# MrOlm/inStrain

Measured on AMD Instinct MI355X. Metric: Gbp profiled/s, higher is better.
Workload: dtype u32

## Files before the change

include/instrain_amd.h:

```cpp
#ifndef INSTRAIN_AMD_H
#define INSTRAIN_AMD_H

#include <stdint.h>

#ifdef __cplusplus
extern "C" {
#endif

#define ISX_OK 0
#define ISX_ERR_ARG (-1)
#define ISX_ERR_HIP (-2)
#define ISX_ERR_CAPACITY (-3)
#define ISX_ERR_MM_RANGE (-4)
#define ISX_ERR_IO (-5)
#define ISX_ERR_STATE (-6)

#define ISX_ABI_VERSION 5


typedef struct isx_ctx isx_ctx;
typedef struct isx_batch isx_batch;
typedef struct isx_bam isx_bam;
struct isx_bam_params_s;
struct isx_bam_info_s;
// ... 206 lines not shown
int isx_genes_create(isx_ctx *ctx, int64_t n_genes, const isx_gene *genes, const char *seq, int64_t seq_bytes, isx_genes **out);
void isx_genes_destroy(isx_genes *g);
int isx_genes_sites(isx_genes *g, double *sites, float *device_ms);
int isx_batch_profile_genes(isx_batch *b, isx_genes *g, int32_t n_scaffolds, const int64_t *scaffold_bounds, const int32_t *gene_first,
                            const int32_t *gene_last, isx_gene_cov *cov_out, uint8_t *scaffold_flags, float *device_ms);
int isx_genes_profile_snvs(isx_genes *g, int32_t n_scaffolds, const int64_t *scaffold_bounds, const int32_t *gene_first,
                           const int32_t *gene_last, int64_t n_snv, const isx_snv *snv, int32_t n_levels, isx_gene_mutation *mut_out,
                           isx_gene_snv_count *cnt_out, float *device_ms);

typedef struct isx_pipe isx_pipe;

typedef struct {
    int64_t max_pos;
    int64_t max_obs;
    int32_t max_splits;
    int32_t depth;
    int32_t host_threads;
    int32_t pin_threads;
    double jump_slack;
    int32_t want_counts;
    int32_t ring_kib;
    int32_t stage_async;
    int32_t lean_output;
    int64_t max_segs;
} isx_pipe_params;

typedef struct {
    uint32_t gpos;
    float clon_rarefied;
} isx_rare;

typedef struct {
    uint32_t gpos;
    uint32_t coverage;
} isx_sat;

typedef struct {
    int64_t ticket;
    int64_t n_pos, n_obs;
    isx_sizes sizes;
    const uint16_t *coverage16;
    const float *clon;
    const isx_rare *rare;
    int64_t n_rare, n_saturated;
    const uint32_t *counts;
    const float *clon_rarefied;
    const isx_snv *snv;
    isx_batch *batch;
    float encode_ms;
    float h2d_ms, kernel_ms, d2h_ms;
    float collect_wait_ms;
    int32_t record_bytes;
    int32_t encode_passes;
    int64_t h2d_bytes, d2h_bytes;
    const isx_ld *ld;
    const uint8_t *coverage8;
    const isx_rare *clon_sparse;
    int64_t n_clon;
    const isx_sat *saturated;
    const uint8_t *coverage4;
    const uint16_t *cov_rows;
    const uint32_t *cov_row_window;
    int64_t n_cov_rows;
    int32_t cov_window, pad_cov;
    const void *lev_mask;
    const void *lev_cov;
    const uint32_t *lev_win_off;
    const isx_rare *lev_clon, *lev_rare;
    const isx_sat *lev_sat;
    int64_t n_lev, n_lev_clon, n_lev_rare, n_lev_sat;
    int32_t lev_mask_bytes, lev_cov_bytes, lev_window, n_lev_windows, lev_min_cov, pad_lev;
    uint64_t rows_checksum;
} isx_pipe_result;

int isx_levels_expand(const isx_pipe_result *r, int32_t host_threads, uint32_t *gpos, uint32_t *mm_cov, float *clon, float *clon_rarefied);

int isx_pipe_create(isx_ctx *ctx, const isx_params *params, const isx_pipe_params *pp, isx_pipe **out);
void isx_pipe_destroy(isx_pipe *p);
int isx_pipe_submit(isx_pipe *p, int64_t n_pos, const uint8_t *ref, int32_t n_splits, const int64_t *split_bounds,
                    int64_t n_obs, const isx_obs *obs, const uint32_t *pair, int64_t *ticket);
int isx_pipe_submit_bam(isx_pipe *p, isx_bam *bam, const struct isx_bam_params_s *bp, const int32_t *refs, int32_t n_refs,
                        const uint8_t *ref, int32_t n_splits, const int64_t *split_bounds, struct isx_bam_info_s *info,
                        int64_t *ticket);
int isx_pipe_collect(isx_pipe *p, int64_t ticket, isx_pipe_result *out);
int isx_pipe_release(isx_pipe *p, int64_t ticket);
int isx_pipe_fetch_entries(isx_pipe *p, int64_t ticket, isx_entry *out);
int isx_pipe_fetch_entries_shrunk(isx_pipe *p, int64_t ticket, uint32_t *gpos, uint32_t *mm_cov, float *clon, float *clon_rarefied);


#define ISX_SEG_BASES 150
#define ISX_SEG_WORDS 15
#define ISX_SEG_SKIP_WORD 0x24924924u
#define ISX_DREC_WORDS 8
#define ISX_DREC_EXC 6
#define ISX_DREC_EXC_FULL 3
#define ISX_DREC_DUAL 0x80000000u
#define ISX_DREC_NO_EXC 0x3FFFFFFFu

typedef struct {
    int64_t n_seg;
    const uint32_t *gpos;
    const uint8_t *len;
    const uint8_t *mm;
    const uint32_t *pair;
    const uint32_t *bases;
} isx_segs;

int isx_batch_create_reads(isx_ctx *ctx, const isx_params *params, int64_t n_pos, const uint8_t *ref, int32_t n_splits,
                           const int64_t *split_bounds, const isx_segs *segs, isx_batch **out);
int isx_pipe_submit_reads(isx_pipe *p, int64_t n_pos, const uint8_t *ref, int32_t n_splits, const int64_t *split_bounds,
                          const isx_segs *segs, int64_t *ticket);

typedef struct isx_wire isx_wire;
int isx_pipe_stage_reads(isx_pipe *p, int64_t n_pos, const uint8_t *ref, int32_t n_splits, const int64_t *split_bounds,
                         const isx_segs *segs, isx_wire **out);
int isx_pipe_submit_wire(isx_pipe *p, const isx_wire *wire, int64_t *ticket);
int64_t isx_wire_bytes(const isx_wire *wire);
void isx_wire_free(isx_wire *wire);
int isx_wire_keep_reference(isx_pipe *p, isx_wire *wire);

#define ISX_PLANE_WORDS 8
typedef struct {
    int64_t n_seg;
    const uint32_t *gpos;
    const uint8_t *len;
    const uint32_t *pair;
    const uint64_t *planes;
    const uint8_t *mm;
} isx_read_planes;

typedef struct {
    const uint8_t *plane2;
    const uint8_t *nplane;
    uint64_t key;
} isx_ref_planes;

int isx_pack_ref_planes(const uint8_t *ref, int64_t n_pos, int32_t host_threads, uint8_t *plane2, uint8_t *nplane, int32_t *has_n);
int isx_planes_from_segs(const isx_segs *segs, int32_t host_threads, uint64_t *planes);
int isx_pack_read_planes(int64_t n_reads, const int64_t *ref_start, const int64_t *clip_lo, const int64_t *clip_hi,
                         const uint32_t *cigar, const int64_t *cigar_off, const char *seq, const uint8_t *qual, const int64_t *seq_off,
                         const uint32_t *pair, int32_t min_base_quality, int64_t cap_seg, uint32_t *seg_gpos,
                         uint8_t *seg_len, uint32_t *seg_pair, uint64_t *seg_planes, int64_t *n_seg);
int isx_pipe_submit_planes(isx_pipe *p, int64_t n_pos, const isx_ref_planes *ref, int32_t n_splits, const int64_t *split_bounds,
                           const isx_read_planes *reads, int64_t *ticket);
int isx_pipe_stage_planes(isx_pipe *p, int64_t n_pos, const isx_ref_planes *ref, int32_t n_splits, const int64_t *split_bounds,
                          const isx_read_planes *reads, isx_wire **out);
int isx_pipe_set_reference_budget(isx_pipe *p, int64_t mib);
int isx_host_register(const void *ptr, int64_t bytes);
int isx_host_unregister(const void *ptr);
int isx_encode_planes(const isx_read_planes *reads, const isx_ref_planes *ref, int64_t n_pos, int32_t host_threads, int32_t slack_groups,
                      int64_t cap_rec, int64_t ring_records, uint32_t *rec, uint32_t *gbase, int64_t *n_rec, int64_t *need_slack);
int isx_encode_planes_mm(const isx_read_planes *reads, const isx_ref_planes *ref, int64_t n_pos, int32_t n_mm_bins, int32_t host_threads, int32_t slack_groups,
                         int64_t cap_rec, int64_t ring_records, uint32_t *rec, uint32_t *gbase, int64_t *n_rec, int64_t *need_slack);

int isx_count_read_segs(int64_t n_reads, const uint32_t *cigar, const int64_t *cigar_off, const int64_t *ref_start,
                        const int64_t *clip_lo, const int64_t *clip_hi, int64_t *n_seg);
int isx_pack_reads(int64_t n_reads, const int64_t *ref_start, const int64_t *clip_lo, const int64_t *clip_hi,
                   const uint32_t *cigar, const int64_t *cigar_off, const char *seq, const uint8_t *qual, const int64_t *seq_off,
                   const uint8_t *mm, const uint32_t *pair, int32_t min_base_quality, int64_t cap_seg, uint32_t *seg_gpos,
                   uint8_t *seg_len, uint8_t *seg_mm, uint32_t *seg_pair, uint32_t *seg_bases, int64_t *n_seg);

int isx_encode_segs(const isx_segs *segs, int64_t n_pos, int32_t n_mm_bins, int32_t host_threads, int64_t cap_rec, uint32_t *rec,
                    uint32_t *gbase, uint32_t *pair_out, int64_t *n_rec);
int64_t isx_seg_records_needed(const uint32_t *gpos, int64_t n_seg, int32_t host_threads);
int isx_encode_segs_ring(const isx_segs *segs, int64_t n_pos, int32_t n_mm_bins, int32_t host_threads, int64_t cap_rec, int64_t ring_records,
                         uint32_t *rec, uint32_t *gbase, uint32_t *pair_out, int64_t *n_rec);

int isx_encode_delta(const isx_segs *segs, const uint8_t *ref, int64_t n_pos, int32_t n_mm_bins, int32_t host_threads, int32_t slack_groups,
                     int64_t cap_rec, int64_t ring_records, uint32_t *rec, uint32_t *gbase, uint32_t *pair_out, int64_t *n_rec, int64_t *need_slack);
int64_t isx_delta_records_needed(const uint32_t *gpos, int64_t n_seg, int32_t host_threads, int32_t slack_groups);

int isx_encode_obs(const isx_obs *obs, const uint32_t *pair, int64_t n_obs, int64_t n_pos, int32_t record_bytes,
                   int32_t host_threads, double slack, int64_t cap_rec, void *rec, uint32_t *gbase, uint32_t *pair_out,
                   int64_t *n_rec, int32_t *passes);
int isx_encode_obs_ring(const isx_obs *obs, const uint32_t *pair, int64_t n_obs, int64_t n_pos, int32_t record_bytes,
                        int32_t host_threads, double slack, int64_t cap_rec, int64_t ring_records, void *rec,
                        uint32_t *gbase, uint32_t *pair_out, int64_t *n_rec, int32_t *passes);

typedef struct {
    int64_t in_off;
    int32_t in_len;
    int32_t out_len;
    int64_t out_off;
} isx_bgzf_block;
int isx_bgzf_index(const uint8_t *image, int64_t n_bytes, int64_t cap_blocks, isx_bgzf_block *blocks, int64_t *n_blocks, int64_t *out_bytes);
int isx_bgzf_inflate_device(isx_ctx *ctx, const uint8_t *image, int64_t n_bytes, const isx_bgzf_block *blocks, int64_t n_blocks,
                            uint8_t *out, int64_t out_bytes, float *kernel_ms);
int isx_bgzf_inflate_host(const uint8_t *image, int64_t n_bytes, const isx_bgzf_block *blocks, int64_t n_blocks, uint8_t *out, int64_t out_bytes);
int isx_bgzf_inflate_fast(const uint8_t *image, int64_t n_bytes, const isx_bgzf_block *blocks, int64_t n_blocks, uint8_t *out, int64_t out_bytes);

typedef struct isx_bam_params_s {
    double min_read_ani;
    int32_t min_mapq;
    double max_insert_relative;
    int32_t min_insert;
    int32_t min_base_quality;
    int32_t skip_mm;
    int32_t window_length;
    int32_t pairing_filter;
} isx_bam_params;

typedef struct isx_bam_info_s {
    int32_t n_refs;
    int32_t n_splits;
    int64_t n_reads;
    int64_t n_pos;
    int64_t n_obs;
    int64_t n_pairs;
    int64_t unfiltered_pairs, filtered_pairs;
    int64_t filtered_bases;
    double median_insert;
    int32_t max_mm;
    int32_t pad;
    int64_t unfiltered_reads, unfiltered_singletons, filtered_singletons;
    int64_t n_segs;
} isx_bam_info;

int isx_bam_open(const char *path, isx_bam **out);
void isx_bam_close(isx_bam *bam);
void isx_bam_close_wait(isx_bam *bam);
int isx_bam_set_threads(isx_bam *bam, int32_t threads);
int isx_bam_ref(const isx_bam *bam, int32_t i, const char **name, int64_t *length, int64_t *flat_offset);
int isx_bam_set_priority_reads(isx_bam *bam, int64_t n, const char *names, const int64_t *offs);
int isx_bam_scan(isx_bam *bam, isx_bam_info *info );
int isx_bam_scan_part(isx_bam *bam, int32_t part, int32_t n_parts, isx_bam_info *info );
int isx_bam_set_wanted_refs(isx_bam *bam, const int32_t *refs, int32_t n);
int isx_bam_insert_sizes(isx_bam *bam, int64_t *out, int64_t cap, int64_t *n);
int isx_bam_filter(isx_bam *bam, const isx_bam_params *p, double median_insert , isx_bam_info *info);
int isx_bam_pair_keys(isx_bam *bam, uint64_t *h1, uint64_t *h2, int32_t *tid, int64_t *info4, int64_t cap, int64_t *n);
int isx_bam_set_cross_names(isx_bam *bam, int64_t n, const int64_t *entry, const int64_t *occurrences, const int64_t *info4);
int isx_bam_filter_insert_sizes(isx_bam *bam, int64_t *out, int64_t cap, int64_t *n);
int isx_bam_set_r2m(isx_bam *bam, int32_t ref, int64_t n, const char *names, const int64_t *offs, const int32_t *mm );
int isx_bam_set_mm_cap(isx_bam *bam, int32_t cap);
int isx_bam_mm_levels(const isx_bam *bam, int32_t *levels, int32_t cap, int32_t *n);
int isx_bam_set_mm_levels(isx_bam *bam, const int32_t *levels, int32_t n);
int isx_bam_batch_pair_names(const isx_bam *bam, int64_t *n, int64_t *name_bytes, char *names, int64_t *offs);
int isx_bam_r2m(const isx_bam *bam, int32_t ref, int64_t *n, int64_t *name_bytes, char *names, int64_t *offs, int32_t *mm);
int isx_bam_drop_names(isx_bam *bam);
int isx_bam_ref_counts(const isx_bam *bam, int64_t *reads, int64_t *filtered_pairs);
int isx_bam_expand_refs(isx_bam *bam, const isx_bam_params *p, const int32_t *refs, int32_t n_refs, isx_bam_info *info);
int isx_bam_segment_refs(isx_bam *bam, const isx_bam_params *p, const int32_t *refs, int32_t n_refs, isx_bam_info *info, int64_t *n_seg);
int isx_bam_copy_segs(const isx_bam *bam, uint32_t *gpos, uint8_t *len, uint8_t *mm, uint32_t *pair, uint32_t *bases,
                      int64_t *split_bounds, int32_t *split_ref);
int isx_bam_copy_read_planes(const isx_bam *bam, uint64_t *planes);
int isx_bam_expand_region(isx_bam *bam, const isx_bam_params *p, int32_t ref, int64_t start, int64_t stop, isx_bam_info *info);
int isx_bam_expand(isx_bam *bam, const isx_bam_params *p, isx_bam_info *info);
int isx_bam_copy(const isx_bam *bam, isx_obs *obs, uint32_t *pair, int64_t *split_bounds, int32_t *split_ref);
int isx_bam_view(const isx_bam *bam, const isx_obs **obs, const uint32_t **pair);

#ifdef __cplusplus
}
#endif
#endif
```

instrain_amd/_lib.py:

```python
import ctypes as C
import os

import numpy as np

_HERE = os.path.dirname(os.path.abspath(__file__))
LIB_PATH = os.path.join(_HERE, "libinstrain_amd.so")
if os.environ.get("ISX_LIB"):
    LIB_PATH = os.path.abspath(os.environ["ISX_LIB"])

BGZF_BLOCK_DT = np.dtype([("in_off", np.int64), ("in_len", np.int32), ("out_len", np.int32), ("out_off", np.int64)])
OBS_DT = np.dtype([("gpos", "<u4"), ("mm", "<u2"), ("base", "u1"), ("flags", "u1")])
ENTRY_DT = np.dtype([("gpos", "<u4"), ("mm", "<u2"), ("flags", "<u2"), ("cnt", "<u4", (4,)), ("clon", "<f4"),
                     ("clon_rarefied", "<f4")])
SNV_DT = np.dtype([("gpos", "<u4"), ("mm", "<u2"), ("con_base", "u1"), ("var_base", "u1"),
                   ("allele_count", "u1"), ("cls", "u1"), ("cryptic", "u1"), ("ref_base", "u1"),
                   ("cnt", "<u4", (4,))])
LD_DT = np.dtype([("gpos_a", "<u4"), ("gpos_b", "<u4"), ("mm", "<u2"), ("allele_A", "u1"), ("allele_a", "u1"),
                  ("allele_B", "u1"), ("allele_b", "u1"), ("pad", "<u2"), ("total", "<u4"), ("countAB", "<u4"),
                  ("countAb", "<u4"), ("countaB", "<u4"), ("countab", "<u4"), ("pad2", "<u4"),
                  ("r2", "<f8"), ("d_prime", "<f8"), ("r2_normalized", "<f8"), ("d_prime_normalized", "<f8")])
AO_DT = np.dtype([("pair", "<u4"), ("gpos", "<u4"), ("order", "<u4"), ("mm", "<u2"), ("base", "u1"), ("pad", "u1")])
assert AO_DT.itemsize == 16
assert OBS_DT.itemsize == 8 and ENTRY_DT.itemsize == 32 and SNV_DT.itemsize == 28 and LD_DT.itemsize == 72


class Params(C.Structure):
    _fields_ = [("min_cov", C.c_int32), ("min_snp", C.c_int32), ("min_freq", C.c_double),
                ("rarefied_coverage", C.c_int32), ("n_mm_bins", C.c_int32), ("enable_linkage", C.c_int32),
                ("linkage_mode", C.c_int32), ("window", C.c_int32), ("seed", C.c_uint64), ("layout", C.c_int32),
                ("reserved", C.c_int32)]


LAYOUT_WIDE_RECORDS, LAYOUT_NO_SHORT_RECORDS, LAYOUT_NO_PACKED_COUNTERS, LAYOUT_SEG64_RECORDS = 1, 2, 4, 8


class PipeParams(C.Structure):
    _fields_ = [("max_pos", C.c_int64), ("max_obs", C.c_int64), ("max_splits", C.c_int32), ("depth", C.c_int32),
                ("host_threads", C.c_int32), ("pin_threads", C.c_int32), ("jump_slack", C.c_double),
                ("want_counts", C.c_int32), ("ring_kib", C.c_int32), ("stage_async", C.c_int32), ("lean_output", C.c_int32),
                ("max_segs", C.c_int64)]


SEG_BASES, SEG_WORDS, SEG_SKIP_WORD = 150, 15, 0x24924924


class Segs(C.Structure):
    _fields_ = [("n_seg", C.c_int64), ("gpos", C.c_void_p), ("len", C.c_void_p), ("mm", C.c_void_p), ("pair", C.c_void_p),
                ("bases", C.c_void_p)]


PLANE_WORDS = 8
LAYOUT_MM_ENTRIES = 16
LAYOUT_MM_DELTA_RECORDS = 32
ABI_VERSION = 5


class ReadPlanes(C.Structure):
    _fields_ = [("n_seg", C.c_int64), ("gpos", C.c_void_p), ("len", C.c_void_p), ("pair", C.c_void_p), ("planes", C.c_void_p), ("mm", C.c_void_p)]


class RefPlanes(C.Structure):
    _fields_ = [("plane2", C.c_void_p), ("nplane", C.c_void_p), ("key", C.c_uint64)]


RARE_DT = np.dtype([("gpos", "<u4"), ("clon_rarefied", "<f4")])
CLON_DT = np.dtype([("gpos", "<u4"), ("clon", "<f4")])
SAT_DT = np.dtype([("gpos", "<u4"), ("coverage", "<u4")])


class Sizes(C.Structure):
    _fields_ = [(n, C.c_int64) for n in ("n_entries", "n_snv", "n_sites", "n_allele_obs", "n_increments",
                                         "n_edges", "n_ld")]


class Timings(C.Structure):
    _fields_ = [(n, C.c_float) for n in ("pileup_ms", "sites_ms", "allele_ms", "group_ms", "incr_ms", "ld_ms",
                                         "total_ms")] + \
               [(n, C.c_int32) for n in ("pileup_blocks", "pileup_threads", "pileup_lds_bytes", "pileup_window")] + \
               [("mfma_ms", C.c_float), ("dense_tiles", C.c_int32), ("dense_macs", C.c_int64), ("dense_bytes", C.c_int64),
                ("record_bytes", C.c_int32), ("pad", C.c_int32)]


class PipeResult(C.Structure):
    _fields_ = [("ticket", C.c_int64), ("n_pos", C.c_int64), ("n_obs", C.c_int64), ("sizes", Sizes),
                ("coverage16", C.c_void_p), ("clon", C.c_void_p), ("rare", C.c_void_p), ("n_rare", C.c_int64),
                ("n_saturated", C.c_int64), ("counts", C.c_void_p), ("clon_rarefied", C.c_void_p), ("snv", C.c_void_p),
                ("batch", C.c_void_p),
                ("encode_ms", C.c_float), ("h2d_ms", C.c_float), ("kernel_ms", C.c_float), ("d2h_ms", C.c_float),
                ("collect_wait_ms", C.c_float), ("record_bytes", C.c_int32), ("encode_passes", C.c_int32),
                ("h2d_bytes", C.c_int64), ("d2h_bytes", C.c_int64), ("ld", C.c_void_p),
                ("coverage8", C.c_void_p), ("clon_sparse", C.c_void_p), ("n_clon", C.c_int64), ("saturated", C.c_void_p),
                ("coverage4", C.c_void_p), ("cov_rows", C.c_void_p), ("cov_row_window", C.c_void_p), ("n_cov_rows", C.c_int64),
                ("cov_window", C.c_int32), ("pad_cov", C.c_int32),
                ("lev_mask", C.c_void_p), ("lev_cov", C.c_void_p), ("lev_win_off", C.c_void_p), ("lev_clon", C.c_void_p), ("lev_rare", C.c_void_p),
                ("lev_sat", C.c_void_p), ("n_lev", C.c_int64), ("n_lev_clon", C.c_int64), ("n_lev_rare", C.c_int64), ("n_lev_sat", C.c_int64),
                ("lev_mask_bytes", C.c_int32), ("lev_cov_bytes", C.c_int32), ("lev_window", C.c_int32), ("n_lev_windows", C.c_int32),
                ("lev_min_cov", C.c_int32), ("pad_lev", C.c_int32), ("rows_checksum", C.c_uint64)]


class BamParams(C.Structure):
    _fields_ = [("min_read_ani", C.c_double), ("min_mapq", C.c_int32), ("max_insert_relative", C.c_double),
                ("min_insert", C.c_int32), ("min_base_quality", C.c_int32), ("skip_mm", C.c_int32),
                ("window_length", C.c_int32), ("pairing_filter", C.c_int32)]


PAIRING_FILTERS = {"paired_only": 0, "non_discordant": 1, "all_reads": 2}


class BamInfo(C.Structure):
    _fields_ = [("n_refs", C.c_int32), ("n_splits", C.c_int32), ("n_reads", C.c_int64), ("n_pos", C.c_int64),
                ("n_obs", C.c_int64), ("n_pairs", C.c_int64), ("unfiltered_pairs", C.c_int64),
                ("filtered_pairs", C.c_int64), ("filtered_bases", C.c_int64), ("median_insert", C.c_double),
                ("max_mm", C.c_int32), ("pad", C.c_int32), ("unfiltered_reads", C.c_int64),
                ("unfiltered_singletons", C.c_int64), ("filtered_singletons", C.c_int64), ("n_segs", C.c_int64)]


SCAFFOLD_LEVEL_DT = np.dtype([("nonzero", "<i8"), ("sum_cov", "<u8"), ("sumsq_cov", "<u8"), ("median_cov", "<f8"),
                              ("counted", "<i8"), ("sum_clon", "<f8"), ("median_clon", "<f8"),
                              ("counted_rarefied", "<i8"), ("sum_clon_rarefied", "<f8"),
                              ("median_clon_rarefied", "<f8"), ("mm", "<i4"), ("present", "<i4")])
assert SCAFFOLD_LEVEL_DT.itemsize == 88
GENOME_LEVEL_DT = np.dtype([("n", "<i8"), ("sum_cov", "<u8"), ("sumsq_cov", "<u8"), ("median_cov", "<f8"), ("mm", "<i4"), ("pad", "<i4")])
assert GENOME_LEVEL_DT.itemsize == 40


COMPARE_LEVEL_DT = np.dtype([("both", "<i8"), ("either", "<i8"), ("mm", "<i4"), ("present_a", "<i4"),
                             ("present_b", "<i4"), ("pad", "<i4"), ("consensus_snps", "<i8"), ("population_snps", "<i8")])
assert COMPARE_LEVEL_DT.itemsize == 48
COMPARE_SNP_DT = np.dtype([("gpos", "<u4"), ("mm", "<u2"), ("consensus_snp", "u1"), ("population_snp", "u1"),
                           ("has_a", "u1"), ("has_b", "u1"), ("con_a", "u1"), ("ref_a", "u1"), ("var_a", "u1"),
                           ("con_b", "u1"), ("ref_b", "u1"), ("var_b", "u1"), ("cnt_a", "<u4", (4,)), ("cnt_b", "<u4", (4,))])
assert COMPARE_SNP_DT.itemsize == 48


GENE_DT = np.dtype([("start", "<i8"), ("end", "<i8"), ("seq_off", "<i8"), ("strand", "<i4"), ("pad", "<i4")])
GENE_COV_DT = np.dtype([("sum_cov", "<u8"), ("nonzero", "<u4"), ("counted", "<u4"), ("sum_clon", "<f8")])
GENE_SNV_COUNT_DT = np.dtype([(n, "<u4") for n in ("divergent", "sns", "sns_n", "sns_s", "snv", "snv_n", "snv_s")])
GENE_MUTATION_DT = np.dtype([("gene", "<i4"), ("k", "<i4"), ("type", "u1"), ("aa_old", "u1"), ("aa_new", "u1"), ("n_genes", "u1"),
                             ("pad", "<u4")])
assert GENE_DT.itemsize == 32 and GENE_COV_DT.itemsize == 24 and GENE_SNV_COUNT_DT.itemsize == 28 and GENE_MUTATION_DT.itemsize == 16
GENE_LEVEL_PRESENT, GENE_COV_ANY, GENE_CLON_ANY = 1, 2, 4


ERR_CAPACITY = -3


class IsxError(RuntimeError):
    def __init__(self, code, msg):
        super().__init__("libinstrain_amd error %d: %s" % (code, msg))
        self.code = code


SYMBOLS = ["isx_last_error", "isx_abi_version", "isx_ctx_create", "isx_ctx_destroy", "isx_ctx_reserve_cus", "isx_set_null_model",
           "isx_batch_create", "isx_batch_create_reads", "isx_batch_destroy", "isx_batch_run", "isx_batch_launch", "isx_batch_wait", "isx_batch_sizes", "isx_batch_timings",
           "isx_batch_fetch_entries", "isx_batch_fetch_dense", "isx_batch_fetch_snv", "isx_batch_fetch_ld", "isx_batch_fetch_allele_obs",
           "isx_batch_summarize", "isx_batch_summarize_genomes", "isx_compare_coverage", "isx_compare_scaffolds", "isx_compare_fetch_snps",
           "isx_genes_create", "isx_genes_destroy", "isx_genes_sites", "isx_batch_profile_genes", "isx_genes_profile_snvs",
           "isx_pipe_create", "isx_pipe_destroy", "isx_pipe_submit", "isx_pipe_submit_reads", "isx_pipe_stage_reads", "isx_pipe_submit_wire", "isx_wire_bytes", "isx_wire_free", "isx_wire_keep_reference", "isx_pipe_submit_bam", "isx_encode_segs", "isx_encode_segs_ring", "isx_seg_records_needed", "isx_encode_delta", "isx_delta_records_needed", "isx_count_read_segs", "isx_pack_reads", "isx_pipe_collect", "isx_pipe_release", "isx_pipe_fetch_entries", "isx_pipe_fetch_entries_shrunk", "isx_levels_expand", "isx_encode_obs", "isx_encode_obs_ring",
           "isx_pack_ref_planes", "isx_planes_from_segs", "isx_pack_read_planes", "isx_pipe_submit_planes", "isx_pipe_stage_planes", "isx_encode_planes", "isx_encode_planes_mm", "isx_pipe_set_reference_budget", "isx_host_register", "isx_host_unregister",
           "isx_bgzf_index", "isx_bgzf_inflate_device", "isx_bgzf_inflate_host", "isx_bgzf_inflate_fast",
           "isx_bam_open", "isx_bam_close", "isx_bam_close_wait", "isx_bam_set_threads", "isx_bam_ref", "isx_bam_set_priority_reads", "isx_bam_scan", "isx_bam_scan_part",
           "isx_bam_insert_sizes", "isx_bam_set_wanted_refs", "isx_bam_pair_keys", "isx_bam_set_cross_names", "isx_bam_filter_insert_sizes", "isx_bam_filter", "isx_bam_set_r2m", "isx_bam_r2m", "isx_bam_drop_names", "isx_bam_batch_pair_names", "isx_bam_set_mm_cap", "isx_bam_mm_levels", "isx_bam_set_mm_levels", "isx_bam_ref_counts",
           "isx_bam_expand_refs", "isx_bam_segment_refs", "isx_bam_copy_segs", "isx_bam_copy_read_planes", "isx_bam_expand_region", "isx_bam_expand", "isx_bam_copy", "isx_bam_view"]

_lib = None


def load():
    global _lib
    if _lib is not None:
        return _lib
    if not os.path.exists(LIB_PATH):
        raise IsxError(-2, "%s not built: run `python -c 'import __graft_entry__ as g; g.build()'` "
                           "(hipcc --offload-arch=gfx950)" % LIB_PATH)
    lib = C.CDLL(LIB_PATH)
    vp, i32, i64 = C.c_void_p, C.c_int32, C.c_int64
    lib.isx_last_error.restype = C.c_char_p
    lib.isx_abi_version.restype = C.c_int
    if lib.isx_abi_version() != ABI_VERSION:
        raise IsxError(-6, "%s has ABI version %d, this package binds version %d: rebuild it (python -c 'import __graft_entry__ as g; g.build()')"
                       % (LIB_PATH, lib.isx_abi_version(), ABI_VERSION))
    lib.isx_ctx_create.argtypes = [C.c_int, C.POINTER(vp)]
    lib.isx_ctx_destroy.argtypes = [vp]
    lib.isx_ctx_reserve_cus.argtypes = [vp, C.c_int]
    lib.isx_bgzf_index.argtypes = [vp, i64, i64, vp, C.POINTER(i64), C.POINTER(i64)]
    lib.isx_bgzf_inflate_device.argtypes = [vp, vp, i64, vp, i64, vp, i64, C.POINTER(C.c_float)]
    lib.isx_bgzf_inflate_host.argtypes = [vp, i64, vp, i64, vp, i64]
    lib.isx_bgzf_inflate_fast.argtypes = [vp, i64, vp, i64, vp, i64]
    lib.isx_ctx_destroy.restype = None
    lib.isx_set_null_model.argtypes = [vp, vp, i64, i32]
    lib.isx_batch_create.argtypes = [vp, C.POINTER(Params), i64, vp, i32, vp, i64, vp, vp, C.POINTER(vp)]
    lib.isx_batch_create_reads.argtypes = [vp, C.POINTER(Params), i64, vp, i32, vp, C.POINTER(Segs), C.POINTER(vp)]
    lib.isx_pipe_submit_reads.argtypes = [vp, i64, vp, i32, vp, C.POINTER(Segs), C.POINTER(i64)]
    lib.isx_pipe_stage_reads.argtypes = [vp, i64, vp, i32, vp, C.POINTER(Segs), C.POINTER(vp)]
    lib.isx_pipe_submit_wire.argtypes = [vp, vp, C.POINTER(i64)]
    lib.isx_wire_bytes.argtypes = [vp]
    lib.isx_wire_bytes.restype = i64
    lib.isx_wire_free.argtypes = [vp]
    lib.isx_wire_keep_reference.argtypes = [vp, vp]
    lib.isx_wire_free.restype = None
    lib.isx_encode_segs.argtypes = [C.POINTER(Segs), i64, i32, i32, i64, vp, vp, vp, C.POINTER(i64)]
    lib.isx_encode_segs_ring.argtypes = [C.POINTER(Segs), i64, i32, i32, i64, i64, vp, vp, vp, C.POINTER(i64)]
    lib.isx_encode_delta.argtypes = [C.POINTER(Segs), vp, i64, i32, i32, i32, i64, i64, vp, vp, vp, C.POINTER(i64), C.POINTER(i64)]
    lib.isx_delta_records_needed.argtypes = [vp, i64, i32, i32]
    lib.isx_delta_records_needed.restype = i64
    lib.isx_seg_records_needed.argtypes = [vp, i64, i32]
    lib.isx_seg_records_needed.restype = i64
    lib.isx_count_read_segs.argtypes = [i64, vp, vp, vp, vp, vp, C.POINTER(i64)]
    lib.isx_pack_reads.argtypes = [i64, vp, vp, vp, vp, vp, vp, vp, vp, vp, vp, i32, i64, vp, vp, vp, vp, vp, C.POINTER(i64)]
    lib.isx_batch_destroy.argtypes = [vp]
    lib.isx_batch_destroy.restype = None
    lib.isx_batch_run.argtypes = [vp]
    lib.isx_batch_launch.argtypes = [vp]
    lib.isx_batch_wait.argtypes = [vp]
    lib.isx_batch_sizes.argtypes = [vp, C.POINTER(Sizes)]
    lib.isx_batch_timings.argtypes = [vp, C.POINTER(Timings)]
    for f in ("isx_batch_fetch_entries", "isx_batch_fetch_snv", "isx_batch_fetch_ld", "isx_batch_fetch_allele_obs"):
        getattr(lib, f).argtypes = [vp, vp]
    lib.isx_batch_fetch_dense.argtypes = [vp, vp, vp, vp]
    lib.isx_batch_summarize.argtypes = [vp, i32, vp, vp, C.POINTER(C.c_float)]
    lib.isx_batch_summarize_genomes.argtypes = [vp, i32, vp, i32, vp, i32, vp, C.POINTER(C.c_float)]
    lib.isx_compare_coverage.argtypes = [vp, vp, i32, vp, i32, vp, C.POINTER(C.c_float)]
    lib.isx_compare_scaffolds.argtypes = [vp, vp, i32, vp, i32, C.c_double, vp, C.POINTER(i64), C.POINTER(C.c_float)]
    lib.isx_compare_fetch_snps.argtypes = [vp, vp]
    lib.isx_genes_create.argtypes = [vp, i64, vp, C.c_char_p, i64, C.POINTER(vp)]
    lib.isx_genes_destroy.argtypes = [vp]
    lib.isx_genes_destroy.restype = None
    lib.isx_genes_sites.argtypes = [vp, vp, C.POINTER(C.c_float)]
    lib.isx_batch_profile_genes.argtypes = [vp, vp, i32, vp, vp, vp, vp, vp, C.POINTER(C.c_float)]
    lib.isx_genes_profile_snvs.argtypes = [vp, i32, vp, vp, vp, i64, vp, i32, vp, vp, C.POINTER(C.c_float)]
    lib.isx_pipe_create.argtypes = [vp, C.POINTER(Params), C.POINTER(PipeParams), C.POINTER(vp)]
    lib.isx_pipe_destroy.argtypes = [vp]
    lib.isx_pipe_destroy.restype = None
    lib.isx_pipe_submit.argtypes = [vp, i64, vp, i32, vp, i64, vp, vp, C.POINTER(i64)]
    lib.isx_pipe_submit_bam.argtypes = [vp, vp, C.POINTER(BamParams), vp, i32, vp, i32, vp, C.POINTER(BamInfo), C.POINTER(i64)]
    lib.isx_pipe_collect.argtypes = [vp, i64, C.POINTER(PipeResult)]
    lib.isx_pipe_release.argtypes = [vp, i64]
    lib.isx_pipe_fetch_entries.argtypes = [vp, i64, vp]
    lib.isx_pipe_fetch_entries_shrunk.argtypes = [vp, i64, vp, vp, vp, vp]
    lib.isx_levels_expand.argtypes = [C.POINTER(PipeResult), i32, vp, vp, vp, vp]
    lib.isx_encode_obs.argtypes = [vp, vp, i64, i64, i32, i32, C.c_double, i64, vp, vp, vp, C.POINTER(i64), C.POINTER(i32)]
    lib.isx_encode_obs_ring.argtypes = [vp, vp, i64, i64, i32, i32, C.c_double, i64, i64, vp, vp, vp, C.POINTER(i64), C.POINTER(i32)]
    lib.isx_bam_open.argtypes = [C.c_char_p, C.POINTER(vp)]
    lib.isx_bam_close.argtypes = [vp]
    lib.isx_bam_close.restype = None
    lib.isx_bam_close_wait.argtypes = [vp]
    lib.isx_bam_close_wait.restype = None
    lib.isx_bam_expand.argtypes = [vp, C.POINTER(BamParams), C.POINTER(BamInfo)]
    lib.isx_bam_set_threads.argtypes = [vp, i32]
    lib.isx_bam_set_priority_reads.argtypes = [vp, i64, C.c_char_p, vp]
    lib.isx_bam_scan.argtypes = [vp, C.POINTER(BamInfo)]
    lib.isx_bam_scan_part.argtypes = [vp, i32, i32, C.POINTER(BamInfo)]
    lib.isx_bam_set_wanted_refs.argtypes = [vp, vp, i32]
    lib.isx_bam_insert_sizes.argtypes = [vp, vp, i64, C.POINTER(i64)]
    lib.isx_bam_filter_insert_sizes.argtypes = [vp, vp, i64, C.POINTER(i64)]
    lib.isx_bam_pair_keys.argtypes = [vp, vp, vp, vp, vp, i64, C.POINTER(i64)]
    lib.isx_bam_set_cross_names.argtypes = [vp, i64, vp, vp, vp]
    lib.isx_bam_filter.argtypes = [vp, C.POINTER(BamParams), C.c_double, C.POINTER(BamInfo)]
    lib.isx_bam_set_r2m.argtypes = [vp, i32, i64, C.c_char_p, vp, vp]
    lib.isx_bam_drop_names.argtypes = [vp]
    lib.isx_bam_r2m.argtypes = [vp, i32, C.POINTER(i64), C.POINTER(i64), vp, vp, vp]
    lib.isx_bam_batch_pair_names.argtypes = [vp, C.POINTER(i64), C.POINTER(i64), vp, vp]
    lib.isx_bam_set_mm_cap.argtypes = [vp, i32]
    lib.isx_bam_mm_levels.argtypes = [vp, vp, i32, vp]
    lib.isx_bam_set_mm_levels.argtypes = [vp, vp, i32]
    lib.isx_bam_ref_counts.argtypes = [vp, vp, vp]
    lib.isx_bam_expand_region.argtypes = [vp, C.POINTER(BamParams), i32, i64, i64, C.POINTER(BamInfo)]
    lib.isx_bam_expand_refs.argtypes = [vp, C.POINTER(BamParams), vp, i32, C.POINTER(BamInfo)]
    lib.isx_bam_segment_refs.argtypes = [vp, C.POINTER(BamParams), vp, i32, C.POINTER(BamInfo), C.POINTER(i64)]
    lib.isx_bam_copy_segs.argtypes = [vp, vp, vp, vp, vp, vp, vp, vp]
    lib.isx_bam_copy_read_planes.argtypes = [vp, vp]
    lib.isx_pack_ref_planes.argtypes = [vp, i64, i32, vp, vp, C.POINTER(i32)]
    lib.isx_planes_from_segs.argtypes = [C.POINTER(Segs), i32, vp]
    lib.isx_pack_read_planes.argtypes = [i64, vp, vp, vp, vp, vp, vp, vp, vp, vp, i32, i64, vp, vp, vp, vp, C.POINTER(i64)]
    lib.isx_pipe_submit_planes.argtypes = [vp, i64, C.POINTER(RefPlanes), i32, vp, C.POINTER(ReadPlanes), C.POINTER(i64)]
    lib.isx_pipe_set_reference_budget.argtypes = [vp, i64]
    lib.isx_host_register.argtypes = [vp, i64]
    lib.isx_host_unregister.argtypes = [vp]
    lib.isx_pipe_stage_planes.argtypes = [vp, i64, C.POINTER(RefPlanes), i32, vp, C.POINTER(ReadPlanes), C.POINTER(vp)]
    lib.isx_encode_planes.argtypes = [C.POINTER(ReadPlanes), C.POINTER(RefPlanes), i64, i32, i32, i64, i64, vp, vp, C.POINTER(i64), C.POINTER(i64)]
    lib.isx_encode_planes_mm.argtypes = [C.POINTER(ReadPlanes), C.POINTER(RefPlanes), i64, i32, i32, i32, i64, i64, vp, vp, C.POINTER(i64), C.POINTER(i64)]
    lib.isx_bam_ref.argtypes = [vp, i32, C.POINTER(C.c_char_p), C.POINTER(i64), C.POINTER(i64)]
    lib.isx_bam_copy.argtypes = [vp, vp, vp, vp, vp]
    lib.isx_bam_view.argtypes = [vp, C.POINTER(vp), C.POINTER(vp)]
    _lib = lib
    return lib


def check(rc):
    if rc != 0:
        raise IsxError(rc, load().isx_last_error().decode(errors="replace"))
```

instrain_amd/csrc/isx_pipe.hip:

```cpp
#include <atomic>
#include <algorithm>
#include <chrono>
#include <cmath>
#include <condition_variable>
#include <cstring>
#include <deque>
#include <mutex>
#include <memory>
#include <string>
#include <thread>
#include <vector>

#include "bam_front.h"
#include "isx_batch.h"
#include "obs_encode.h"
#include "seg_encode.h"
#include "isx_summary.h"
#include <unordered_map>

namespace {

constexpr size_t ALIGN = 256;
inline size_t up(size_t v, size_t a = ALIGN) { return (v + a - 1) / a * a; }

double now_ms()
{
    return std::chrono::duration<double, std::milli>(std::chrono::steady_clock::now().time_since_epoch()).count();
}

int host_block_alloc(void **p, size_t bytes, bool pinned)
{
    *p = nullptr;
    if (pinned) { HIP_TRY(isx_pin_malloc(p, std::max<size_t>(bytes, 1))); return ISX_OK; }
    if (posix_memalign(p, 4096, std::max<size_t>(bytes, 4096)) != 0) { *p = nullptr; isx_set_error("out of host memory"); return ISX_ERR_ARG; }
    return ISX_OK;
}

void host_block_free(void *p, bool pinned)
{
    if (!p) return;
    if (pinned) isx_pin_free(p); else free(p);
}

static const bool pipe_timing = getenv("ISX_PIPE_TIMING") != nullptr;
#define H2D(p, s) ((s).h2d ? (s).h2d : (p)->s_h2d)
struct Slot {
    isx_batch *b = nullptr;
    hipStream_t h2d = nullptr;
    uint8_t *h_in = nullptr, *d_in = nullptr;
    size_t in_bytes = 0;
    size_t off_bounds = 0, off_win = 0, off_ref = 0, off_gbase = 0, off_ridx = 0, off_rec = 0;
    size_t off_pairs = 0;
    isxenc::PairRun *h_runs = nullptr;
    bool runs_pinned = true;
    uint2 *d_runs = nullptr;
    size_t cap_runs = 0;
    hipEvent_t ev_ring[2] = {nullptr, nullptr};
    bool ring_busy[2] = {false, false};
    uint8_t *h_out = nullptr;
    uint8_t *h_small = nullptr;
    size_t small_bytes = 0;
    bool out_pinned = true;
    size_t out_bytes = 0, o_counts = 0, o_clon = 0, o_clonr = 0, o_snv = 0, o_cov16 = 0, o_rare = 0;
    bool rare_dense = false;
    bool cov8 = false, clon_sparse = false;
    bool cov4 = false;
    size_t cov_rows_off = 0;
    int cov_window = 0;
    std::vector<uint32_t> cov_row_win;
    std::vector<isx_sat> sat_rows;
    bool sat_complete = true;
    void *sort_temp = nullptr;
    size_t sort_temp_bytes = 0;
    std::vector<float> clonr_big;
    std::vector<isx_rare> rare_big;
    std::vector<uint32_t> cmin, cmax, dir_pmax, dir_smin;
    std::vector<uint8_t> cany;
    std::vector<uint2> win;
    size_t o_lmask = 0, o_lwin = 0, o_lcov = 0, o_lclon = 0, o_lrare = 0;
    size_t lcov_room = 0, lclon_room = 0, lrare_room = 0;
    std::vector<uint8_t> lcov_big;
    std::vector<isx_rare> lclon_big, lrare_big;
    std::vector<isx_snv> snv_big;
    std::vector<isx_ld> ld_rows;
    uint64_t rows_checksum = 0;
    hipEvent_t ev_h2d0 = nullptr, ev_h2d1 = nullptr, ev_pass = nullptr, ev_d2h0 = nullptr, ev_d2h1 = nullptr;
    hipEvent_t ev_h2da = nullptr, ev_h2db = nullptr;
    bool h2d_split = false;
    int64_t ticket = -1;
    BamBatch *dead_batch = nullptr;
    bool ref_has_n = false;
    int state = 0;
    int rc = 0;
    std::string err;
    float finish_wait_ms = 0.f;
    float encode_ms = 0.f;
    int encode_passes = 0;
    int64_t h2d_bytes = 0, d2h_bytes = 0;
    uint16_t *d_gpos16 = nullptr;
};

static uint64_t bytes_checksum(const void *p, size_t bytes, uint64_t seed)
{
    const uint8_t *b = static_cast<const uint8_t *>(p);
    uint64_t a[4] = {seed ^ 0x9E3779B97F4A7C15ull, seed + 0xC2B2AE3D27D4EB4Full, seed ^ 0x165667B19E3779F9ull, seed + 0x27D4EB2F165667C5ull};
    const size_t n8 = bytes / 8;
    size_t i = 0;
    for (; i + 4 <= n8; i += 4) {
        uint64_t w[4];
        memcpy(w, b + 8 * i, 32);
        for (int k = 0; k < 4; k++) a[k] = a[k] * 0x100000001B3ull + w[k];
    }
    uint64_t h = (uint64_t)bytes;
    for (; i < n8; i++) { uint64_t w; memcpy(&w, b + 8 * i, 8); h = h * 0x100000001B3ull + w; }
    for (size_t j = n8 * 8; j < bytes; j++) h = h * 0x100000001B3ull + b[j];
    for (int k = 0; k < 4; k++) { h ^= a[k]; h *= 0xFF51AFD7ED558CCDull; h ^= h >> 33; }
    return h;
}

static inline size_t ref2_bytes(int64_t n_pos) { return (((size_t)n_pos + 3) / 4 + 15) & ~(size_t)15; }
static inline size_t refn_bytes(int64_t n_pos) { return (((size_t)n_pos + 7) / 8 + 15) & ~(size_t)15; }

static bool copy_ref_planes(isxenc::HostPool &pool, const isx_ref_planes *rp, int64_t n_pos, uint8_t *plane2, uint8_t *nplane)
{
    const size_t b2 = ((size_t)n_pos + 3) / 4, bn = ((size_t)n_pos + 7) / 8;
    const size_t piece = (size_t)1 << 20;
    const int t2 = (int)((b2 + piece - 1) / piece), tn = rp->nplane ? (int)((bn + piece - 1) / piece) : 0;
    std::atomic<int> any{0};
    pool.run(t2 + tn, [&](int t) {
        if (t < t2) { const size_t a = (size_t)t * piece; memcpy(plane2 + a, rp->plane2 + a, std::min(piece, b2 - a)); return; }
        const size_t a = (size_t)(t - t2) * piece, n = std::min(piece, bn - a);
        const uint8_t *src = rp->nplane + a;
        uint8_t acc = 0;
        for (size_t i = 0; i < n; i++) acc |= src[i];
        memcpy(nplane + a, src, n);
        if (acc) any.store(1, std::memory_order_relaxed);
    });
    return any.load() != 0;
}

static bool plane_any(isxenc::HostPool &pool, const uint8_t *pl, size_t bytes)
{
    const size_t piece = (size_t)1 << 20;
    const int nt = (int)((bytes + piece - 1) / piece);
    std::atomic<int> any{0};
    pool.run(nt, [&](int t) {
        const size_t a = (size_t)t * piece, n = std::min(piece, bytes - a);
        uint64_t acc = 0;
        size_t i = 0;
        for (; i + 8 <= n; i += 8) { uint64_t v; memcpy(&v, pl + a + i, 8); acc |= v; }
        for (; i < n; i++) acc |= pl[a + i];
        if (acc) any.store(1, std::memory_order_relaxed);
    });
    return any.load() != 0;
}

static uint64_t ref_plane_checksum(const uint8_t *plane2, int64_t n_pos)
{
    const size_t words = (((size_t)n_pos + 3) / 4) / 8;
    uint64_t h = 0x9E3779B97F4A7C15ull ^ (uint64_t)n_pos;
    if (!words) { for (size_t i = 0; i < ((size_t)n_pos + 3) / 4; i++) h = (h ^ plane2[i]) * 0x100000001B3ull; return h; }
    const size_t n_s = std::min<size_t>(words, 4096), step = words / n_s;
    for (size_t k = 0; k < n_s; k++) {
        uint64_t w;
        memcpy(&w, plane2 + 8 * (k * step), 8);
        h = (h ^ w) * 0x100000001B3ull;
        h ^= h >> 29;
    }
    return h;
}

int cgroup_cpus()
{
    if (FILE *f = fopen("/sys/fs/cgroup/cpu.max", "r")) {
        char q[64] = {0};
        long period = 0;
        const int n = fscanf(f, "%63s %ld", q, &period);
        fclose(f);
        if (n == 2 && period > 0 && strcmp(q, "max") != 0) return (int)std::max<long>(1, atol(q) / period);
    }
    return 0;
}

int gpu_numa_node(int device)
{
    char bus[64] = {0};
    if (hipDeviceGetPCIBusId(bus, sizeof bus, device) != hipSuccess) return -1;
    std::string id(bus);
    std::transform(id.begin(), id.end(), id.begin(), [](unsigned char ch) { return (char)std::tolower(ch); });
    int node = -1;
    if (FILE *f = fopen(("/sys/bus/pci/devices/" + id + "/numa_node").c_str(), "r")) {
        if (fscanf(f, "%d", &node) != 1) node = -1;
        fclose(f);
    }
    return node;
}

}

struct isx_pipe {
    isx_ctx *ctx = nullptr;
    isx_params prm{};
    isx_pipe_params pp{};
    std::unique_ptr<isxenc::HostPool> pool;
    std::vector<Slot> slots;
    hipStream_t s_h2d = nullptr, s_d2h = nullptr;
    hipStream_t s_h2d2 = nullptr;
    hipStream_t s_fin = nullptr;
    hipStream_t s_fin2 = nullptr;
    int64_t next_ticket = 0;
    int64_t cap_rec = 0;
    int64_t ring_half = 0;
    int rb = 2;
    bool segs = false;
    bool drec = false;
    int64_t dslack = 1;
    uint32_t G = ISX_GROUP16;
    size_t snv_prefix = 0;
    size_t rare_prefix = 0, cap_rare = 0;
    double slack = 0.0;
    std::thread finisher;
    std::thread finisher2;
    std::vector<std::thread> more_finishers;
    std::vector<hipStream_t> extra_fin;
    std::mutex bounce_mu;
    std::mutex mu;
    std::condition_variable cv_work, cv_done;
    std::deque<int64_t> work;
    bool stop = false;
    std::mutex launch_mu;
    uint8_t *bounce[2] = {nullptr, nullptr};
    hipEvent_t bounce_ev[2] = {nullptr, nullptr};
    size_t bounce_bytes = 0;
    std::unique_ptr<isxenc::HostPool> fin_pool;
    struct StageJob {
        int64_t ticket, n_pos;
        const uint8_t *ref;
        std::vector<int64_t> bounds;
        isx_segs segs;
        bool planes = false;
        isx_read_planes reads{};
        isx_ref_planes rp{};
    };
    struct RefEntry { uint8_t *d = nullptr; size_t bytes = 0; int64_t n_pos = 0; bool has_n = false; hipEvent_t ready = nullptr; uint64_t sum = 0; };
    std::unordered_map<uint64_t, RefEntry> ref_cache;
    size_t ref_cache_bytes = 0;
    std::atomic<size_t> ref_cache_budget{(size_t)4096 << 20};
    std::thread stager;
    std::deque<StageJob> stage_q;
    std::condition_variable cv_stage;
    int64_t next_promise = 0;
    bool stage_stop = false;
};

static int bounce_d2h(isx_pipe *p, void *hdst, const void *dsrc, size_t bytes, hipStream_t st)
{
    if (!bytes) return ISX_OK;
    std::lock_guard<std::mutex> bounce_lk(p->bounce_mu);
    const size_t piece = p->bounce_bytes;
    const size_t n_pieces = (bytes + piece - 1) / piece;
    auto issue = [&](size_t k) -> hipError_t {
        const size_t off = k * piece, len = std::min(piece, bytes - off);
        hipError_t e = isx_copy_to_host(p->bounce[k & 1], static_cast<const uint8_t *>(dsrc) + off, len, st);
        return e == hipSuccess ? hipEventRecord(p->bounce_ev[k & 1], st) : e;
    };
    HIP_TRY(issue(0));
    for (size_t k = 0; k < n_pieces; k++) {
        if (k + 1 < n_pieces) HIP_TRY(issue(k + 1));
        HIP_TRY(isx_wait_event(p->bounce_ev[k & 1]));
        const size_t off = k * piece, len = std::min(piece, bytes - off);
        const size_t sub = (size_t)1 << 20;
        const uint8_t *src = p->bounce[k & 1];
        uint8_t *dst = static_cast<uint8_t *>(hdst) + off;
        p->fin_pool->run((int)((len + sub - 1) / sub), [&](int t) {
            const size_t a = (size_t)t * sub;
            memcpy(dst + a, src + a, std::min(sub, len - a));
        });
    }
    return ISX_OK;
}

static void pipe_free(isx_pipe *p)
{
    if (!p) return;
    if (p->stager.joinable()) {
        { std::lock_guard<std::mutex> lk(p->mu); p->stage_stop = true; }
        p->cv_stage.notify_all();
        p->stager.join();
    }
    if (p->finisher.joinable()) {
        { std::lock_guard<std::mutex> lk(p->mu); p->stop = true; }
        p->cv_work.notify_all();
        p->finisher.join();
        if (p->finisher2.joinable()) p->finisher2.join();
        for (auto &t : p->more_finishers) if (t.joinable()) t.join();
    }
    (void)hipSetDevice(p->ctx->device);
    if (p->s_h2d) (void)isx_wait_stream(p->s_h2d);
    if (p->s_h2d2) (void)isx_wait_stream(p->s_h2d2);
    if (p->s_d2h) (void)isx_wait_stream(p->s_d2h);
    if (p->s_fin) (void)isx_wait_stream(p->s_fin);
    if (p->s_fin2) (void)isx_wait_stream(p->s_fin2);
    for (hipStream_t st : p->extra_fin) (void)isx_wait_stream(st);
    for (int i = 0; i < 2; i++) if (p->ctx->pstream[i]) (void)isx_wait_stream(p->ctx->pstream[i]);
    const double t_f0 = now_ms();
    double t_batch = 0, t_dev = 0, t_pin = 0;
    for (Slot &s : p->slots) {
        double t_x = now_ms();
        if (s.b) {
            isx_batch *b = s.b;
            b->d_seg = nullptr; b->d_drec = nullptr;
            b->d_rec = nullptr; b->d_rec32 = nullptr; b->d_rec16 = nullptr; b->d_gbase = nullptr; b->d_pair = nullptr;
            b->d_pair_runs = nullptr; b->d_run_index = nullptr;
            b->d_gpos = nullptr; b->d_gpos16 = nullptr; b->d_cbase = nullptr; b->d_ref = nullptr; b->d_win = nullptr;
            b->d_bounds = nullptr;
            isx_batch_destroy(b);
        }
        t_batch += now_ms() - t_x; t_x = now_ms();
        if (s.sort_temp) isx_dev_free(s.sort_temp);
        if (s.d_gpos16) isx_dev_free(s.d_gpos16);
        if (s.d_in) isx_dev_free(s.d_in);
        if (s.d_runs) isx_dev_free(s.d_runs);
        t_dev += now_ms() - t_x; t_x = now_ms();
        if (s.h_in) isx_pin_free(s.h_in);
        host_block_free(s.h_runs, s.runs_pinned);
        for (hipEvent_t e : s.ev_ring) if (e) (void)hipEventDestroy(e);
        host_block_free(s.h_out, s.out_pinned);
        if (s.h_small) isx_pin_free(s.h_small);
        t_pin += now_ms() - t_x;
        for (hipEvent_t e : {s.ev_h2d0, s.ev_h2d1, s.ev_pass, s.ev_d2h0, s.ev_d2h1, s.ev_h2da, s.ev_h2db}) if (e) (void)hipEventDestroy(e);
    }
    if (pipe_timing)
        fprintf(stderr, "[isx_pipe_destroy] device tables %.1f ms, device arena %.1f ms, pinned staging %.1f ms, total %.1f ms\n", t_batch, t_dev, t_pin, now_ms() - t_f0);
    for (auto &kv : p->ref_cache) { if (kv.second.d) isx_dev_free(kv.second.d); if (kv.second.ready) (void)hipEventDestroy(kv.second.ready); }
    for (int i = 0; i < 2; i++) {
        if (p->bounce[i]) isx_pin_free(p->bounce[i]);
        if (p->bounce_ev[i]) (void)hipEventDestroy(p->bounce_ev[i]);
    }
    if (p->s_h2d) (void)hipStreamDestroy(p->s_h2d);
    if (p->s_h2d2) (void)hipStreamDestroy(p->s_h2d2);
    if (p->s_d2h) (void)hipStreamDestroy(p->s_d2h);
    if (p->s_fin) (void)hipStreamDestroy(p->s_fin);
    if (p->s_fin2) (void)hipStreamDestroy(p->s_fin2);
    for (hipStream_t st : p->extra_fin) (void)hipStreamDestroy(st);
    delete p;
}

static int slot_batch_create(isx_pipe *p, Slot &s, int index)
{
    isx_ctx *c = p->ctx;
    const isx_params *prm = &p->prm;
    const double t_s0 = now_ms();
    isx_batch *b = new isx_batch();
    s.b = b;
    b->ctx = c; b->prm = *prm; b->M = prm->n_mm_bins;
    b->ps = getenv("ISX_ONE_PASS_QUEUE") ? 0 : (index & 1);
    b->cap_pos = p->pp.max_pos; b->cap_obs = p->pp.max_obs; b->arena = true; b->ref_packed = 2;
    b->n_pos = p->pp.max_pos; b->n_obs = p->pp.max_obs;
    b->segs = p->segs; b->drec = p->drec;
    b->lean = p->pp.lean_output != 0 && !p->pp.want_counts;
    b->lev_sparse = b->M > 1 && b->M <= 32 && p->segs && !p->pp.want_counts && !(prm->layout & ISX_LAYOUT_MM_ENTRIES);
    b->spin_us = (p->pp.host_threads > 0 && p->pp.host_threads < 8) ? 200 : 2000;
    const bool dense = b->M == 1;
    batch_pick_block(b);
    const int64_t cap_pos = p->pp.max_pos;
    for (auto &e : b->ev) HIP_TRY(hipEventCreate(&e));
    for (auto &e : b->ev_sum) HIP_TRY(hipEventCreate(&e));
    HIP_TRY(isx_dev_malloc(reinterpret_cast<void **>(&b->d_cursors), (CUR_N + 4) * sizeof(uint32_t)));
    b->d_flags = b->d_cursors + CUR_N;
    HIP_TRY(hipHostMalloc(&b->h_state, (CUR_N + 8) * sizeof(uint32_t), hipHostMallocMapped | hipHostMallocCoherent));
    memset(b->h_state, 0, (CUR_N + 8) * sizeof(uint32_t));
    HIP_TRY(hipHostGetDevicePointer(reinterpret_cast<void **>(&b->d_host_state), b->h_state, 0));
    HIP_TRY(hipMemset(b->d_cursors, 0, (CUR_N + 4) * sizeof(uint32_t)));
    {
        std::vector<uint16_t> thr = build_thresholds(c->h_lut, c->fallback, prm->min_freq);
        HIP_TRY(isx_dev_malloc(reinterpret_cast<void **>(&b->d_thr), thr.size() * sizeof(uint16_t)));
        HIP_TRY(hipMemcpy(b->d_thr, thr.data(), thr.size() * sizeof(uint16_t), hipMemcpyHostToDevice));
    }
    const uint64_t npm = (uint64_t)cap_pos * b->M;
    const uint64_t cap_obs = (uint64_t)std::max<int64_t>(p->pp.max_obs, 1);
    if (dense) {
        if (p->pp.want_counts) HIP_TRY(isx_dev_malloc(reinterpret_cast<void **>(&b->d_counts), (size_t)cap_pos * sizeof(uint4)));
        else {
            b->cap_clon = (size_t)cap_pos / 2 + 65536;
            HIP_TRY(isx_dev_malloc(reinterpret_cast<void **>(&b->d_cov8), (size_t)cap_pos));
            if (p->pp.lean_output) {
                b->cap_cov_row_win = (size_t)cap_pos / 64 + 2;
                HIP_TRY(isx_dev_malloc(reinterpret_cast<void **>(&b->d_cov_row_win), b->cap_cov_row_win * sizeof(uint32_t)));
            }
            HIP_TRY(isx_dev_malloc(reinterpret_cast<void **>(&b->d_clon_list), b->cap_clon * sizeof(uint2)));
            HIP_TRY(isx_dev_malloc(reinterpret_cast<void **>(&b->d_clon_sorted), b->cap_clon * sizeof(uint2)));
        }
        b->cap_sat = (size_t)cap_pos / 16 + 65536;
        HIP_TRY(isx_dev_malloc(reinterpret_cast<void **>(&b->d_sat), b->cap_sat * sizeof(uint2)));
        HIP_TRY(isx_dev_malloc(reinterpret_cast<void **>(&b->d_clon), (size_t)cap_pos * sizeof(float)));
        HIP_TRY(isx_dev_malloc(reinterpret_cast<void **>(&b->d_clon_r), (size_t)cap_pos * sizeof(float)));
        HIP_TRY(isx_dev_malloc(reinterpret_cast<void **>(&b->d_cov16), (size_t)cap_pos * sizeof(uint16_t)));
        if (prm->rarefied_coverage > 0) {
            b->cap_rare = p->cap_rare;
            HIP_TRY(isx_dev_malloc(reinterpret_cast<void **>(&b->d_rare), b->cap_rare * sizeof(uint2)));
        }
    } else if (b->lev_sparse) {
        b->lev_mask_bytes = b->M <= 8 ? 1 : (b->M <= 16 ? 2 : 4);
        b->cap_lev = (size_t)std::min<uint64_t>(std::min<uint64_t>(npm, 0xFFFFFFF0ull), std::max<uint64_t>((uint64_t)cap_pos * (uint64_t)std::min(b->M, 4), 1u << 20));
        HIP_TRY(isx_dev_malloc(&b->d_lev_mask, (size_t)cap_pos * b->lev_mask_bytes + 64));
// ... 289 lines not shown

static void finisher_main(isx_pipe *p, hipStream_t sfin)
{
    (void)hipSetDevice(p->ctx->device);
    for (;;) {
        int64_t ticket;
        {
            std::unique_lock<std::mutex> lk(p->mu);
            p->cv_work.wait(lk, [&] { return p->stop || !p->work.empty(); });
            if (p->work.empty()) return;
            ticket = p->work.front();
            p->work.pop_front();
        }
        Slot &s = p->slots[(size_t)(ticket % (int64_t)p->slots.size())];
        const int rc = finish_slot(p, s, sfin);
        std::string err = rc == ISX_OK ? std::string() : std::string(isx_last_error());
        BamBatch *dead = nullptr;
        {
            std::lock_guard<std::mutex> lk(p->mu);
            s.rc = rc; s.err.swap(err);
            dead = s.dead_batch; s.dead_batch = nullptr;
            s.state = 2;
        }
        p->cv_done.notify_all();
        if (dead) bam_batch_retire(dead);
    }
}

static int submit_segs_common(isx_pipe *p, int64_t n_pos, const uint8_t *ref, int32_t n_splits, const int64_t *split_bounds,
                              isxenc::SegJob &J, int64_t *ticket, const isx_ref_planes *rp = nullptr);

static void stager_main(isx_pipe *p)
{
    for (;;) {
        isx_pipe::StageJob job;
        {
            std::unique_lock<std::mutex> lk(p->mu);
            p->cv_stage.wait(lk, [&] { return p->stage_stop || !p->stage_q.empty(); });
            if (p->stage_q.empty()) return;
            job = std::move(p->stage_q.front());
            p->stage_q.pop_front();
        }
        isxenc::SegJob J;
        if (job.planes) { J.in2 = job.reads; J.n_seg = job.reads.n_seg; }
        else { J.in = job.segs; J.n_seg = job.segs.n_seg; }
        int64_t got = -1;
        const int rc = submit_segs_common(p, job.n_pos, job.ref, (int32_t)job.bounds.size() - 1, job.bounds.data(), J, &got, job.planes ? &job.rp : nullptr);
        if (rc != ISX_OK) {
            Slot &s = p->slots[(size_t)(job.ticket % (int64_t)p->slots.size())];
            std::string err(isx_last_error());
            std::lock_guard<std::mutex> lk(p->mu);
            s.ticket = job.ticket; s.rc = rc; s.err.swap(err); s.state = 2;
            p->next_ticket = job.ticket + 1;
        }
        p->cv_done.notify_all();
    }
}

static void drain_stager(isx_pipe *p)
{
    if (!p->stager.joinable()) return;
    std::unique_lock<std::mutex> lk(p->mu);
    p->cv_done.wait(lk, [&] { return p->next_ticket == p->next_promise; });
}

extern "C" {

int isx_pipe_create(isx_ctx *c, const isx_params *prm, const isx_pipe_params *pp, isx_pipe **out)
{
    if (!c || !prm || !pp || !out) { isx_set_error("isx_pipe_create: bad argument"); return ISX_ERR_ARG; }
    *out = nullptr;
    if (!c->d_lut) { isx_set_error("isx_pipe_create: call isx_set_null_model first"); return ISX_ERR_STATE; }
    if (prm->n_mm_bins < 1 || prm->n_mm_bins > 128) { isx_set_error("n_mm_bins must be in [1, 128]"); return ISX_ERR_ARG; }
    if (pp->max_pos <= 0 || pp->max_obs < 0 || pp->max_splits <= 0 || pp->depth < 1 || pp->depth > 64 || pp->max_segs < 0) {
        isx_set_error("isx_pipe_create: max_pos > 0, max_obs >= 0, max_segs >= 0, max_splits > 0, 1 <= depth <= 64");
        return ISX_ERR_ARG;
    }
    if (pp->max_segs > 0 && prm->linkage_mode == 2) { isx_set_error("isx_pipe_create: the dense MFMA linkage path takes observation batches only"); return ISX_ERR_ARG; }
    if (pp->max_pos >= (int64_t)0xFFFF0000ll) { isx_set_error("flat position space must be < 2^32 - 65536"); return ISX_ERR_ARG; }
    if (prm->window && (prm->window < 64 || (prm->window & 63) || prm->window > 8192)) { isx_set_error("window must be a multiple of 64 in [64, 8192]"); return ISX_ERR_ARG; }
    if (prm->layout & ISX_LAYOUT_WIDE_RECORDS) { isx_set_error("a pipe streams 2- / 4-byte records only"); return ISX_ERR_ARG; }
    HIP_TRY(hipSetDevice(c->device));
    isx_pipe *p = new isx_pipe();
    p->ctx = c; p->prm = *prm; p->pp = *pp;
    p->segs = pp->max_segs > 0;
    p->drec = p->segs && !(prm->layout & ISX_LAYOUT_SEG64_RECORDS) && (prm->n_mm_bins == 1 || (prm->layout & ISX_LAYOUT_MM_DELTA_RECORDS));
    p->rb = p->segs ? (p->drec ? 32 : 64) : ((prm->n_mm_bins == 1 && !(prm->layout & ISX_LAYOUT_NO_SHORT_RECORDS)) ? 2 : 4);
    p->G = p->segs ? (p->drec ? ISX_DREC_GROUP : ISX_SEG_GROUP) : (p->rb == 2 ? ISX_GROUP16 : ISX_GROUP);
    const double js = pp->jump_slack > 0 ? pp->jump_slack : 0.25;
    if (p->segs) {
        if (p->pp.max_obs == 0) p->pp.max_obs = pp->max_segs * ISX_SEG_BASES;
        const uint64_t G = p->G;
        const uint64_t groups = (uint64_t)(pp->max_segs + G - 1) / G + (uint64_t)pp->max_segs / 4096 * (p->drec ? 3 : 1) + (uint64_t)pp->max_pos / 65536 +
                                (uint64_t)pp->max_splits + 64 + (uint64_t)((double)pp->max_segs / G * js * (p->drec ? 1.0 : 0.25));
        p->cap_rec = (int64_t)(groups * G);
        if ((uint64_t)p->cap_rec >= (1ull << 26)) { delete p; isx_set_error("more than 2^26 segment records in one batch (4 GiB of records)"); return ISX_ERR_ARG; }
        const size_t rec_bytes = (size_t)p->cap_rec * (size_t)p->rb;
        size_t ring = 0;
        if (pp->ring_kib > 0) ring = (size_t)pp->ring_kib << 10;
        else if (pp->ring_kib == 0 && rec_bytes > ((size_t)(pp->depth == 1 ? 96 : 256) << 20)) ring = (size_t)64 << 20;
        if (ring && ring < rec_bytes) {
            p->ring_half = (int64_t)(ring / 2 / (size_t)p->rb) / (int64_t)p->G * (int64_t)p->G;
            if (p->ring_half * p->rb < (4096 + 16 * ISX_SEG_GROUP) * 64) { delete p; isx_set_error("isx_pipe_create: ring_kib too small for a read-level pipe (at least 1024)"); return ISX_ERR_ARG; }
        }
    } else {
        const uint64_t want = (uint64_t)((double)pp->max_obs * (1.0 + js)) + 4 * ISX_PAD;
        p->cap_rec = (int64_t)((want + ISX_PAD - 1) / ISX_PAD * ISX_PAD);
        if ((uint64_t)p->cap_rec >= 0xFFFFFFFFull) { delete p; isx_set_error("more than 2^32 records in one batch"); return ISX_ERR_ARG; }
    }
    if (!p->segs) {
        const size_t rec_bytes = (size_t)p->cap_rec * p->rb;
        size_t ring = 0;
        if (pp->ring_kib > 0) ring = (size_t)pp->ring_kib << 10;
        else if (pp->ring_kib == 0 && pp->depth == 1 && rec_bytes > ((size_t)128 << 20)) ring = (size_t)64 << 20;
        else if (pp->ring_kib == 0 && rec_bytes > ((size_t)512 << 20)) ring = (size_t)256 << 20;
        if (ring && ring < rec_bytes) {
            p->ring_half = (int64_t)(ring / 2 / p->rb) / ISX_PAD * ISX_PAD;
            if (p->ring_half < 2 * ISX_PAD) { delete p; isx_set_error("isx_pipe_create: ring_kib too small (at least 32)"); return ISX_ERR_ARG; }
        }
    }
    p->snv_prefix = (size_t)std::min<int64_t>(std::max<int64_t>(pp->max_pos / 64, 1 << 16), 1 << 22);
    p->cap_rare = (size_t)std::max<int64_t>(pp->max_pos, 1 << 16);
    p->rare_prefix = (size_t)std::max<int64_t>(pp->max_pos / 16, 1 << 16);
    int nt = pp->host_threads;
    if (nt <= 0) {
        const int q = cgroup_cpus();
        nt = q > 0 ? q : (int)std::thread::hardware_concurrency();
        nt = std::max(1, std::min(nt, 32));
    }
    c->n_pipes++;
    const double t_c0 = now_ms();
    p->pool.reset(new isxenc::HostPool(nt, gpu_numa_node(c->device), pp->pin_threads != 0));
    const double t_c1 = now_ms();
    int rc = ISX_OK;
    hipError_t e;
    if ((e = isx_side_stream_create(c, &p->s_h2d)) != hipSuccess ||
        (e = isx_side_stream_create(c, &p->s_fin)) != hipSuccess ||
        (e = isx_side_stream_create(c, &p->s_fin2)) != hipSuccess ||
        (e = isx_side_stream_create(c, &p->s_d2h)) != hipSuccess) {
        isx_set_error(std::string("isx_pipe_create: ") + hipGetErrorString(e));
        pipe_free(p);
        return ISX_ERR_HIP;
    }
    p->slots.resize((size_t)pp->depth);
    {
        const char *e2 = getenv("ISX_PIPE_H2D_STREAMS");
        if (e2 && atoi(e2) >= 2 && pp->depth >= 2 && isx_side_stream_create(c, &p->s_h2d2) != hipSuccess) { p->s_h2d2 = nullptr; (void)hipGetLastError(); }
    }
    for (int i = 0; i < pp->depth && rc == ISX_OK; i++) {
        rc = slot_batch_create(p, p->slots[(size_t)i], i);
        if ((i & 1) && p->s_h2d2) p->slots[(size_t)i].h2d = p->s_h2d2;
    }
    if (rc != ISX_OK) { pipe_free(p); return rc; }
    if (!p->slots[0].out_pinned) {
        p->bounce_bytes = (size_t)16 << 20;
        for (int i = 0; i < 2 && rc == ISX_OK; i++) {
            if (isx_pin_malloc(reinterpret_cast<void **>(&p->bounce[i]), p->bounce_bytes) != hipSuccess ||
                hipEventCreateWithFlags(&p->bounce_ev[i], hipEventDisableTiming) != hipSuccess) rc = ISX_ERR_HIP;
        }
        if (rc != ISX_OK) { isx_set_error("isx_pipe_create: bounce buffers"); pipe_free(p); return rc; }
        p->fin_pool.reset(new isxenc::HostPool(std::max(1, std::min(nt, 6)), -1, false));
    }
    p->finisher = std::thread(finisher_main, p, p->s_fin);
    if (pp->depth >= 2) p->finisher2 = std::thread(finisher_main, p, p->s_fin2);
    {
        int want = pp->depth >= 4 ? 4 : 2;
        if (const char *e = getenv("ISX_PIPE_FINISHERS")) want = std::max(1, atoi(e));
        want = std::min(want, pp->depth);
        for (int i = 2; i < want; i++) {
            hipStream_t st = nullptr;
            if (isx_side_stream_create(c, &st) != hipSuccess) break;
            p->extra_fin.push_back(st);
            p->more_finishers.emplace_back(finisher_main, p, st);
        }
    }
    if (pipe_timing)
        fprintf(stderr, "[isx_pipe_create] thread pool %.1f ms, %d slot(s) %.1f ms\n", t_c1 - t_c0, pp->depth, now_ms() - t_c1);
    if (pp->stage_async && p->segs) p->stager = std::thread(stager_main, p);
    *out = p;
    return ISX_OK;
}

void isx_pipe_destroy(isx_pipe *p) { pipe_free(p); }

static int enqueue_pass_impl(isx_pipe *p, Slot &s, int64_t n_pos, int64_t *ticket);

static int enqueue_pass(isx_pipe *p, Slot &s, int64_t n_pos, int64_t *ticket)
{
    const int rc = enqueue_pass_impl(p, s, n_pos, ticket);
    if (rc != ISX_OK) {
        const std::string why(isx_last_error());
        (void)isx_wait_stream(H2D(p, s));
        (void)isx_wait_stream(p->ctx->pstream[s.b->ps]);
        (void)isx_wait_stream(p->s_d2h);
        isx_set_error(why);
    }
    return rc;
}

static int enqueue_pass_impl(isx_pipe *p, Slot &s, int64_t n_pos, int64_t *ticket)
{
    isx_ctx *c = p->ctx;
    isx_batch *b = s.b;
    const bool dense = b->M == 1, linkage = p->prm.enable_linkage != 0;
    hipStream_t ps = c->pstream[b->ps];
    int rc = ISX_OK;
    std::unique_lock<std::mutex> launch_lk(p->launch_mu);
    HIP_TRY(hipStreamWaitEvent(ps, s.ev_h2d1, 0));
    if (dense && p->prm.rarefied_coverage > 0 && b->rare_dense)
        HIP_TRY(hipMemsetD32Async(reinterpret_cast<hipDeviceptr_t>(b->d_clon_r), 0x7FC00000, (size_t)n_pos, ps));
    if (linkage && p->rb == 4)
        launch_extract_gpos(nullptr, b->d_rec32, b->d_gbase, nullptr, b->d_gpos16, b->d_gbase, ISX_GROUP, b->n_rec, ps);
    if ((rc = launch_pass(b)) != ISX_OK) return rc;
    {
        PileupArgs pa{};
        pa.cursors = b->d_cursors; pa.host_state = b->d_host_state;
        launch_publish_state(pa, b->epoch, ps);
        b->publish_enqueued = true;
        if (c->unpublished[b->ps] == b) c->unpublished[b->ps] = nullptr;
    }
    HIP_TRY(hipEventRecord(s.ev_pass, ps));

    HIP_TRY(hipStreamWaitEvent(p->s_d2h, s.ev_pass, 0));
    HIP_TRY(hipEventRecord(s.ev_d2h0, p->s_d2h));
    const size_t snv_rows = std::min(p->snv_prefix, b->cap_snv);
    HIP_TRY(isx_copy_rows_to_host(s.h_small + s.o_snv, b->d_snv, b->d_cursors + CUR_SNV, b->base[CUR_SNV], (uint32_t)sizeof(isx_snv), snv_rows, p->s_d2h));
    s.d2h_bytes = 0;
    if (dense) {
        if (p->prm.rarefied_coverage > 0) {
            const size_t n = std::min(p->rare_prefix, std::min(p->cap_rare, (size_t)n_pos));
            HIP_TRY(isx_copy_rows_to_host(s.h_small + s.o_rare, b->d_rare, b->d_cursors + CUR_RARE, b->base[CUR_RARE], (uint32_t)sizeof(isx_rare), n, p->s_d2h));
        }
        if (!b->sparse_out) s.d2h_bytes += (int64_t)n_pos * 6;
    }
    if (dense && s.out_pinned && !b->sparse_out) {
        HIP_TRY(isx_copy_to_host(s.h_out + s.o_cov16, b->d_cov16, (size_t)n_pos * 2, p->s_d2h));
        HIP_TRY(isx_copy_to_host(s.h_out + s.o_clon, b->d_clon, (size_t)n_pos * 4, p->s_d2h));
        if (p->pp.want_counts) {
            HIP_TRY(isx_copy_to_host(s.h_out + s.o_counts, b->d_counts, (size_t)n_pos * 16, p->s_d2h));
            s.d2h_bytes += (int64_t)n_pos * 16;
            if (p->prm.rarefied_coverage > 0) {
                HIP_TRY(isx_copy_to_host(s.h_out + s.o_clonr, b->d_clon_r, (size_t)n_pos * 4, p->s_d2h));
                s.d2h_bytes += (int64_t)n_pos * 4;
            }
        }
    }
    HIP_TRY(hipEventRecord(s.ev_d2h1, p->s_d2h));
    launch_lk.unlock();
    {
        std::lock_guard<std::mutex> lk(p->mu);
        s.ticket = p->next_ticket++;
        if (p->next_promise < p->next_ticket) p->next_promise = p->next_ticket;
        s.state = 1; s.rc = ISX_OK;
        *ticket = s.ticket;
        p->work.push_back(s.ticket);
    }
    p->cv_work.notify_one();
    return ISX_OK;
}


static int check_capacity(const isx_pipe *p, const char *who, int64_t n_pos, int64_t n_items, int64_t max_items, int32_t n_splits)
{
    if (n_pos > p->pp.max_pos || n_items > max_items || n_splits > p->pp.max_splits) {
        isx_set_error(std::string(who) + ": batch larger than the pipe was created for");
        return ISX_ERR_CAPACITY;
    }
    return ISX_OK;
}

static int slot_acquire(isx_pipe *p, const char *who, Slot **out)
{
    Slot &s = p->slots[(size_t)(p->next_ticket % (int64_t)p->slots.size())];
    {
        std::lock_guard<std::mutex> lk(p->mu);
        if (s.state != 0) { isx_set_error(std::string(who) + ": every slot is in use (collect + release the oldest batch first)"); return ISX_ERR_STATE; }
    }
    HIP_TRY(hipSetDevice(p->ctx->device));
    *out = &s;
    return ISX_OK;
}

static int queue_for_stager(isx_pipe *p, isx_pipe::StageJob &&job, const char *who, int64_t *ticket)
{
    const int rc = check_capacity(p, who, job.n_pos, job.planes ? job.reads.n_seg : job.segs.n_seg, p->pp.max_segs, (int32_t)job.bounds.size() - 1);
    if (rc != ISX_OK) return rc;
    {
        std::lock_guard<std::mutex> lk(p->mu);
        const int64_t t = p->next_promise, n = (int64_t)p->slots.size();
        const Slot &s = p->slots[(size_t)(t % n)];
        if (t - n >= p->next_ticket || s.state != 0) { isx_set_error(std::string(who) + ": every slot is in use (collect + release the oldest batch first)"); return ISX_ERR_STATE; }
        job.ticket = t;
        p->next_promise = t + 1;
        *ticket = t;
        p->stage_q.push_back(std::move(job));
    }
    p->cv_stage.notify_one();
    return ISX_OK;
}

struct RingFeed { hipError_t err = hipSuccess; size_t bytes = 0; };

static int ring_feed_install(isx_pipe *p, Slot &s, RingFeed &r, int64_t &ring_groups, std::function<void(int)> &wave_begin,
                             std::function<void(int, int64_t, int64_t)> &wave_flush)
{
    if (p->ring_half <= 0) return ISX_OK;
    HIP_TRY(hipEventRecord(s.ev_h2d0, H2D(p, s)));
    const size_t half_bytes = (size_t)p->ring_half * (size_t)p->rb, grp_bytes = (size_t)p->G * (size_t)p->rb;
    uint8_t *d_rec = s.d_in + s.off_rec;
    ring_groups = p->ring_half / (int64_t)p->G;
    wave_begin = [&s, &r](int h) {
        if (s.ring_busy[h]) { const hipError_t e = isx_wait_event(s.ev_ring[h]); if (e != hipSuccess && r.err == hipSuccess) r.err = e; s.ring_busy[h] = false; }
    };
    wave_flush = [p, &s, &r, half_bytes, grp_bytes, d_rec](int h, int64_t g0, int64_t g1) {
        const size_t n = (size_t)(g1 - g0) * grp_bytes;
        if (g0 == 0) r.bytes = 0;
        hipError_t e = hipMemcpyAsync(d_rec + (size_t)g0 * grp_bytes, s.h_in + s.off_rec + (size_t)h * half_bytes, n, hipMemcpyHostToDevice, H2D(p, s));
        if (e == hipSuccess) e = hipEventRecord(s.ev_ring[h], H2D(p, s));
        if (e != hipSuccess && r.err == hipSuccess) r.err = e;
        s.ring_busy[h] = true;
        r.bytes += n;
    };
    return ISX_OK;
}

static int slot_choose_windows(isx_pipe *p, Slot &s, uint32_t chunk, bool threads)
{
    isx_batch *b = s.b;
    DirThreads mt{*p->pool, s.dir_pmax, s.dir_smin};
    const ChunkDir dir{s.cmin.data(), s.cmax.data(), s.cany.data(), b->n_rec / chunk, chunk};
    b->W = choose_windows(b, b->n_pos, dir, threads ? &mt : nullptr, s.win, &b->packed);
    b->n_win = (int)s.win.size();
    if (s.win.size() > (size_t)p->pp.max_pos / 64 + 2) { isx_set_error("internal: window directory larger than the arena"); return ISX_ERR_STATE; }
    memcpy(s.h_in + s.off_win, s.win.data(), s.win.size() * sizeof(uint2));
    return ISX_OK;
}

constexpr double COV8_BELOW_DEPTH = 16.0;
constexpr double NIB_BELOW_DEPTH = 6.0;
constexpr double LEV_COV8_BELOW_DEPTH = 64.0;
constexpr double RARE_DENSE_OBS_FACTOR = 4.0;

static int slot_shape_pass(isx_pipe *p, Slot &s)
{
    isx_batch *b = s.b;
    const bool dense = b->M == 1;
    const double n_obs = (double)b->n_obs, n_pos = (double)b->n_pos;
    b->sparse_out = dense && b->d_clon_list != nullptr;
    b->cov8_out = b->sparse_out && n_obs < COV8_BELOW_DEPTH * n_pos;
    b->nib_out = b->cov8_out && b->lean && n_obs < NIB_BELOW_DEPTH * n_pos;
    b->clon_dense = false;
    b->rare_dense = !(b->lean && b->sparse_out) || n_obs * RARE_DENSE_OBS_FACTOR >= (double)p->prm.rarefied_coverage * n_pos;
    if (b->lev_sparse) b->lev_cov_bytes = n_obs < LEV_COV8_BELOW_DEPTH * n_pos ? 1 : 2;
    const int rc = batch_set_geometry(b);
    if (rc != ISX_OK) return rc;
    if (!dense && !b->lev_sparse) {
        const size_t used = (size_t)b->n_win * b->slab;
        if (used > b->slab_region) { isx_set_error("internal: entry slabs larger than the slot's region"); return ISX_ERR_STATE; }
        b->cap_ovf = b->cap_entries - used;
    }
    return ISX_OK;
}

static void slot_bind_inputs(isx_pipe *p, Slot &s, uint8_t *resident_ref)
{
    isx_batch *b = s.b;
    const bool linkage = p->prm.enable_linkage != 0;
    uint8_t *rec = s.d_in + s.off_rec;
    b->d_bounds = reinterpret_cast<int64_t *>(s.d_in + s.off_bounds);
    b->d_win = reinterpret_cast<uint2 *>(s.d_in + s.off_win);
    b->d_ref = resident_ref ? resident_ref : s.d_in + s.off_ref;
    b->d_ref_n = s.ref_has_n ? b->d_ref + ref2_bytes(b->n_pos) : nullptr;
    b->d_gbase = reinterpret_cast<uint32_t *>(s.d_in + s.off_gbase);
    b->d_rec16 = p->rb == 2 ? reinterpret_cast<uint16_t *>(rec) : nullptr;
    b->d_rec32 = p->rb == 4 ? reinterpret_cast<uint32_t *>(rec) : nullptr;
    if (p->segs) {
        b->d_seg = p->drec ? nullptr : reinterpret_cast<uint4 *>(rec);
        b->d_drec = p->drec ? reinterpret_cast<uint4 *>(rec) : nullptr;
        b->d_pair = linkage && !p->drec ? reinterpret_cast<uint32_t *>(s.d_in + s.off_pairs) : nullptr;
        b->d_pair_runs = nullptr; b->d_run_index = nullptr; b->n_runs = 0;
    } else {
        b->d_pair = nullptr;
        b->d_pair_runs = linkage ? s.d_runs : nullptr;
        b->d_run_index = linkage ? reinterpret_cast<uint32_t *>(s.d_in + s.off_ridx) : nullptr;
        b->d_gpos16 = s.d_gpos16; b->gpos16_shift = 5;
    }
}

static void ref_cache_insert(isx_pipe *p, Slot &s, const isx_ref_planes *rp, int64_t n_pos)
{
    const size_t rb_all = ref2_bytes(n_pos) + (s.ref_has_n ? refn_bytes(n_pos) : 0);
    if (p->ref_cache_bytes + rb_all > p->ref_cache_budget.load(std::memory_order_relaxed)) return;
    isx_pipe::RefEntry e;
    bool ok = isx_dev_malloc(reinterpret_cast<void **>(&e.d), rb_all + 64) == hipSuccess && hipEventCreateWithFlags(&e.ready, hipEventDisableTiming) == hipSuccess;
    ok = ok && hipMemcpyAsync(e.d, s.d_in + s.off_ref, rb_all, hipMemcpyDeviceToDevice, H2D(p, s)) == hipSuccess && hipEventRecord(e.ready, H2D(p, s)) == hipSuccess;
    if (ok) {
        e.bytes = rb_all; e.n_pos = n_pos; e.has_n = s.ref_has_n; e.sum = ref_plane_checksum(rp->plane2, n_pos);
        p->ref_cache_bytes += rb_all;
        p->ref_cache.emplace(rp->key, e);
    } else {
        if (e.d) isx_dev_free(e.d);
        if (e.ready) (void)hipEventDestroy(e.ready);
        (void)hipGetLastError();
    }
}

struct RefStage {
    bool early = false;
    uint8_t *resident = nullptr;
    double host_ms = 0.0;
};

static int stage_reference(isx_pipe *p, Slot &s, int64_t n_pos, const uint8_t *ref, const isx_ref_planes *rp, isxenc::SegJob &J, RefStage *out)
{
    const bool ring = p->ring_half > 0;
    const double t_r = now_ms();
    const size_t b2 = ((size_t)n_pos + 3) / 4, bn = ((size_t)n_pos + 7) / 8;
    hipStream_t st = H2D(p, s);

    const auto hit = rp && rp->key ? p->ref_cache.find(rp->key) : p->ref_cache.end();
    if (hit != p->ref_cache.end()) {
        const isx_pipe::RefEntry &e = hit->second;
        if (e.n_pos != n_pos || e.has_n != (rp->nplane != nullptr && e.has_n) || e.sum != ref_plane_checksum(rp->plane2, n_pos)) {
            isx_set_error("isx_pipe_submit_planes: the reference key stands for other planes (positions / non-ACGT plane / content differ)");
            return ISX_ERR_ARG;
        }
        s.ref_has_n = e.has_n;
        J.ref2 = rp->plane2; J.refn = e.has_n ? rp->nplane : nullptr;
        out->resident = e.d;
        HIP_TRY(hipStreamWaitEvent(st, e.ready, 0));
        if (!ring) HIP_TRY(hipEventRecord(s.ev_h2d0, st));
        HIP_TRY(hipEventRecord(s.ev_h2da, st));
        out->early = true;
        out->host_ms = now_ms() - t_r;
        return ISX_OK;
    }

    const bool first_trip = rp && rp->key && p->ref_cache_budget.load(std::memory_order_relaxed) > 0;
    if (rp && !first_trip && isx_host_is_registered(rp->plane2, b2) && (!rp->nplane || isx_host_is_registered(rp->nplane, bn))) {
        const bool any_n = rp->nplane && plane_any(*p->pool, rp->nplane, bn);
        s.ref_has_n = any_n;
        J.ref2 = rp->plane2; J.refn = any_n ? rp->nplane : nullptr;
        out->host_ms = now_ms() - t_r;
        if (!ring) HIP_TRY(hipEventRecord(s.ev_h2d0, st));
        HIP_TRY(hipMemcpyAsync(s.d_in + s.off_ref, rp->plane2, b2, hipMemcpyHostToDevice, st));
        if (any_n) HIP_TRY(hipMemcpyAsync(s.d_in + s.off_ref + ref2_bytes(n_pos), rp->nplane, bn, hipMemcpyHostToDevice, st));
        if (!ring) HIP_TRY(hipEventRecord(s.ev_h2da, st));
        out->early = true;
        return ISX_OK;
    }

    uint8_t *h2 = s.h_in + s.off_ref, *hn = h2 + ref2_bytes(n_pos);
    s.ref_has_n = rp ? copy_ref_planes(*p->pool, rp, n_pos, h2, hn) : isxenc::pack_ref_planes(*p->pool, ref, n_pos, h2, hn);
    J.ref2 = h2; J.refn = s.ref_has_n ? hn : nullptr;
    out->host_ms = now_ms() - t_r;
    static const bool late_dma = getenv("ISX_PIPE_LATE_DMA") != nullptr;
    if (late_dma) return ISX_OK;
    if (!ring) HIP_TRY(hipEventRecord(s.ev_h2d0, st));
    HIP_TRY(hipMemcpyAsync(s.d_in + s.off_ref, h2, ref2_bytes(n_pos) + (s.ref_has_n ? refn_bytes(n_pos) : 0), hipMemcpyHostToDevice, st));
    if (!ring) HIP_TRY(hipEventRecord(s.ev_h2da, st));
    out->early = true;
    if (rp && rp->key) ref_cache_insert(p, s, rp, n_pos);
    return ISX_OK;
}

static int submit_common(isx_pipe *p, int64_t n_pos, const uint8_t *ref, int32_t n_splits, const int64_t *split_bounds,
                         int64_t n_obs, isxenc::EncodeJob &J, int64_t *ticket)
{
    static const char who[] = "isx_pipe_submit";
    int rc;
    if ((rc = check_capacity(p, who, n_pos, n_obs, p->pp.max_obs, n_splits)) != ISX_OK) return rc;
    if ((rc = check_split_bounds(n_pos, n_splits, split_bounds)) != ISX_OK) return rc;
    Slot *slot = nullptr;
    if ((rc = slot_acquire(p, who, &slot)) != ISX_OK) return rc;
    Slot &s = *slot;
    isx_batch *b = s.b;
    const bool linkage = p->prm.enable_linkage != 0;

    const double t0 = now_ms();
    const bool ring = p->ring_half > 0;
    uint8_t *d_rec = s.d_in + s.off_rec;
    RingFeed feed;
    J.n_obs = n_obs; J.n_pos = n_pos; J.record_bytes = p->rb;
    J.rec = s.h_in + s.off_rec; J.gbase = reinterpret_cast<uint32_t *>(s.h_in + s.off_gbase);
    J.pair_out = nullptr;
    J.cmin = s.cmin.data(); J.cmax = s.cmax.data(); J.cany = s.cany.data();
    J.cap_rec = p->cap_rec;
    if ((rc = ring_feed_install(p, s, feed, J.ring_groups, J.wave_begin, J.wave_flush)) != ISX_OK) return rc;
    int erc = 0;
    for (int attempt = 0;; attempt++) {
        if (linkage) {
            J.runs_out = s.h_runs; J.cap_runs = s.cap_runs;
            J.run_index_out = reinterpret_cast<uint32_t *>(s.h_in + s.off_ridx);
        }
        J.slack = p->slack;
        feed.bytes = 0;
        erc = isxenc::encode_obs(*p->pool, J);
        if (erc != isxenc::ENC_OK || !linkage || J.n_runs <= s.cap_runs || attempt == 1) break;
        HIP_TRY(isx_wait_stream(H2D(p, s)));
        host_block_free(s.h_runs, s.runs_pinned); s.h_runs = nullptr;
        isx_dev_free(s.d_runs); s.d_runs = nullptr;
        s.cap_runs = J.n_runs + J.n_runs / 4 + 4096;
        { const int hrc = host_block_alloc(reinterpret_cast<void **>(&s.h_runs), s.cap_runs * sizeof(isxenc::PairRun), s.runs_pinned); if (hrc != ISX_OK) return hrc; }
        HIP_TRY(isx_dev_malloc(reinterpret_cast<void **>(&s.d_runs), s.cap_runs * sizeof(uint2)));
    }
    const double t_enc = now_ms();
    if (feed.err != hipSuccess) { isx_set_error(std::string("isx_pipe_submit: staging ring: ") + hipGetErrorString(feed.err)); return ISX_ERR_HIP; }
    if (erc == isxenc::ENC_CAPACITY) { isx_set_error("isx_pipe_submit: the stream jumps too often for the pipe's record capacity (raise jump_slack)"); return ISX_ERR_CAPACITY; }
    if (erc == isxenc::ENC_MM_RANGE) { isx_set_error("an observation has mm >= 256"); return ISX_ERR_MM_RANGE; }
    if (erc == isxenc::ENC_BAD_POS) { isx_set_error("observation gpos >= n_pos"); return ISX_ERR_ARG; }
    if (linkage) {
        if (J.n_runs > s.cap_runs) { isx_set_error("isx_pipe_submit: internal: pair-id run table did not fit after growing it"); return ISX_ERR_STATE; }
        b->n_runs = (uint32_t)J.n_runs;
    }
    if (J.passes > 1 && J.n_groups_in > 0)
        p->slack = std::max(p->slack, 1.25 * ((double)J.n_groups_real / (double)J.n_groups_in - 1.0) + 0.01);
    s.ref_has_n = isxenc::pack_ref_planes(*p->pool, ref, n_pos, s.h_in + s.off_ref, s.h_in + s.off_ref + ref2_bytes(n_pos));
    memcpy(s.h_in + s.off_bounds, split_bounds, (size_t)(n_splits + 1) * sizeof(int64_t));

    b->n_pos = n_pos; b->n_obs = n_obs; b->n_splits = n_splits; b->n_rec = (uint64_t)J.n_rec;
    b->n_pairs = (uint64_t)J.max_pair + 1;
    if ((rc = slot_choose_windows(p, s, ISX_CHUNK, false)) != ISX_OK) return rc;
    if ((rc = slot_shape_pass(p, s)) != ISX_OK) return rc;
    slot_bind_inputs(p, s, nullptr);
    s.encode_ms = (float)(now_ms() - t0);
    s.encode_passes = J.passes;
    if (pipe_timing)
        fprintf(stderr, "[isx_pipe_submit] records %.2f ms (%d pass), reference + bounds + windows %.2f ms; %lld obs, %lld runs\n",
                t_enc - t0, J.passes, now_ms() - t_enc, (long long)n_obs, (long long)J.n_runs);

    if (!ring) HIP_TRY(hipEventRecord(s.ev_h2d0, H2D(p, s)));
    const size_t ref_bytes = ref2_bytes(n_pos) + (s.ref_has_n ? refn_bytes(n_pos) : 0);
    const size_t head = (size_t)(n_splits + 1) * sizeof(int64_t) + s.win.size() * sizeof(uint2) + ref_bytes;
    memset(s.h_in + s.off_gbase + (size_t)(b->n_rec / p->G) * sizeof(uint32_t), 0, ISX_TAIL_GROUPS * sizeof(uint32_t));
    const size_t gb_bytes = ((size_t)(b->n_rec / p->G) + ISX_TAIL_GROUPS) * sizeof(uint32_t), rec_bytes = (size_t)b->n_rec * p->rb + ISX_TAIL_BYTES;
    HIP_TRY(hipMemcpyAsync(s.d_in + s.off_bounds, s.h_in + s.off_bounds, (size_t)(n_splits + 1) * sizeof(int64_t), hipMemcpyHostToDevice, H2D(p, s)));
    HIP_TRY(hipMemcpyAsync(s.d_in + s.off_win, s.h_in + s.off_win, s.win.size() * sizeof(uint2), hipMemcpyHostToDevice, H2D(p, s)));
    HIP_TRY(hipMemcpyAsync(s.d_in + s.off_ref, s.h_in + s.off_ref, ref_bytes, hipMemcpyHostToDevice, H2D(p, s)));
    HIP_TRY(hipMemcpyAsync(s.d_in + s.off_gbase, s.h_in + s.off_gbase, gb_bytes, hipMemcpyHostToDevice, H2D(p, s)));
    if (ring) {
        if (p->rb == 2) HIP_TRY(hipMemsetD8Async(reinterpret_cast<hipDeviceptr_t>(d_rec + (size_t)b->n_rec * 2), 0xFF, ISX_TAIL_BYTES, H2D(p, s)));
        else HIP_TRY(hipMemsetD32Async(reinterpret_cast<hipDeviceptr_t>(d_rec + (size_t)b->n_rec * 4), (int)ISX_PAD32, ISX_TAIL_BYTES / 4, H2D(p, s)));
        if (feed.bytes != (size_t)b->n_rec * p->rb) { isx_set_error("internal: the staging ring did not carry the whole stream"); return ISX_ERR_STATE; }
    } else {
        if (p->rb == 2) memset(s.h_in + s.off_rec + (size_t)b->n_rec * 2, 0xFF, ISX_TAIL_BYTES);
        else std::fill_n(reinterpret_cast<uint32_t *>(s.h_in + s.off_rec + (size_t)b->n_rec * 4), ISX_TAIL_BYTES / 4, (uint32_t)ISX_PAD32);
        HIP_TRY(hipMemcpyAsync(d_rec, s.h_in + s.off_rec, rec_bytes, hipMemcpyHostToDevice, H2D(p, s)));
    }
    s.h2d_bytes = (int64_t)(head + gb_bytes + rec_bytes);
    if (linkage) {
        const size_t rb = (size_t)b->n_runs * sizeof(isxenc::PairRun), ib = (size_t)(b->n_rec / ISX_CHUNK) * sizeof(uint32_t);
        HIP_TRY(hipMemcpyAsync(s.d_runs, s.h_runs, rb, hipMemcpyHostToDevice, H2D(p, s)));
        HIP_TRY(hipMemcpyAsync(s.d_in + s.off_ridx, s.h_in + s.off_ridx, ib, hipMemcpyHostToDevice, H2D(p, s)));
        s.h2d_bytes += (int64_t)(rb + ib);
    }
    HIP_TRY(hipEventRecord(s.ev_h2d1, H2D(p, s)));
    s.h2d_split = false;

    return enqueue_pass(p, s, n_pos, ticket);
}

static int encode_reads(isx_pipe *p, Slot &s, isxenc::SegJob &J, bool planes_in, RingFeed &feed)
{
    s.encode_passes = 1;
    if (!p->drec) return isxenc::encode_segs(*p->pool, J);
    std::vector<int64_t> exact;
    for (int attempt = 0;; attempt++) {
        J.slack_groups = p->dslack;
        J.task_groups = exact.empty() ? nullptr : exact.data();
        feed.bytes = 0;
        const int erc = planes_in ? isxenc::encode_planes(*p->pool, J) : isxenc::encode_delta(*p->pool, J);
        if (erc != isxenc::SEG_CAPACITY || J.need_slack <= p->dslack || attempt != 0) return erc;
        exact = J.task_need;
        int64_t tot = 0;
        for (int64_t v : exact) tot += v;
        const int64_t n_t = (int64_t)exact.size(), base_tot = J.n_rec / ISX_DREC_GROUP - n_t * p->dslack;
        p->dslack = std::max<int64_t>(p->dslack, 1 + (tot - base_tot + n_t - 1) / std::max<int64_t>(n_t, 1));
        s.encode_passes = 2;
    }
}

static int submit_segs_common(isx_pipe *p, int64_t n_pos, const uint8_t *ref, int32_t n_splits, const int64_t *split_bounds,
                              isxenc::SegJob &J, int64_t *ticket, const isx_ref_planes *rp)
{
    static const char who[] = "isx_pipe_submit_reads";
    const bool planes_in = J.in2.planes != nullptr || (bool)J.produce_planes || (J.n_seg == 0 && rp != nullptr);
    int rc;
    if ((rc = check_capacity(p, who, n_pos, J.n_seg, p->pp.max_segs, n_splits)) != ISX_OK) return rc;
    if ((rc = check_split_bounds(n_pos, n_splits, split_bounds)) != ISX_OK) return rc;
    Slot *slot = nullptr;
    if ((rc = slot_acquire(p, who, &slot)) != ISX_OK) return rc;
    Slot &s = *slot;
    isx_batch *b = s.b;
    const bool linkage = p->prm.enable_linkage != 0;

    const double t0 = now_ms();
    J.n_pos = n_pos; J.n_mm_bins = b->M;
    J.rec = reinterpret_cast<uint32_t *>(s.h_in + s.off_rec);
    J.gbase = reinterpret_cast<uint32_t *>(s.h_in + s.off_gbase);
    J.pair_out = linkage && !p->drec ? reinterpret_cast<uint32_t *>(s.h_in + s.off_pairs) : nullptr;
    J.cmin = s.cmin.data(); J.cmax = s.cmax.data(); J.cany = s.cany.data();
    J.cap_rec = p->cap_rec;
    const bool ring = p->ring_half > 0;
    RingFeed feed;
    if ((rc = ring_feed_install(p, s, feed, J.ring_groups, J.wave_begin, J.wave_flush)) != ISX_OK) return rc;
    RefStage rs;
    if (planes_in) {
        if (!p->drec) { isx_set_error("bit-plane reads need a pipe whose batches travel as reference-delta records (one mm bin, or ISX_LAYOUT_MM_DELTA_RECORDS)"); return ISX_ERR_STATE; }
        if ((rc = stage_reference(p, s, n_pos, ref, rp, J, &rs)) != ISX_OK) return rc;
    }
    if (p->drec) J.ref = ref;
    const int erc = encode_reads(p, s, J, planes_in, feed);
    const double t_enc = now_ms();
    if (feed.err != hipSuccess) { isx_set_error(std::string("isx_pipe_submit_reads: staging ring: ") + hipGetErrorString(feed.err)); return ISX_ERR_HIP; }
    if ((rc = seg_status_error(erc, "isx_pipe_submit_reads: the stream jumps too often for the pipe's record capacity (raise jump_slack)", ISX_ERR_CAPACITY)) != ISX_OK) return rc;
    if (J.n_bases > p->pp.max_obs) { isx_set_error("isx_pipe_submit_reads: more bases than the pipe's max_obs"); return ISX_ERR_CAPACITY; }
    bool early_rec = false;
    if (rs.early && !ring) {
        const size_t gb_bytes0 = (size_t)(J.n_rec / (int64_t)p->G) * sizeof(uint32_t), rec_bytes0 = (size_t)J.n_rec * (size_t)p->rb;
        HIP_TRY(hipEventRecord(s.ev_h2db, H2D(p, s)));
        if (s.off_pairs == s.off_rec && s.off_ridx == s.off_rec && s.off_rec - s.off_gbase < ((size_t)2 << 20)) {
            HIP_TRY(hipMemcpyAsync(s.d_in + s.off_gbase, s.h_in + s.off_gbase, (s.off_rec - s.off_gbase) + rec_bytes0, hipMemcpyHostToDevice, H2D(p, s)));
        } else {
            HIP_TRY(hipMemcpyAsync(s.d_in + s.off_gbase, s.h_in + s.off_gbase, gb_bytes0, hipMemcpyHostToDevice, H2D(p, s)));
            HIP_TRY(hipMemcpyAsync(s.d_in + s.off_rec, s.h_in + s.off_rec, rec_bytes0, hipMemcpyHostToDevice, H2D(p, s)));
        }
        early_rec = true;
    }
    if (!planes_in) s.ref_has_n = isxenc::pack_ref_planes(*p->pool, ref, n_pos, s.h_in + s.off_ref, s.h_in + s.off_ref + ref2_bytes(n_pos));
    const double t_ref = now_ms();
    memcpy(s.h_in + s.off_bounds, split_bounds, (size_t)(n_splits + 1) * sizeof(int64_t));

    b->n_pos = n_pos; b->n_obs = J.n_bases; b->n_splits = n_splits; b->n_rec = (uint64_t)J.n_rec;
    b->n_pairs = (uint64_t)J.max_pair + 1;
    if ((rc = slot_choose_windows(p, s, p->G, true)) != ISX_OK) return rc;
    if ((rc = slot_shape_pass(p, s)) != ISX_OK) return rc;
    slot_bind_inputs(p, s, rs.resident);
    s.encode_ms = (float)(now_ms() - t0);
    if (pipe_timing)
        fprintf(stderr, "[isx_pipe_submit_reads] records %.2f ms, reference %.2f ms, bounds + windows %.2f ms; %lld segments, %lld records%s\n",
                t_enc - t0 - rs.host_ms, t_ref - t_enc + rs.host_ms, now_ms() - t_ref, (long long)J.n_seg, (long long)J.n_rec, planes_in ? " (bit planes)" : "");
    const double t_q0 = now_ms();

    if (!ring && !rs.early) HIP_TRY(hipEventRecord(s.ev_h2d0, H2D(p, s)));
    const size_t ref_bytes = ref2_bytes(n_pos) + (s.ref_has_n ? refn_bytes(n_pos) : 0);
    const size_t head = (size_t)(n_splits + 1) * sizeof(int64_t) + s.win.size() * sizeof(uint2) + ref_bytes;
    const size_t gb_bytes = (size_t)(b->n_rec / p->G) * sizeof(uint32_t), rec_bytes = (size_t)b->n_rec * (size_t)p->rb;
    if (s.off_win - s.off_bounds < ((size_t)1 << 20)) {
        HIP_TRY(hipMemcpyAsync(s.d_in + s.off_bounds, s.h_in + s.off_bounds, (s.off_win - s.off_bounds) + s.win.size() * sizeof(uint2), hipMemcpyHostToDevice, H2D(p, s)));
    } else {
        HIP_TRY(hipMemcpyAsync(s.d_in + s.off_bounds, s.h_in + s.off_bounds, (size_t)(n_splits + 1) * sizeof(int64_t), hipMemcpyHostToDevice, H2D(p, s)));
        HIP_TRY(hipMemcpyAsync(s.d_in + s.off_win, s.h_in + s.off_win, s.win.size() * sizeof(uint2), hipMemcpyHostToDevice, H2D(p, s)));
    }
    if (!rs.early) HIP_TRY(hipMemcpyAsync(s.d_in + s.off_ref, s.h_in + s.off_ref, ref_bytes, hipMemcpyHostToDevice, H2D(p, s)));
    if (!early_rec) HIP_TRY(hipMemcpyAsync(s.d_in + s.off_gbase, s.h_in + s.off_gbase, gb_bytes, hipMemcpyHostToDevice, H2D(p, s)));
    if (ring) { if (feed.bytes != rec_bytes) { isx_set_error("internal: the staging ring did not carry the whole stream"); return ISX_ERR_STATE; } }
    else if (!early_rec) HIP_TRY(hipMemcpyAsync(s.d_in + s.off_rec, s.h_in + s.off_rec, rec_bytes, hipMemcpyHostToDevice, H2D(p, s)));
    s.h2d_bytes = (int64_t)(head + gb_bytes + rec_bytes) - (rs.resident ? (int64_t)ref_bytes : 0);
    if (linkage && !p->drec) {
        HIP_TRY(hipMemcpyAsync(s.d_in + s.off_pairs, s.h_in + s.off_pairs, (size_t)b->n_rec * sizeof(uint32_t), hipMemcpyHostToDevice, H2D(p, s)));
        s.h2d_bytes += (int64_t)b->n_rec * 4;
    }
    HIP_TRY(hipEventRecord(s.ev_h2d1, H2D(p, s)));
    s.h2d_split = early_rec;
    const double t_q1 = now_ms();
    rc = enqueue_pass(p, s, n_pos, ticket);
    if (pipe_timing) fprintf(stderr, "[isx_pipe_submit_reads] copy-in queue %.2f ms, pass + copy-out queue %.2f ms\n", t_q1 - t_q0, now_ms() - t_q1);
    return rc;
}

struct isx_wire {
    isx_pipe *pipe = nullptr;
    uint8_t *h = nullptr;
    size_t bytes = 0;
    size_t o_bounds = 0, o_win = 0, o_ref = 0, o_gbase = 0, o_pairs = 0, o_rec = 0;
    size_t bounds_bytes = 0, win_bytes = 0, ref_bytes = 0, gbase_bytes = 0, pairs_bytes = 0, rec_bytes = 0;
    int64_t n_pos = 0, n_bases = 0, n_rec = 0, n_seg = 0;
    int32_t n_splits = 0;
    uint64_t n_pairs = 0;
    int W = 0, packed = 0;
    bool ref_has_n = false;
    float stage_ms = 0.f;
    int encode_passes = 1;
    uint8_t *d_ref = nullptr;
    int device = 0;
};

static int stage_common(isx_pipe *p, int64_t n_pos, const uint8_t *ref, const isx_ref_planes *rp, int32_t n_splits, const int64_t *split_bounds,
                        const isx_segs *segs, const isx_read_planes *reads, isx_wire **out)
{
    isx_segs as_segs{};
    if (reads) { as_segs.n_seg = reads->n_seg; as_segs.gpos = reads->gpos; as_segs.len = reads->len; as_segs.pair = reads->pair; segs = &as_segs; }
    *out = nullptr;
    if (!p->segs) { isx_set_error("isx_pipe_stage_reads: not a read-level pipe (isx_pipe_params.max_segs == 0)"); return ISX_ERR_STATE; }
    const bool linkage = p->prm.enable_linkage != 0;
    if (linkage && segs->n_seg && !segs->pair) { isx_set_error("linkage needs the pair array"); return ISX_ERR_ARG; }
    int rc;
    if ((rc = check_capacity(p, "isx_pipe_stage_reads", n_pos, segs->n_seg, p->pp.max_segs, n_splits)) != ISX_OK) return rc;
    if ((rc = check_split_bounds(n_pos, n_splits, split_bounds)) != ISX_OK) return rc;
    HIP_TRY(hipSetDevice(p->ctx->device));
    const double t0 = now_ms();
    std::unique_ptr<isx_wire, void (*)(isx_wire *)> w(new isx_wire(), isx_wire_free);
    w->pipe = p; w->n_pos = n_pos; w->n_splits = n_splits; w->n_seg = segs->n_seg;
    const isx_batch *b0 = p->slots[0].b;
    const int M = b0->M;
    const size_t G = p->G, rb = (size_t)p->rb;
    auto up = [](size_t v) { return (v + 255) & ~(size_t)255; };
    isxenc::SegJob J;
    std::vector<uint32_t> cmin, cmax;
    std::vector<uint8_t> cany;
    std::vector<int64_t> exact;
    for (int attempt = 0;; attempt++) {
        int64_t cap = p->drec ? isxenc::delta_groups_needed(*p->pool, segs->gpos, segs->n_seg, p->dslack) * ISX_DREC_GROUP
                              : isxenc::seg_groups_needed(*p->pool, segs->gpos, segs->n_seg) * ISX_SEG_GROUP;
        if (!exact.empty()) { cap = 0; for (int64_t v : exact) cap += std::max<int64_t>(v, 1) * ISX_DREC_GROUP; }
        if (cap > p->cap_rec) { isx_set_error("isx_pipe_stage_reads: the stream needs more records than the pipe's capacity (raise jump_slack)"); return ISX_ERR_CAPACITY; }
        const size_t n_groups = (size_t)cap / G;
        w->bounds_bytes = (size_t)(n_splits + 1) * sizeof(int64_t);
        w->ref_bytes = ref2_bytes(n_pos) + refn_bytes(n_pos);
        const size_t win_cap = ((size_t)n_pos / 64 + 2) * sizeof(uint2);
        size_t o = 0;
        w->o_bounds = o; o = up(o + w->bounds_bytes);
        w->o_win = o; o = up(o + win_cap);
        w->o_ref = o; o = up(o + w->ref_bytes);
        w->o_gbase = o; o = up(o + n_groups * sizeof(uint32_t));
        w->o_pairs = o; if (linkage && !p->drec) o = up(o + (size_t)cap * sizeof(uint32_t));
        w->o_rec = o; o = up(o + (size_t)cap * rb);
        if (w->h) { isx_pin_free(w->h); w->h = nullptr; }
        HIP_TRY(isx_pin_malloc(reinterpret_cast<void **>(&w->h), o));
        w->bytes = o;
        cmin.assign(n_groups + 2, 0xFFFFFFFFu); cmax.assign(n_groups + 2, 0u); cany.assign(n_groups + 2, 0);
        J = isxenc::SegJob();
        J.n_seg = segs->n_seg; J.n_pos = n_pos; J.n_mm_bins = M;
        if (reads) { J.in2 = *reads; if (!linkage) J.in2.pair = nullptr; }
        else { J.in = *segs; if (!linkage) J.in.pair = nullptr; }
        J.rec = reinterpret_cast<uint32_t *>(w->h + w->o_rec);
        J.gbase = reinterpret_cast<uint32_t *>(w->h + w->o_gbase);
        J.pair_out = linkage && !p->drec ? reinterpret_cast<uint32_t *>(w->h + w->o_pairs) : nullptr;
        J.cmin = cmin.data(); J.cmax = cmax.data(); J.cany = cany.data();
        J.cap_rec = cap;
        int erc;
        if (reads) {
            uint8_t *h2 = w->h + w->o_ref, *hn = h2 + ref2_bytes(n_pos);
            w->ref_has_n = rp ? copy_ref_planes(*p->pool, rp, n_pos, h2, hn) : isxenc::pack_ref_planes(*p->pool, ref, n_pos, h2, hn);
            J.ref2 = h2; J.refn = w->ref_has_n ? hn : nullptr;
        }
        if (p->drec) {
            J.ref = ref; J.slack_groups = p->dslack;
            J.task_groups = exact.empty() ? nullptr : exact.data();
            erc = reads ? isxenc::encode_planes(*p->pool, J) : isxenc::encode_delta(*p->pool, J);
            if (erc == isxenc::SEG_CAPACITY && J.need_slack > p->dslack && attempt == 0) { exact = J.task_need; w->encode_passes = 2; continue; }
        } else erc = isxenc::encode_segs(*p->pool, J);
        if ((rc = seg_status_error(erc, "isx_pipe_stage_reads: the stream does not fit the record capacity", ISX_ERR_CAPACITY)) != ISX_OK) return rc;
        break;
    }
    if (J.n_bases > p->pp.max_obs) { isx_set_error("isx_pipe_stage_reads: more bases than the pipe's max_obs"); return ISX_ERR_CAPACITY; }
    w->n_rec = J.n_rec; w->n_bases = J.n_bases; w->n_pairs = (uint64_t)J.max_pair + 1;
    w->gbase_bytes = (size_t)(J.n_rec / (int64_t)G) * sizeof(uint32_t);
    w->rec_bytes = (size_t)J.n_rec * rb;
    w->pairs_bytes = linkage && !p->drec ? (size_t)J.n_rec * sizeof(uint32_t) : 0;
    if (!reads) w->ref_has_n = isxenc::pack_ref_planes(*p->pool, ref, n_pos, w->h + w->o_ref, w->h + w->o_ref + ref2_bytes(n_pos));
    if (!w->ref_has_n) w->ref_bytes = ref2_bytes(n_pos);
    memcpy(w->h + w->o_bounds, split_bounds, w->bounds_bytes);
    {
        std::vector<uint2> win;
        std::vector<uint32_t> dir_pmax, dir_smin;
        DirThreads mt{*p->pool, dir_pmax, dir_smin};
        w->W = choose_windows(b0, n_pos, ChunkDir{cmin.data(), cmax.data(), cany.data(), (uint64_t)J.n_rec / G, (uint32_t)G}, &mt, win, &w->packed);
        w->win_bytes = win.size() * sizeof(uint2);
        if (w->win_bytes > ((size_t)n_pos / 64 + 2) * sizeof(uint2) || win.size() > (size_t)p->pp.max_pos / 64 + 2) { isx_set_error("internal: window directory larger than its region"); return ISX_ERR_STATE; }
        memcpy(w->h + w->o_win, win.data(), w->win_bytes);
    }
    w->stage_ms = (float)(now_ms() - t0);
    *out = w.release();
    return ISX_OK;
}

int isx_pipe_stage_reads(isx_pipe *p, int64_t n_pos, const uint8_t *ref, int32_t n_splits, const int64_t *split_bounds,
                         const isx_segs *segs, isx_wire **out)
{
    if (!p || !ref || !split_bounds || !out || n_pos <= 0 || n_splits <= 0 || !segs || segs->n_seg < 0 ||
        (segs->n_seg && (!segs->gpos || !segs->len || !segs->bases))) {
        isx_set_error("isx_pipe_stage_reads: bad argument");
        return ISX_ERR_ARG;
    }
    return stage_common(p, n_pos, ref, nullptr, n_splits, split_bounds, segs, nullptr, out);
}

int isx_pipe_stage_planes(isx_pipe *p, int64_t n_pos, const isx_ref_planes *ref, int32_t n_splits, const int64_t *split_bounds,
                          const isx_read_planes *reads, isx_wire **out)
{
    if (!p || !ref || !ref->plane2 || !split_bounds || !out || n_pos <= 0 || n_splits <= 0 || !reads || reads->n_seg < 0 ||
        (reads->n_seg && (!reads->gpos || !reads->len || !reads->planes))) {
        isx_set_error("isx_pipe_stage_planes: bad argument");
        return ISX_ERR_ARG;
    }
    if (!p->drec) { isx_set_error("isx_pipe_stage_planes: bit-plane reads need a read-level pipe with one mm bin or ISX_LAYOUT_MM_DELTA_RECORDS"); return ISX_ERR_STATE; }
    return stage_common(p, n_pos, nullptr, ref, n_splits, split_bounds, nullptr, reads, out);
}

void isx_wire_free(isx_wire *w)
{
    if (!w) return;
    if (w->h) isx_pin_free(w->h);
    if (w->d_ref) { (void)hipSetDevice(w->device); isx_dev_free(w->d_ref); }
    delete w;
}

int isx_wire_keep_reference(isx_pipe *p, isx_wire *w)
{
    if (!p || !w || w->pipe != p) { isx_set_error("isx_wire_keep_reference: bad argument"); return ISX_ERR_ARG; }
// ... 366 lines not shown
```

instrain_amd/csrc/seg_encode.cpp:

```cpp
#include "seg_encode.h"

#include <immintrin.h>

#include <algorithm>
#include <atomic>
#include <cstdlib>
#include <cstring>
#include <string>
#include <vector>

void isx_set_error(const std::string &msg);

namespace isxenc {

namespace {

constexpr int64_t TASK = 4096;
constexpr uint32_t SPAN = 65535u;

inline int64_t count_groups(const uint32_t *gpos, int64_t a, int64_t e, int64_t group = ISX_SEG_GROUP)
{
    int64_t n = 0;
    for (int64_t i = a; i < e;) {
        uint32_t lo = gpos[i], hi = gpos[i];
// ... 397 lines not shown
            nb += L;
            if (vbmi) cols_vbmi(bs + (size_t)s * ISX_SEG_WORDS, J.ref + p, L, C);
            else cols_scalar(bs + (size_t)s * ISX_SEG_WORDS, J.ref + p, L, C);
            if (J.n_mm_bins > 1) {
                C.exc[0] |= C.nbase[0]; C.exc[1] |= C.nbase[1]; C.exc[2] |= C.nbase[2];
            }
            const int n_exc = __builtin_popcountll(C.exc[0]) + __builtin_popcountll(C.exc[1]) + __builtin_popcountll(C.exc[2]);
            const bool plain = (C.skip[0] | C.skip[1] | C.skip[2]) == 0;
            if (n_exc == 0) {
                const uint32_t none[2] = {ISX_DREC_NO_EXC, ISX_DREC_NO_EXC};
                add_piece(p, L, pid, C.skip, none, plain, m);
                continue;
            }
            const uint32_t max_exc = plain ? ISX_DREC_EXC : ISX_DREC_EXC_FULL;
            uint64_t ex[3] = {C.exc[0], C.exc[1], C.exc[2]};
            uint32_t b = 0;
            while (b < L) {
                uint32_t f[ISX_DREC_EXC], nf = 0, end = L;
                for (int k = 0; k < 3; k++) {
                    while (ex[k]) {
                        const uint32_t col = (uint32_t)(64 * k + __builtin_ctzll(ex[k]));
                        if (nf == max_exc) { end = col; goto cut; }
                        ex[k] &= ex[k] - 1;
                        f[nf++] = ((col - b) & 0xFFu) | ((uint32_t)(C.code[col] & 3u) << 8);
                    }
                }
            cut:
                uint32_t w[2] = {ISX_DREC_NO_EXC, ISX_DREC_NO_EXC};
                for (uint32_t i = 0; i < nf; i++) {
                    const int wi = i / 3, sh = 10 * (int)(i % 3);
                    w[wi] = (w[wi] & ~(0x3FFu << sh)) | (f[i] << sh);
                }
                uint64_t msk[3];
                window160(C.skip, b, end - b, msk);
                add_piece(p + b, end - b, pid, msk, w, plain, m);
                b = end;
            }
        }
        close_group();
        need_of[(size_t)t] = used;
        for (; g < g_end; g++) {
            put_empty_group(rec_at(g));
            J.gbase[g] = 0; J.cmin[g] = 0xFFFFFFFFu; J.cmax[g] = 0; J.cany[g] = 0;
        }
        bases_of[(size_t)t] = nb; maxp_of[(size_t)t] = maxp; pieces_of[(size_t)t] = np;
    };
    if (!RG) pool.run(n_tasks, [&](int t) { run_task(t, 0, 0); });
    else {
        int half = 0;
        for (int t0 = 0; t0 < n_tasks && err.load() == SEG_OK;) {
            int t1 = t0 + 1;
            while (t1 < n_tasks && g_at[(size_t)t1 + 1] - g_at[(size_t)t0] <= RG) t1++;
            if (g_at[(size_t)t1] - g_at[(size_t)t0] > RG) return SEG_CAPACITY;
            J.wave_begin(half);
            const int64_t wg0 = g_at[(size_t)t0];
            pool.run(t1 - t0, [&](int k) { run_task(t0 + k, wg0, half); });
            if (err.load() == SEG_OK) J.wave_flush(half, wg0, g_at[(size_t)t1]);
            t0 = t1; half ^= 1;
        }
    }
    if (err.load() != SEG_OK) return err.load();
    J.n_bases = 0; J.max_pair = 0; J.n_pieces = 0;
    int64_t worst = 0;
    bool fits = true;
    J.task_need.assign(need_of.begin(), need_of.begin() + n_tasks);
    for (int t = 0; t < n_tasks; t++) {
        J.n_bases += bases_of[(size_t)t]; J.max_pair = std::max(J.max_pair, maxp_of[(size_t)t]); J.n_pieces += pieces_of[(size_t)t];
        const int64_t region = g_at[(size_t)t + 1] - g_at[(size_t)t];
        if (need_of[(size_t)t] > region) fits = false;
        worst = std::max(worst, need_of[(size_t)t] - (region - (J.task_groups ? 0 : slack)));
    }
    J.need_slack = fits ? slack : std::max<int64_t>(worst, slack + 1);
    if (!fits) return SEG_CAPACITY;
    return SEG_OK;
}


namespace {

struct LenMasks {
    alignas(32) uint64_t m[ISX_SEG_BASES + 1][4];
    LenMasks()
    {
        for (uint32_t L = 0; L <= ISX_SEG_BASES; L++)
            for (uint32_t k = 0; k < 4; k++) {
                const uint32_t from = 64 * k;
                m[L][k] = L <= from ? 0 : (L - from >= 64 ? ~(uint64_t)0 : (((uint64_t)1 << (L - from)) - 1));
            }
    }
};

inline bool cpu_has_bmi2()
{
    static const bool v = __builtin_cpu_supports("bmi2") && !getenv("ISX_NO_BMI2");
    return v;
}

inline uint64_t even_bits_portable(uint64_t x)
{
    x &= 0x5555555555555555ull;
    x = (x | (x >> 1)) & 0x3333333333333333ull;
    x = (x | (x >> 2)) & 0x0F0F0F0F0F0F0F0Full;
    x = (x | (x >> 4)) & 0x00FF00FF00FF00FFull;
    x = (x | (x >> 8)) & 0x0000FFFF0000FFFFull;
    x = (x | (x >> 16)) & 0x00000000FFFFFFFFull;
    return x;
}

inline void bits160(const uint8_t *q, uint32_t sh, uint64_t d[3])
{
    uint64_t w[4];
    memcpy(w, q, 32);
    for (int i = 0; i < 3; i++) d[i] = (w[i] >> sh) | ((w[i + 1] << 1) << (63 - sh));
}

struct PlaneTask {
    int64_t a, e;
    const uint32_t *gp, *pr, *gpos_all;
    const uint8_t *ln;
    const uint8_t *mm = nullptr;
    const uint64_t *pl;
    uint32_t *rec0;
    int64_t g0, ga, ge;
    bool fast_store;
    int64_t used = 0, np = 0, nb = 0;
    uint32_t maxp = 0;
};

inline void put_empty_drec(uint32_t *o)
{
    o[0] = o[1] = o[2] = o[4] = o[5] = o[6] = o[7] = 0;
    o[3] = ISX_DREC_NO_EXC;
}

#ifndef ISX_PLANES_PREFETCH
#define ISX_PLANES_PREFETCH 16
#endif
constexpr int64_t PLANES_PREFETCH = ISX_PLANES_PREFETCH;
struct PlaneGroup {
    alignas(64) uint32_t rec[ISX_DREC_GROUP][ISX_DREC_WORDS];
    int n = 0, open = -1;
    uint32_t lo = 0, hi = 0, last = 0;
    int64_t g = 0, used = 0;
};
__attribute__((noinline)) void rebase_drecs(PlaneGroup &G, uint32_t new_lo)
{
    const uint32_t up = G.lo - new_lo;
    for (int r = 0; r < G.n; r++) {
        uint32_t *o = G.rec[r];
        if ((o[0] >> 16) & 0xFFu) o[0] += up;
        if ((o[0] & ISX_DREC_DUAL) && ((o[4] >> 16) & 0xFFu)) o[4] += up;
    }
    G.lo = new_lo;
}

struct PlaneScratch {
    std::vector<uint32_t> gpos, pair;
    std::vector<uint8_t> len, mm;
    std::vector<uint64_t> planes;
    uint64_t *pl = nullptr;
};

#define ISX_PLANES_FN planes_task_portable
#define ISX_CLOSE_FN close_group_portable
#define ISX_DIFFERS_FN differs160_portable
#define ISX_PLANES_VARIANT 0
#include "seg_planes.inc"
#undef ISX_PLANES_FN
#undef ISX_CLOSE_FN
#undef ISX_DIFFERS_FN
#undef ISX_PLANES_VARIANT
#pragma GCC push_options
#pragma GCC target("bmi,bmi2,popcnt,lzcnt")
#define ISX_PLANES_FN planes_task_bmi2
#define ISX_CLOSE_FN close_group_bmi2
#define ISX_DIFFERS_FN differs160_bmi2
#define ISX_PLANES_VARIANT 1
#include "seg_planes.inc"
#undef ISX_PLANES_FN
#undef ISX_CLOSE_FN
#undef ISX_DIFFERS_FN
#undef ISX_PLANES_VARIANT
#pragma GCC pop_options
#pragma GCC push_options
#pragma GCC target("bmi,bmi2,popcnt,lzcnt,avx512f,avx512bw,avx512vl,avx512vbmi2,gfni")
#define ISX_PLANES_FN planes_task_avx512
#define ISX_CLOSE_FN close_group_avx512
#define ISX_DIFFERS_FN differs160_avx512
#define ISX_PLANES_VARIANT 2
#include "seg_planes.inc"
#undef ISX_PLANES_FN
#undef ISX_CLOSE_FN
#undef ISX_DIFFERS_FN
#undef ISX_PLANES_VARIANT
#pragma GCC pop_options

inline int planes_variant()
{
    static const int v = [] {
        if (const char *e = getenv("ISX_PLANES_VARIANT")) return std::max(0, std::min(2, atoi(e)));
        if (!cpu_has_bmi2()) return 0;
        return cpu_has_avx512() && __builtin_cpu_supports("avx512vbmi2") && __builtin_cpu_supports("gfni") ? 2 : 1;
    }();
    if (v == 2 && !(cpu_has_avx512() && __builtin_cpu_supports("avx512vbmi2") && __builtin_cpu_supports("gfni") && __builtin_cpu_supports("bmi2"))) return __builtin_cpu_supports("bmi2") ? 1 : 0;
    if (v == 1 && !__builtin_cpu_supports("bmi2")) return 0;
    return v;
}

}

int encode_planes(HostPool &pool, SegJob &J)
{
    const int64_t n = J.n_seg;
    const bool producer = (bool)J.produce_planes;
    const uint32_t *gpos_all = producer ? J.gpos_all : J.in2.gpos;
    const int n_tasks = (int)((n + TASK - 1) / TASK);
    const int64_t slack = std::max<int64_t>(J.slack_groups, 1);
    std::vector<int64_t> g_at((size_t)n_tasks + 1, 0);
    if (J.task_groups) for (int t = 0; t < n_tasks; t++) g_at[(size_t)t + 1] = std::max<int64_t>(J.task_groups[t], 1);
    else pool.run(n_tasks, [&](int t) {
        const int64_t a = (int64_t)t * TASK, e = std::min<int64_t>(n, a + TASK);
        g_at[(size_t)t + 1] = count_groups(gpos_all, a, e, 2 * ISX_DREC_GROUP) + slack;
    });
    for (int t = 0; t < n_tasks; t++) g_at[(size_t)t + 1] += g_at[(size_t)t];
    const int64_t n_groups = std::max<int64_t>(g_at[(size_t)n_tasks], 1);
    J.n_rec = n_groups * ISX_DREC_GROUP;
    J.need_slack = slack;
    if (J.n_rec > J.cap_rec) return SEG_CAPACITY;
    std::atomic<int> err{SEG_OK};
    std::vector<int64_t> bases_of((size_t)std::max(n_tasks, 1), 0), need_of((size_t)std::max(n_tasks, 1), 0), pieces_of((size_t)std::max(n_tasks, 1), 0);
    std::vector<uint32_t> maxp_of((size_t)std::max(n_tasks, 1), 0);
    const bool pairs = producer ? J.want_pairs : J.in2.pair != nullptr;
    const int64_t RG = J.ring_groups;
    constexpr size_t group_words = (size_t)ISX_DREC_GROUP * ISX_DREC_WORDS;
    const bool fast_store = cpu_has_avx512() && (reinterpret_cast<uintptr_t>(J.rec) & 63) == 0;
    const int variant = planes_variant();
    if (n == 0) {
        if (RG) J.wave_begin(0);
        for (int r = 0; r < ISX_DREC_GROUP; r++) put_empty_drec(J.rec + (size_t)r * ISX_DREC_WORDS);
        J.gbase[0] = 0; J.cmin[0] = 0xFFFFFFFFu; J.cmax[0] = 0; J.cany[0] = 0;
        J.n_bases = 0; J.max_pair = 0; J.n_pieces = 0;
        if (RG) J.wave_flush(0, 0, 1);
        return SEG_OK;
    }
    auto run_task = [&](int t, int64_t wave_g0, int half) {
        if (err.load(std::memory_order_relaxed) != SEG_OK) return;
        const int64_t a = (int64_t)t * TASK, e = std::min<int64_t>(n, a + TASK);
        const uint32_t *gp, *pr;
        const uint8_t *ln, *mmv = nullptr;
        const uint64_t *pl;
        if (producer) {
            thread_local PlaneScratch S;
            if (S.gpos.size() < (size_t)TASK) {
                S.gpos.resize((size_t)TASK); S.pair.resize((size_t)TASK); S.len.resize((size_t)TASK); S.mm.resize((size_t)TASK);
                S.planes.resize((size_t)TASK * ISX_PLANE_WORDS + 8);
                S.pl = reinterpret_cast<uint64_t *>((reinterpret_cast<uintptr_t>(S.planes.data()) + 63) & ~(uintptr_t)63);
            }
            J.produce_planes(a, e - a, S.gpos.data(), S.len.data(), J.n_mm_bins > 1 ? S.mm.data() : nullptr, pairs ? S.pair.data() : nullptr, S.pl);
            gp = S.gpos.data() - a; ln = S.len.data() - a; pr = pairs ? S.pair.data() - a : nullptr;
            if (J.n_mm_bins > 1) mmv = S.mm.data() - a;
            pl = S.pl - (size_t)a * ISX_PLANE_WORDS;
        } else {
            gp = J.in2.gpos; ln = J.in2.len; pr = pairs ? J.in2.pair : nullptr; pl = J.in2.planes;
            if (J.n_mm_bins > 1) mmv = J.in2.mm;
        }
        PlaneTask K;
        K.a = a; K.e = e; K.gp = gp; K.ln = ln; K.mm = mmv; K.pr = pr; K.pl = pl; K.gpos_all = gpos_all;
        K.rec0 = RG ? J.rec + (size_t)((int64_t)half * RG) * group_words : J.rec;
        K.g0 = RG ? wave_g0 : 0; K.ga = g_at[(size_t)t]; K.ge = g_at[(size_t)t + 1]; K.fast_store = fast_store;
        if (variant == 2) planes_task_avx512(J, err, K);
        else if (variant == 1) planes_task_bmi2(J, err, K);
        else planes_task_portable(J, err, K);
        if (err.load(std::memory_order_relaxed) != SEG_OK) return;
        need_of[(size_t)t] = K.used;
        bases_of[(size_t)t] = K.nb; maxp_of[(size_t)t] = K.maxp; pieces_of[(size_t)t] = K.np;
    };
    if (!RG) pool.run(n_tasks, [&](int t) { run_task(t, 0, 0); });
    else {
        int half = 0;
        for (int t0 = 0; t0 < n_tasks && err.load() == SEG_OK;) {
            int t1 = t0 + 1;
            while (t1 < n_tasks && g_at[(size_t)t1 + 1] - g_at[(size_t)t0] <= RG) t1++;
            if (g_at[(size_t)t1] - g_at[(size_t)t0] > RG) return SEG_CAPACITY;
            J.wave_begin(half);
            const int64_t wg0 = g_at[(size_t)t0];
            pool.run(t1 - t0, [&](int k) { run_task(t0 + k, wg0, half); });
            if (err.load() == SEG_OK) J.wave_flush(half, wg0, g_at[(size_t)t1]);
            t0 = t1; half ^= 1;
        }
    }
    if (err.load() != SEG_OK) return err.load();
    J.n_bases = 0; J.max_pair = 0; J.n_pieces = 0;
    int64_t worst = 0;
    bool fits = true;
    J.task_need.assign(need_of.begin(), need_of.begin() + n_tasks);
    for (int t = 0; t < n_tasks; t++) {
        J.n_bases += bases_of[(size_t)t]; J.max_pair = std::max(J.max_pair, maxp_of[(size_t)t]); J.n_pieces += pieces_of[(size_t)t];
        const int64_t region = g_at[(size_t)t + 1] - g_at[(size_t)t];
        if (need_of[(size_t)t] > region) fits = false;
        worst = std::max(worst, need_of[(size_t)t] - (region - (J.task_groups ? 0 : slack)));
    }
    J.need_slack = fits ? slack : std::max<int64_t>(worst, slack + 1);
    if (!fits) return SEG_CAPACITY;
    return SEG_OK;
}


namespace {
__attribute__((target("bmi2")))
inline void pack_ref_piece_bmi2(const uint8_t *r, int64_t n, uint8_t *o2, uint8_t *on, bool &seen)
{
    int64_t i = 0;
    uint64_t any = 0;
    for (; i + 8 <= n; i += 8) {
        uint64_t x;
        memcpy(&x, r + i, 8);
        const uint64_t bad = x & 0xFCFCFCFCFCFCFCFCull;
        if (__builtin_expect(bad == 0, 1)) {
            const uint16_t v = (uint16_t)_pext_u64(x, 0x0303030303030303ull);
            memcpy(o2 + (i >> 2), &v, 2);
            on[i >> 3] = 0;
            continue;
        }
        uint64_t t = bad | (bad >> 4);
        t |= t >> 2; t |= t >> 1;
        const uint64_t nb = t & 0x0101010101010101ull;
        const uint64_t keep = ~(nb * 0xFFull);
        const uint16_t v = (uint16_t)_pext_u64(x & keep, 0x0303030303030303ull);
        memcpy(o2 + (i >> 2), &v, 2);
        on[i >> 3] = (uint8_t)_pext_u64(nb, 0x0101010101010101ull);
        any |= nb;
    }
    for (; i < n; i += 8) {
        uint32_t lo = 0, hi = 0, nbits = 0;
        const int64_t m = std::min<int64_t>(8, n - i);
        for (int64_t k = 0; k < m; k++) {
            const uint32_t c = r[i + k];
            const uint32_t b = c > 3u;
            nbits |= b << k;
            const uint32_t v = b ? 0u : c;
            if (k < 4) lo |= v << (2 * k); else hi |= v << (2 * (k - 4));
        }
        o2[i >> 2] = (uint8_t)lo;
        if (m > 4) o2[(i >> 2) + 1] = (uint8_t)hi;
        on[i >> 3] = (uint8_t)nbits;
        any |= nbits;
    }
    seen = any != 0;
}

inline void pack_ref_piece_scalar(const uint8_t *r, int64_t n, uint8_t *o2, uint8_t *on, bool &seen)
{
    seen = false;
    for (int64_t i = 0; i < n; i += 8) {
        uint32_t lo = 0, hi = 0, nb = 0;
        const int64_t m = std::min<int64_t>(8, n - i);
        for (int64_t k = 0; k < m; k++) {
            const uint32_t c = r[i + k];
            const uint32_t bad = c > 3u;
            nb |= bad << k;
            const uint32_t v = bad ? 0u : c;
            if (k < 4) lo |= v << (2 * k); else hi |= v << (2 * (k - 4));
        }
        o2[i >> 2] = (uint8_t)lo;
        if (m > 4) o2[(i >> 2) + 1] = (uint8_t)hi;
        on[i >> 3] = (uint8_t)nb;
// ... 115 lines not shown

int isx_encode_delta(const isx_segs *segs, const uint8_t *ref, int64_t n_pos, int32_t n_mm_bins, int32_t host_threads, int32_t slack_groups,
                     int64_t cap_rec, int64_t ring_records, uint32_t *rec, uint32_t *gbase, uint32_t *pair_out, int64_t *n_rec, int64_t *need_slack)
{
    if (!segs || !ref || !rec || !gbase || !n_rec || segs->n_seg < 0 || cap_rec < ISX_DREC_GROUP || (cap_rec % ISX_DREC_GROUP) || n_pos <= 0 ||
        (segs->n_seg && (!segs->gpos || !segs->len || !segs->bases)) || ring_records < 0 ||
        (ring_records % (2 * ISX_DREC_GROUP)) || slack_groups < 0) {
        isx_set_error("isx_encode_delta: bad argument");
        return ISX_ERR_ARG;
    }
    std::vector<uint32_t> ring;
    isxenc::HostPool pool(std::max(1, host_threads), -1, false);
    std::vector<uint32_t> cmin((size_t)(cap_rec / ISX_DREC_GROUP)), cmax(cmin.size());
    std::vector<uint8_t> cany(cmin.size());
    isxenc::SegJob J;
    J.in = *segs; J.n_seg = segs->n_seg; J.n_pos = n_pos; J.n_mm_bins = std::max(1, n_mm_bins);
    J.ref = ref; J.slack_groups = std::max(1, slack_groups);
    (void)pair_out;
    J.rec = rec; J.gbase = gbase; J.pair_out = nullptr;
    J.cmin = cmin.data(); J.cmax = cmax.data(); J.cany = cany.data(); J.cap_rec = cap_rec;
    if (ring_records) {
        const int64_t half = ring_records / 2;
        ring.assign((size_t)ring_records * ISX_DREC_WORDS, 0xABABABABu);
        J.rec = ring.data();
        J.ring_groups = half / ISX_DREC_GROUP;
        J.wave_begin = [](int) {};
        J.wave_flush = [&](int h, int64_t g0, int64_t g1) {
            const size_t gw = (size_t)ISX_DREC_GROUP * ISX_DREC_WORDS;
            memcpy(rec + (size_t)g0 * gw, ring.data() + (size_t)h * half * ISX_DREC_WORDS, (size_t)(g1 - g0) * gw * 4);
            std::fill_n(ring.begin() + (ptrdiff_t)((size_t)h * half * ISX_DREC_WORDS), (size_t)half * ISX_DREC_WORDS, 0xABABABABu);
        };
    }
    const int rc = isxenc::encode_delta(pool, J);
    if (need_slack) *need_slack = J.need_slack;
    *n_rec = J.n_rec;
    if (rc == isxenc::SEG_CAPACITY) {
        isx_set_error(J.need_slack > J.slack_groups ? "isx_encode_delta: a task needs more spare groups than slack_groups (see *need_slack)"
                                                    : "isx_encode_delta: the stream does not fit cap_rec records");
        return ISX_ERR_CAPACITY;
    }
    if (rc == isxenc::SEG_MM_RANGE) { isx_set_error("a segment has mm >= n_mm_bins"); return ISX_ERR_MM_RANGE; }
    if (rc == isxenc::SEG_BAD_POS) { isx_set_error("a segment reaches beyond n_pos"); return ISX_ERR_ARG; }
    if (rc == isxenc::SEG_BAD_LEN) { isx_set_error("a segment's length is not in [1, 150]"); return ISX_ERR_ARG; }
    return ISX_OK;
}

int64_t isx_delta_records_needed(const uint32_t *gpos, int64_t n_seg, int32_t host_threads, int32_t slack_groups)
{
    if (n_seg < 0 || (n_seg && !gpos) || slack_groups < 0) return -1;
    isxenc::HostPool pool(std::max(1, host_threads), -1, false);
    return isxenc::delta_groups_needed(pool, gpos, n_seg, std::max(1, slack_groups)) * ISX_DREC_GROUP;
}

int64_t isx_seg_records_needed(const uint32_t *gpos, int64_t n_seg, int32_t host_threads)
{
    if (n_seg < 0 || (n_seg && !gpos)) return -1;
    isxenc::HostPool pool(std::max(1, host_threads), -1, false);
    return isxenc::seg_groups_needed(pool, gpos, n_seg) * ISX_SEG_GROUP;
}

int isx_count_read_segs(int64_t n_reads, const uint32_t *cigar, const int64_t *cigar_off, const int64_t *ref_start,
                        const int64_t *clip_lo, const int64_t *clip_hi, int64_t *n_seg)
{
    if (n_reads < 0 || !n_seg || (n_reads && (!cigar || !cigar_off || !ref_start || !clip_lo || !clip_hi))) {
        isx_set_error("isx_count_read_segs: bad argument");
        return ISX_ERR_ARG;
    }
    int64_t n = 0;
    for (int64_t r = 0; r < n_reads; r++) {
        const bool ok = for_runs(cigar + cigar_off[r], cigar_off[r + 1] - cigar_off[r], ref_start[r], clip_lo[r], clip_hi[r],
                                 [&](int64_t, int64_t, int64_t cols) { n += (cols + ISX_SEG_BASES - 1) / ISX_SEG_BASES; });
        if (!ok) { isx_set_error("isx_count_read_segs: unknown CIGAR operator"); return ISX_ERR_ARG; }
    }
    *n_seg = n;
    return ISX_OK;
}

int isx_pack_reads(int64_t n_reads, const int64_t *ref_start, const int64_t *clip_lo, const int64_t *clip_hi,
                   const uint32_t *cigar, const int64_t *cigar_off, const char *seq, const uint8_t *qual, const int64_t *seq_off,
                   const uint8_t *mm, const uint32_t *pair, int32_t min_base_quality, int64_t cap_seg, uint32_t *seg_gpos,
                   uint8_t *seg_len, uint8_t *seg_mm, uint32_t *seg_pair, uint32_t *seg_bases, int64_t *n_seg)
{
    if (n_reads < 0 || !n_seg || cap_seg < 0 || (n_reads && (!ref_start || !clip_lo || !clip_hi || !cigar || !cigar_off || !seq || !qual || !seq_off)) ||
        (cap_seg && (!seg_gpos || !seg_len || !seg_bases)) || (pair && cap_seg && !seg_pair)) {
        isx_set_error("isx_pack_reads: bad argument");
        return ISX_ERR_ARG;
    }
    int64_t n = 0;
    bool full = false, bad = false;
    for (int64_t r = 0; r < n_reads && !full && !bad; r++) {
        const char *sq = seq + seq_off[r];
        const uint8_t *ql = qual + seq_off[r];
        const int64_t q_len = seq_off[r + 1] - seq_off[r];
        const bool ok = for_runs(cigar + cigar_off[r], cigar_off[r + 1] - cigar_off[r], ref_start[r], clip_lo[r], clip_hi[r],
                                 [&](int64_t pos, int64_t q0, int64_t cols) {
            if (q0 + cols > q_len || pos < 0 || pos + cols > (int64_t)0xFFFFFFFFll) { bad = true; return; }
            for (int64_t c0 = 0; c0 < cols && !full; c0 += ISX_SEG_BASES) {
                const int L = (int)std::min<int64_t>(ISX_SEG_BASES, cols - c0);
                if (n >= cap_seg) { full = true; return; }
                uint32_t *w = seg_bases + (size_t)n * ISX_SEG_WORDS;
                for (int k = 0; k < ISX_SEG_WORDS; k++) w[k] = ISX_SEG_SKIP_WORD;
                for (int j = 0; j < L; j++) {
                    const int64_t qi = q0 + c0 + j;
                    const uint32_t code = (int)ql[qi] >= min_base_quality ? ascii_code(sq[qi]) : 4u;
                    w[j / 10] = (w[j / 10] & ~(7u << (3 * (j % 10)))) | (code << (3 * (j % 10)));
                }
                seg_gpos[n] = (uint32_t)(pos + c0); seg_len[n] = (uint8_t)L;
                if (seg_mm) seg_mm[n] = mm ? mm[r] : (uint8_t)0;
                if (seg_pair) seg_pair[n] = pair ? pair[r] : 0u;
                n++;
            }
        });
        if (!ok) { isx_set_error("isx_pack_reads: unknown CIGAR operator"); return ISX_ERR_ARG; }
    }
    if (bad) { isx_set_error("isx_pack_reads: a CIGAR reaches beyond its read's bases or the flat space"); return ISX_ERR_ARG; }
    if (full) { isx_set_error("isx_pack_reads: more segments than cap_seg (isx_count_read_segs gives the number)"); return ISX_ERR_CAPACITY; }
    *n_seg = n;
    return ISX_OK;
}

int isx_pack_ref_planes(const uint8_t *ref, int64_t n_pos, int32_t host_threads, uint8_t *plane2, uint8_t *nplane, int32_t *has_n)
{
    if (!ref || n_pos <= 0 || !plane2 || !nplane) { isx_set_error("isx_pack_ref_planes: bad argument"); return ISX_ERR_ARG; }
    isxenc::HostPool pool(std::max(1, host_threads), -1, false);
    const bool any = isxenc::pack_ref_planes(pool, ref, n_pos, plane2, nplane);
    if (has_n) *has_n = any ? 1 : 0;
    return ISX_OK;
}

int isx_planes_from_segs(const isx_segs *segs, int32_t host_threads, uint64_t *planes)
{
    if (!segs || segs->n_seg < 0 || (segs->n_seg && (!segs->len || !segs->bases || !planes))) { isx_set_error("isx_planes_from_segs: bad argument"); return ISX_ERR_ARG; }
    const int64_t n = segs->n_seg, piece = 8192;
    std::atomic<bool> bad{false};
    isxenc::HostPool pool(std::max(1, host_threads), -1, false);
    pool.run((int)((n + piece - 1) / piece), [&](int t) {
        const int64_t a = (int64_t)t * piece, e = std::min<int64_t>(n, a + piece);
        for (int64_t i = a; i < e; i++) {
            const uint32_t L = segs->len[i];
            if (L == 0 || L > ISX_SEG_BASES) { bad.store(true); return; }
            isxenc::planes_from_words(segs->bases + (size_t)i * ISX_SEG_WORDS, L, planes + (size_t)i * ISX_PLANE_WORDS);
        }
    });
    if (bad.load()) { isx_set_error("a segment's length is not in [1, 150]"); return ISX_ERR_ARG; }
    return ISX_OK;
}

int isx_encode_planes(const isx_read_planes *reads, const isx_ref_planes *ref, int64_t n_pos, int32_t host_threads, int32_t slack_groups,
                      int64_t cap_rec, int64_t ring_records, uint32_t *rec, uint32_t *gbase, int64_t *n_rec, int64_t *need_slack)
{
    return isx_encode_planes_mm(reads, ref, n_pos, 1, host_threads, slack_groups, cap_rec, ring_records, rec, gbase, n_rec, need_slack);
}

int isx_encode_planes_mm(const isx_read_planes *reads, const isx_ref_planes *ref, int64_t n_pos, int32_t n_mm_bins, int32_t host_threads, int32_t slack_groups,
                         int64_t cap_rec, int64_t ring_records, uint32_t *rec, uint32_t *gbase, int64_t *n_rec, int64_t *need_slack)
{
    if (n_mm_bins < 1 || n_mm_bins > 128) { isx_set_error("isx_encode_planes: n_mm_bins must be in [1, 128]"); return ISX_ERR_ARG; }
    if (!reads || !ref || !ref->plane2 || !rec || !gbase || !n_rec || reads->n_seg < 0 || cap_rec < ISX_DREC_GROUP || (cap_rec % ISX_DREC_GROUP) || n_pos <= 0 ||
        (reads->n_seg && (!reads->gpos || !reads->len || !reads->planes)) || ring_records < 0 ||
        (ring_records % (2 * ISX_DREC_GROUP)) || slack_groups < 0) {
        isx_set_error("isx_encode_planes: bad argument");
        return ISX_ERR_ARG;
    }
    std::vector<uint32_t> ring;
    isxenc::HostPool pool(std::max(1, host_threads), -1, false);
    std::vector<uint32_t> cmin((size_t)(cap_rec / ISX_DREC_GROUP)), cmax(cmin.size());
    std::vector<uint8_t> cany(cmin.size());
    isxenc::SegJob J;
    J.in2 = *reads; J.n_seg = reads->n_seg; J.n_pos = n_pos; J.n_mm_bins = n_mm_bins;
    J.ref2 = ref->plane2; J.refn = ref->nplane; J.slack_groups = std::max(1, slack_groups);
    J.rec = rec; J.gbase = gbase; J.pair_out = nullptr;
    J.cmin = cmin.data(); J.cmax = cmax.data(); J.cany = cany.data(); J.cap_rec = cap_rec;
    if (ring_records) {
        const int64_t half = ring_records / 2;
        ring.assign((size_t)ring_records * ISX_DREC_WORDS + 16, 0xABABABABu);
        uint32_t *r0 = reinterpret_cast<uint32_t *>((reinterpret_cast<uintptr_t>(ring.data()) + 63) & ~(uintptr_t)63);
        J.rec = r0;
        J.ring_groups = half / ISX_DREC_GROUP;
        J.wave_begin = [](int) {};
        J.wave_flush = [&, r0](int h, int64_t g0, int64_t g1) {
            const size_t gw = (size_t)ISX_DREC_GROUP * ISX_DREC_WORDS;
            memcpy(rec + (size_t)g0 * gw, r0 + (size_t)h * half * ISX_DREC_WORDS, (size_t)(g1 - g0) * gw * 4);
            std::fill_n(r0 + (size_t)h * half * ISX_DREC_WORDS, (size_t)half * ISX_DREC_WORDS, 0xABABABABu);
        };
    }
    const int rc = isxenc::encode_planes(pool, J);
    if (need_slack) *need_slack = J.need_slack;
    *n_rec = J.n_rec;
    if (rc == isxenc::SEG_CAPACITY) {
        isx_set_error(J.need_slack > J.slack_groups ? "isx_encode_planes: a task needs more spare groups than slack_groups (see *need_slack)"
                                                    : "isx_encode_planes: the stream does not fit cap_rec records");
        return ISX_ERR_CAPACITY;
    }
    if (rc == isxenc::SEG_BAD_POS) { isx_set_error("a segment reaches beyond n_pos"); return ISX_ERR_ARG; }
    if (rc == isxenc::SEG_BAD_LEN) { isx_set_error("a segment's length is not in [1, 150]"); return ISX_ERR_ARG; }
    if (rc == isxenc::SEG_MM_RANGE) { isx_set_error("a segment has mm >= n_mm_bins"); return ISX_ERR_MM_RANGE; }
    return ISX_OK;
}

int isx_pack_read_planes(int64_t n_reads, const int64_t *ref_start, const int64_t *clip_lo, const int64_t *clip_hi,
                         const uint32_t *cigar, const int64_t *cigar_off, const char *seq, const uint8_t *qual, const int64_t *seq_off,
                         const uint32_t *pair, int32_t min_base_quality, int64_t cap_seg, uint32_t *seg_gpos,
                         uint8_t *seg_len, uint32_t *seg_pair, uint64_t *seg_planes, int64_t *n_seg)
{
    if (n_reads < 0 || !n_seg || cap_seg < 0 || (n_reads && (!ref_start || !clip_lo || !clip_hi || !cigar || !cigar_off || !seq || !qual || !seq_off)) ||
        (cap_seg && (!seg_gpos || !seg_len || !seg_planes)) || (pair && cap_seg && !seg_pair)) {
        isx_set_error("isx_pack_read_planes: bad argument");
        return ISX_ERR_ARG;
    }
    int64_t n = 0;
    bool full = false, bad = false;
    for (int64_t r = 0; r < n_reads && !full && !bad; r++) {
        const char *sq = seq + seq_off[r];
        const uint8_t *ql = qual + seq_off[r];
        const int64_t q_len = seq_off[r + 1] - seq_off[r];
        const bool ok = for_runs(cigar + cigar_off[r], cigar_off[r + 1] - cigar_off[r], ref_start[r], clip_lo[r], clip_hi[r],
                                 [&](int64_t pos, int64_t q0, int64_t cols) {
            if (q0 + cols > q_len || pos < 0 || pos + cols > (int64_t)0xFFFFFFFFll) { bad = true; return; }
            for (int64_t c0 = 0; c0 < cols && !full; c0 += ISX_SEG_BASES) {
                const int L = (int)std::min<int64_t>(ISX_SEG_BASES, cols - c0);
                if (n >= cap_seg) { full = true; return; }
                uint64_t *P = seg_planes + (size_t)n * ISX_PLANE_WORDS;
                for (int k = 0; k < ISX_PLANE_WORDS; k++) P[k] = 0;
                for (int j = 0; j < L; j++) {
                    const int64_t qi = q0 + c0 + j;
                    const uint32_t code = (int)ql[qi] >= min_base_quality ? ascii_code(sq[qi]) : 4u;
                    if (code >= 4) {
                        P[5 + (j >> 6)] |= (uint64_t)1 << (j & 63);
                        if (code == 5) { P[j >> 5] |= (uint64_t)1 << (2 * (j & 31)); P[7] |= (uint64_t)1 << 63; }
                    } else P[j >> 5] |= (uint64_t)code << (2 * (j & 31));
                }
                seg_gpos[n] = (uint32_t)(pos + c0); seg_len[n] = (uint8_t)L;
                if (seg_pair) seg_pair[n] = pair ? pair[r] : 0u;
                n++;
            }
        });
        if (!ok) { isx_set_error("isx_pack_read_planes: unknown CIGAR operator"); return ISX_ERR_ARG; }
    }
    if (bad) { isx_set_error("isx_pack_read_planes: a CIGAR reaches beyond its read's bases or the flat space"); return ISX_ERR_ARG; }
    if (full) { isx_set_error("isx_pack_read_planes: more segments than cap_seg (isx_count_read_segs gives the number)"); return ISX_ERR_CAPACITY; }
    *n_seg = n;
    return ISX_OK;
}

}
```

instrain_amd/csrc/seg_encode.h:

```cpp
#pragma once
#include <stdint.h>

#include <functional>
#include <vector>

#include "../../include/instrain_amd.h"
#include "obs_encode.h"

#define ISX_SEG_GROUP 16
#define ISX_SEG_REC_WORDS 16
#define ISX_DREC_GROUP 32

namespace isxenc {

struct SegJob {
    isx_segs in{};
    std::function<void(int64_t first, int64_t count, uint32_t *gpos, uint8_t *len, uint8_t *mm, uint32_t *pair, uint32_t *bases)> produce;
    const uint32_t *gpos_all = nullptr;
    isx_read_planes in2{};
    std::function<void(int64_t first, int64_t count, uint32_t *gpos, uint8_t *len, uint8_t *mm, uint32_t *pair, uint64_t *planes)> produce_planes;
    const uint8_t *ref2 = nullptr, *refn = nullptr;
    int64_t n_seg = 0, n_pos = 0;
    int n_mm_bins = 1;
    bool want_pairs = false;
    uint32_t *rec = nullptr;
    uint32_t *gbase = nullptr;
    uint32_t *pair_out = nullptr;
    uint32_t *cmin = nullptr, *cmax = nullptr;
    uint8_t *cany = nullptr;
    int64_t cap_rec = 0;
    int64_t ring_groups = 0;
    std::function<void(int half)> wave_begin;
    std::function<void(int half, int64_t g0, int64_t g1)> wave_flush;
    const uint8_t *ref = nullptr;
    int64_t slack_groups = 1;
    int64_t need_slack = 0;
    std::vector<int64_t> task_need;
    const int64_t *task_groups = nullptr;
    int64_t n_pieces = 0;
    int64_t n_rec = 0;
    int64_t n_bases = 0;
    uint32_t max_pair = 0;
};

enum { SEG_OK = 0, SEG_CAPACITY = 1, SEG_MM_RANGE = 2, SEG_BAD_POS = 3, SEG_BAD_LEN = 4 };

int encode_segs(HostPool &pool, SegJob &job);
int encode_delta(HostPool &pool, SegJob &job);
int encode_planes(HostPool &pool, SegJob &job);
int64_t delta_groups_needed(HostPool &pool, const uint32_t *gpos, int64_t n, int64_t slack_groups);
int64_t seg_groups_needed(HostPool &pool, const uint32_t *gpos, int64_t n);
bool pack_ref_planes(HostPool &pool, const uint8_t *ref, int64_t n_pos, uint8_t *plane2, uint8_t *nplane);
void planes_from_words(const uint32_t *words, uint32_t len, uint64_t *planes);

}
```

instrain_amd/csrc/seg_planes.inc:

```

#if ISX_PLANES_VARIANT == 2
static inline __attribute__((always_inline)) __m256i ISX_DIFFERS_FN(const uint8_t *q, uint32_t sh, __m512i P)
{
    const __m512i lo = _mm512_maskz_loadu_epi64((__mmask8)0x1F, q), hi = _mm512_maskz_loadu_epi64((__mmask8)0x1F, q + 8);
    const __m512i r = _mm512_shrdv_epi64(lo, hi, _mm512_set1_epi64((long long)sh));
    const __m512i x = _mm512_xor_si512(r, P);
    const __m512i m = _mm512_or_si512(x, _mm512_srli_epi64(x, 1));
    const __m512i nib = _mm512_gf2p8affine_epi64_epi8(m, _mm512_set1_epi64((long long)0x0104104000000000ull), 0);
    const __m512i t = _mm512_or_si512(nib, _mm512_srli_epi16(nib, 4));
    return _mm512_cvtepi16_epi8(t);
}
#else
static inline __attribute__((always_inline)) void ISX_DIFFERS_FN(const uint8_t *q, uint32_t sh, const uint64_t *P, uint64_t d[3])
{
    uint64_t w[6];
    memcpy(w, q, 48);
    uint64_t e[5];
    for (int i = 0; i < 5; i++) {
        const uint64_t r = (w[i] >> sh) | ((w[i + 1] << 1) << (63 - sh));
        const uint64_t x = r ^ P[i];
        const uint64_t m = x | (x >> 1);
#if ISX_PLANES_VARIANT == 1
        e[i] = _pext_u64(m, 0x5555555555555555ull);
#else
        e[i] = even_bits_portable(m);
#endif
    }
    d[0] = e[0] | (e[1] << 32);
    d[1] = e[2] | (e[3] << 32);
    d[2] = e[4];
}
#endif

static __attribute__((noinline)) void ISX_CLOSE_FN(SegJob &J, const PlaneTask &K, PlaneGroup &G)
{
    if (!G.n) return;
    if (G.g < K.ge) {
        for (int r = G.n; r < ISX_DREC_GROUP; r++) put_empty_drec(G.rec[r]);
        uint32_t *o = K.rec0 + (size_t)(G.g - K.g0) * (size_t)ISX_DREC_GROUP * ISX_DREC_WORDS;
        if (!K.fast_store) memcpy(o, G.rec, sizeof G.rec);
        else {
#if ISX_PLANES_VARIANT == 2
            for (int r = 0; r < ISX_DREC_GROUP; r += 2) _mm512_stream_si512(reinterpret_cast<__m512i *>(o + (size_t)r * ISX_DREC_WORDS), _mm512_load_si512(G.rec[r]));
#else
            const __m128i *src = reinterpret_cast<const __m128i *>(G.rec);
            __m128i *dst = reinterpret_cast<__m128i *>(o);
            for (int i = 0; i < ISX_DREC_GROUP * ISX_DREC_WORDS / 4; i++) _mm_stream_si128(dst + i, _mm_load_si128(src + i));
#endif
        }
        J.gbase[G.g] = G.lo; J.cmin[G.g] = G.lo; J.cmax[G.g] = G.last; J.cany[G.g] = 1;
        G.g++;
    }
    G.used++;
    G.n = 0; G.open = -1;
}

#if ISX_PLANES_VARIANT == 0
#define ISX_TZ64(x) ((x) ? (uint32_t)__builtin_ctzll(x) : 64u)
#else
#define ISX_TZ64(x) ((uint32_t)_tzcnt_u64(x))
#endif
static void ISX_PLANES_FN(SegJob &J, std::atomic<int> &err, PlaneTask &K)
{
    static const LenMasks LM;
    PlaneGroup G;
    G.g = K.ga;
    const uint8_t *const ref2 = J.ref2, *const refn = J.refn;
    const int64_t n_pos = J.n_pos;
    const int64_t safe_pos = n_pos - 200;
    const uint32_t *const gp = K.gp, *const pr = K.pr, *const ga = K.gpos_all;
    const uint8_t *const ln = K.ln;
    int64_t nb = 0, np = 0;
    uint32_t maxp = 0;
    auto place = [&](uint32_t start, uint32_t len, bool plain, bool &fill) __attribute__((always_inline)) -> uint32_t * {
        fill = plain && G.open >= 0;
        if (G.n) {
            const uint32_t nlo = std::min(G.lo, start), nhi = std::max(G.hi, start);
            if (__builtin_expect(nhi - nlo > SPAN || (!fill && G.n == ISX_DREC_GROUP), 0)) { ISX_CLOSE_FN(J, K, G); fill = false; }
        }
        if (!G.n) { G.lo = G.hi = start; G.last = start + len - 1; }
        else {
            if (__builtin_expect(start < G.lo, 0)) rebase_drecs(G, start);
            G.hi = std::max(G.hi, start); G.last = std::max(G.last, start + len - 1);
        }
        np++;
        if (fill) { uint32_t *o = G.rec[G.open] + 4; G.open = -1; return o; }
        uint32_t *o = G.rec[G.n];
        G.open = plain ? G.n : -1;
        G.n++;
        return o;
    };
    uint32_t hdr_hi = 0;
    auto add_full = [&](uint32_t start, uint32_t len, uint32_t pid, uint64_t s0, uint64_t s1, uint64_t s2, uint32_t exc) __attribute__((always_inline)) {
        bool fill;
        uint32_t *o = place(start, len, false, fill);
        const uint64_t v0 = (uint64_t)((start - G.lo) | (len << 16) | hdr_hi) | (s0 << 32), v1 = (s0 >> 32) | ((uint64_t)exc << 32);
        const uint64_t v3 = (s2 & 0xFFFFFFFFull) | ((uint64_t)pid << 32);
        memcpy(o, &v0, 8); memcpy(o + 2, &v1, 8); memcpy(o + 4, &s1, 8); memcpy(o + 6, &v3, 8);
    };
    auto add_plain = [&](uint32_t start, uint32_t len, uint32_t pid, uint32_t exc0, uint32_t exc1) __attribute__((always_inline)) {
        bool fill;
        uint32_t *o = place(start, len, true, fill);
        const uint64_t v0 = (uint64_t)((start - G.lo) | (len << 16) | hdr_hi | ISX_DREC_DUAL) | ((uint64_t)pid << 32), v1 = (uint64_t)exc0 | ((uint64_t)exc1 << 32);
        memcpy(o, &v0, 8); memcpy(o + 2, &v1, 8);
        if (!fill) {
            const uint64_t v2 = (uint64_t)ISX_DREC_DUAL, v3 = (uint64_t)ISX_DREC_NO_EXC | ((uint64_t)ISX_DREC_NO_EXC << 32);
            memcpy(o + 4, &v2, 8); memcpy(o + 6, &v3, 8);
        }
    };
#if ISX_PLANES_VARIANT == 2
    const __m256i rec_idx = _mm256_setr_epi32(8, 0, 1, 8, 2, 3, 4, 8);
#endif
    const bool mm_on = J.n_mm_bins > 1;
    const int64_t pf_end = K.e - PLANES_PREFETCH;
    for (int64_t s = K.a; s < K.e; s++) {
        const uint32_t L = ln[s], p = gp[s];
        const uint64_t *P = K.pl + (size_t)s * ISX_PLANE_WORDS;
        if (s < pf_end) {
            _mm_prefetch(reinterpret_cast<const char *>(P + (size_t)PLANES_PREFETCH * ISX_PLANE_WORDS), _MM_HINT_T0);
            _mm_prefetch(reinterpret_cast<const char *>(ref2 + (gp[s + PLANES_PREFETCH] >> 2) + 40), _MM_HINT_T0);
        }
        if (__builtin_expect(L == 0 || L > ISX_SEG_BASES, 0)) { err.store(SEG_BAD_LEN); return; }
        if (__builtin_expect((int64_t)p + (int64_t)L > n_pos || p != ga[s], 0)) { err.store(SEG_BAD_POS); return; }
        const uint32_t pid = pr ? pr[s] : 0u;
        maxp = pid > maxp ? pid : maxp;
        nb += L;
        const uint64_t *lm = LM.m[L];
        uint64_t s0, s1, s2, ex[3];
        bool n_marked = false;
        if (mm_on) {
            const uint32_t mv = K.mm ? K.mm[s] : 0u;
            if (__builtin_expect((int)mv >= J.n_mm_bins || mv > 127u, 0)) { err.store(SEG_MM_RANGE); return; }
            hdr_hi = mv << 24;
            n_marked = (P[7] >> 63) != 0;
        }
#if ISX_PLANES_VARIANT == 2
        __m256i skv = _mm256_setzero_si256();
        const bool in_regs = (int64_t)p < safe_pos && !refn && !n_marked;
        if (__builtin_expect(in_regs, 1)) {
            const __m512i Pv = _mm512_loadu_si512(P);
            const __m256i lmv = _mm256_loadu_si256(reinterpret_cast<const __m256i *>(lm));
            skv = _mm256_and_si256(_mm256_maskz_loadu_epi64((__mmask8)0x7, P + 5), lmv);
            const __m256i dv = ISX_DIFFERS_FN(ref2 + (p >> 2), (p & 3u) * 2u, Pv);
            const __m256i exv = _mm256_and_si256(dv, _mm256_xor_si256(skv, lmv));
            alignas(32) uint64_t t[8];
            _mm256_store_si256(reinterpret_cast<__m256i *>(t), skv);
            _mm256_store_si256(reinterpret_cast<__m256i *>(t + 4), exv);
            s0 = t[0]; s1 = t[1]; s2 = t[2];
            ex[0] = t[4]; ex[1] = t[5]; ex[2] = t[6];
        } else
#endif
        {
            s0 = P[5] & lm[0]; s1 = P[6] & lm[1]; s2 = P[7] & lm[2];
            uint64_t d[3];
#if ISX_PLANES_VARIANT == 2
            alignas(32) uint64_t dq[4];
#define ISX_DIFFERS_AT(q_, sh_) do { _mm256_store_si256(reinterpret_cast<__m256i *>(dq), ISX_DIFFERS_FN((q_), (sh_), _mm512_loadu_si512(P))); d[0] = dq[0]; d[1] = dq[1]; d[2] = dq[2]; } while (0)
#else
#define ISX_DIFFERS_AT(q_, sh_) ISX_DIFFERS_FN((q_), (sh_), P, d)
#endif
            if (__builtin_expect((int64_t)p < safe_pos, 1)) {
                ISX_DIFFERS_AT(ref2 + (p >> 2), (p & 3u) * 2u);
                if (refn) {
                    uint64_t nn[3];
                    if (__builtin_expect((int64_t)p + 264 <= n_pos, 1)) bits160(refn + (p >> 3), p & 7u, nn);
                    else {
                        uint8_t bn[32] = {0};
                        const int64_t haven = (n_pos + 7) / 8 - (int64_t)(p >> 3);
                        memcpy(bn, refn + (p >> 3), (size_t)std::min<int64_t>(32, haven));
                        bits160(bn, p & 7u, nn);
                    }
                    d[0] |= nn[0]; d[1] |= nn[1]; d[2] |= nn[2];
                }
            } else {
                alignas(64) uint8_t buf[64] = {0};
                const int64_t have2 = (n_pos + 3) / 4 - (int64_t)(p >> 2);
                memcpy(buf, ref2 + (p >> 2), (size_t)std::min<int64_t>(48, have2));
                ISX_DIFFERS_AT(buf, (p & 3u) * 2u);
                if (refn) {
                    uint8_t bn[32] = {0};
                    const int64_t haven = (n_pos + 7) / 8 - (int64_t)(p >> 3);
                    memcpy(bn, refn + (p >> 3), (size_t)std::min<int64_t>(32, haven));
                    uint64_t nn[3];
                    bits160(bn, p & 7u, nn);
                    d[0] |= nn[0]; d[1] |= nn[1]; d[2] |= nn[2];
                }
            }
#undef ISX_DIFFERS_AT
            ex[0] = d[0] & (lm[0] ^ s0); ex[1] = d[1] & (lm[1] ^ s1); ex[2] = d[2] & (lm[2] ^ s2);
            if (__builtin_expect(n_marked, 0)) {
                ex[0] |= (even_bits_portable(P[0]) | (even_bits_portable(P[1]) << 32)) & s0;
                ex[1] |= (even_bits_portable(P[2]) | (even_bits_portable(P[3]) << 32)) & s1;
                ex[2] |= even_bits_portable(P[4]) & s2;
            }
        }
        const bool plain = (s0 | s1 | s2) == 0;
        const uint32_t n_exc = (uint32_t)(__builtin_popcountll(ex[0]) + __builtin_popcountll(ex[1]) + __builtin_popcountll(ex[2]));
        if (__builtin_expect(n_exc <= 1, 1)) {
            const uint32_t t0 = ISX_TZ64(ex[0]), t1 = ISX_TZ64(ex[1]), t2 = ISX_TZ64(ex[2] | ((uint64_t)1 << 63));
            const uint32_t m0 = 0u - (uint32_t)(ex[0] == 0), m01 = m0 & (0u - (uint32_t)(ex[1] == 0));
            const uint32_t col = t0 + (t1 & m0) + (t2 & m01);
            const uint32_t code = (uint32_t)(P[col >> 5] >> (2 * (col & 31u))) & 3u;
            const uint32_t w0 = 0x3FFFFC00u | ((col | (code << 8) | (0u - (uint32_t)(n_exc == 0))) & 0x3FFu);
            if (__builtin_expect(plain, 0)) { add_plain(p, L, pid, w0, ISX_DREC_NO_EXC); continue; }
#if ISX_PLANES_VARIANT == 2
            if (__builtin_expect(in_regs, 1)) {
                bool fill;
                uint32_t *o = place(p, L, false, fill);
                __m256i v = _mm256_permutex2var_epi32(skv, rec_idx, _mm256_set1_epi32((int)w0));
                v = _mm256_mask_set1_epi32(v, (__mmask8)0x01, (int)((p - G.lo) | (L << 16) | hdr_hi));
                v = _mm256_mask_set1_epi32(v, (__mmask8)0x80, (int)pid);
                _mm256_store_si256(reinterpret_cast<__m256i *>(o), v);
                continue;
            }
#endif
            add_full(p, L, pid, s0, s1, s2, w0);
            continue;
        }
        const uint32_t max_exc = plain ? ISX_DREC_EXC : ISX_DREC_EXC_FULL;
        if (__builtin_expect(n_exc <= max_exc, 1)) {
            uint64_t fields = 0;
            for (uint32_t i = 0; i < n_exc; i++) {
                const int k = ex[0] ? 0 : (ex[1] ? 1 : 2);
                const uint32_t col = (uint32_t)(64 * k + __builtin_ctzll(ex[k]));
                ex[k] &= ex[k] - 1;
                const uint64_t code = (P[col >> 5] >> (2 * (col & 31u))) & 3u;
                fields |= ((uint64_t)col | (code << 8)) << (10 * i);
            }
            const uint64_t all = (fields | (0x0FFFFFFFFFFFFFFFull << (10 * n_exc))) & 0x0FFFFFFFFFFFFFFFull;
            const uint32_t w0 = (uint32_t)all & ISX_DREC_NO_EXC, w1 = (uint32_t)(all >> 30) & ISX_DREC_NO_EXC;
            if (plain) add_plain(p, L, pid, w0, w1);
            else add_full(p, L, pid, s0, s1, s2, w0);
            continue;
        }
        const uint64_t sk[3] = {s0, s1, s2};
        uint32_t b = 0;
        while (b < L) {
            uint32_t w[2] = {ISX_DREC_NO_EXC, ISX_DREC_NO_EXC};
            uint32_t nf = 0, end = L;
            for (int k = 0; k < 3; k++) {
                while (ex[k]) {
                    const uint32_t col = (uint32_t)(64 * k + __builtin_ctzll(ex[k]));
                    if (nf == max_exc) { end = col; goto cut; }
                    ex[k] &= ex[k] - 1;
                    const uint32_t code = (uint32_t)(P[col >> 5] >> (2 * (col & 31u))) & 3u;
                    const uint32_t f = ((col - b) & 0xFFu) | (code << 8);
                    const int wi = (int)(nf / 3), shf = 10 * (int)(nf % 3);
                    w[wi] = (w[wi] & ~(0x3FFu << shf)) | (f << shf);
                    nf++;
                }
            }
        cut:
            if (plain) add_plain(p + b, end - b, pid, w[0], w[1]);
            else if (b == 0 && end == L) add_full(p, L, pid, s0, s1, s2, w[0]);
            else {
                uint64_t msk[3];
                window160(sk, b, end - b, msk);
                add_full(p + b, end - b, pid, msk[0], msk[1], msk[2], w[0]);
            }
            b = end;
        }
    }
    ISX_CLOSE_FN(J, K, G);
    for (; G.g < K.ge; G.g++) {
        uint32_t *o = K.rec0 + (size_t)(G.g - K.g0) * (size_t)ISX_DREC_GROUP * ISX_DREC_WORDS;
        for (int r = 0; r < ISX_DREC_GROUP; r++) put_empty_drec(o + (size_t)r * ISX_DREC_WORDS);
        J.gbase[G.g] = 0; J.cmin[G.g] = 0xFFFFFFFFu; J.cmax[G.g] = 0; J.cany[G.g] = 0;
    }
    if (K.fast_store) _mm_sfence();
    K.used = G.used; K.np = np; K.nb = nb; K.maxp = maxp;
}
#undef ISX_TZ64
```

instrain_amd/engine.py:

```python
import ctypes as C
import os

import numpy as np

from . import _lib
from ._lib import (ENTRY_DT, LD_DT, OBS_DT, SNV_DT, BamInfo, BamParams, IsxError, Params, Sizes,
                   Timings, check)


def pack_obs(gpos, base, mm):
    o = np.empty(len(gpos), dtype=OBS_DT)
    o["gpos"] = gpos
    o["mm"] = mm
    o["base"] = base
    o["flags"] = 0
    return o


class SegBatch:

    def __init__(self, gpos, length, bases, mm=None, pair=None):
        self.gpos = np.ascontiguousarray(gpos, dtype=np.uint32)
        self.len = np.ascontiguousarray(length, dtype=np.uint8)
        self.bases = np.ascontiguousarray(bases, dtype=np.uint32).reshape(-1, _lib.SEG_WORDS)
# ... 607 lines not shown


def _par_copy(a):
    global _COPY_POOL
    if a.nbytes < (8 << 20):
        return a.copy()
    if _COPY_POOL is None:
        from concurrent.futures import ThreadPoolExecutor
        _COPY_POOL = ThreadPoolExecutor(6)
    out = np.empty_like(a)
    n = len(a)
    step = -(-n // 12)
    list(_COPY_POOL.map(lambda k: np.copyto(out[k:k + step], a[k:k + step]), range(0, n, step)))
    return out


class LevelTables:

    def __init__(self, lib, r):
        self.lib = lib
        n_pos, n_lev, n_win = int(r.n_pos), int(r.n_lev), int(r.n_lev_windows)

        def own(addr, dtype, n):
            if not n or not addr:
                return np.empty(0, dtype=dtype)
            return _par_copy(np.frombuffer((C.c_uint8 * (n * np.dtype(dtype).itemsize)).from_address(addr), dtype=dtype))

        self.mask = own(r.lev_mask, {1: np.uint8, 2: np.uint16, 4: np.uint32}[int(r.lev_mask_bytes)], n_pos)
        self.cov = own(r.lev_cov, np.uint8 if r.lev_cov_bytes == 1 else np.uint16, n_lev)
        self.win_off = own(r.lev_win_off, np.uint32, n_win)
        self.clon = own(r.lev_clon, _lib.RARE_DT, int(r.n_lev_clon))
        self.rare = own(r.lev_rare, _lib.RARE_DT, int(r.n_lev_rare))
        self.sat = own(r.lev_sat, _lib.SAT_DT, int(r.n_lev_sat))
        q = _lib.PipeResult()
        q.n_pos, q.n_lev, q.n_lev_clon, q.n_lev_rare, q.n_lev_sat = n_pos, n_lev, len(self.clon), len(self.rare), len(self.sat)
        q.lev_mask_bytes, q.lev_cov_bytes, q.lev_window, q.n_lev_windows, q.lev_min_cov = r.lev_mask_bytes, r.lev_cov_bytes, r.lev_window, r.n_lev_windows, r.lev_min_cov
        ptr = lambda a: a.ctypes.data if len(a) else None
        q.lev_mask, q.lev_cov, q.lev_win_off = ptr(self.mask), ptr(self.cov) or ptr(self.win_off), ptr(self.win_off)
        q.lev_clon, q.lev_rare, q.lev_sat = ptr(self.clon), ptr(self.rare), ptr(self.sat)
        self._r = q
        self._cols = None
        self.n = n_lev

    def columns(self, threads=0):
        if self._cols is None:
            n = max(1, self.n)
            cols = [np.empty(n, np.uint32), np.empty(n, np.uint32), np.empty(n, np.float32), np.empty(n, np.float32) if len(self.rare) else None]
            check(self.lib.isx_levels_expand(C.byref(self._r), int(threads) or min(16, len(os.sched_getaffinity(0))), *(c.ctypes.data if c is not None else None for c in cols)))
            if cols[3] is None:
                cols[3] = np.broadcast_to(np.float32(np.nan), (n,))
            self._cols = tuple(c[:self.n] for c in cols)
        return self._cols


class Wire:

    def __init__(self, pipe, h):
        self.lib, self.h, self.pipe_h = pipe.lib, h, pipe.h
        self.bytes = int(self.lib.isx_wire_bytes(h))

    def keep_reference(self):
        check(self.lib.isx_wire_keep_reference(self.pipe_h, self.h))
        self.bytes = int(self.lib.isx_wire_bytes(self.h))

    def close(self):
        h, self.h = self.h, None
        if h:
            self.lib.isx_wire_free(h)

    def __del__(self):
        pass


def encode_obs(obs, pair=None, n_pos=None, record_bytes=2, threads=1, slack=0.0, cap_rec=None, ring_records=0):
    lib = _lib.load()
    obs = np.ascontiguousarray(obs, dtype=OBS_DT)
    G = 512 if record_bytes == 2 else 256
    if cap_rec is None:
        cap_rec = (int(len(obs) * 1.5) + 4 * 2048 + 2047) // 2048 * 2048
    if n_pos is None:
        n_pos = int(obs["gpos"].max()) + 1 if len(obs) else 1
    rec = np.empty(cap_rec, dtype=np.uint16 if record_bytes == 2 else np.uint32)
    gbase = np.empty(cap_rec // G, dtype=np.uint32)
    pout = np.empty(cap_rec, dtype=np.uint32) if pair is not None else None
    if pair is not None:
        pair = np.ascontiguousarray(pair, dtype=np.uint32)
    n_rec, passes = C.c_int64(0), C.c_int32(0)
    check(lib.isx_encode_obs_ring(obs.ctypes.data if len(obs) else None, pair.ctypes.data if pair is not None else None, len(obs),
                                  int(n_pos), int(record_bytes), int(threads), float(slack), int(cap_rec), int(ring_records),
                                  rec.ctypes.data, gbase.ctypes.data, pout.ctypes.data if pout is not None else None,
                                  C.byref(n_rec), C.byref(passes)))
    n = n_rec.value
    return rec[:n], gbase[:n // G], (pout[:n] if pout is not None else None), passes.value


def dense_clon(cov, clon_sparse, min_cov):
    out = np.where(np.asarray(cov) >= min_cov, np.float32(1.0), np.float32(np.nan)).astype(np.float32)
    out[clon_sparse["gpos"]] = clon_sparse["clon"]
    return out


def encode_segs(segs, n_pos, n_mm_bins=1, threads=1, cap_rec=None, ring_records=0):
    lib = _lib.load()
    if cap_rec is None:
        cap_rec = int(lib.isx_seg_records_needed(segs.gpos.ctypes.data if segs.n_seg else None, segs.n_seg, int(threads)))
    rec = np.empty((cap_rec, 16), dtype=np.uint32)
    gbase = np.empty(cap_rec // 16, dtype=np.uint32)
    pout = np.empty(cap_rec, dtype=np.uint32) if segs.pair is not None else None
    n_rec = C.c_int64(0)
    cs = segs.c()
    check(lib.isx_encode_segs_ring(C.byref(cs), int(n_pos), int(n_mm_bins), int(threads), int(cap_rec), int(ring_records), rec.ctypes.data,
                                   gbase.ctypes.data, pout.ctypes.data if pout is not None else None, C.byref(n_rec)))
    n = n_rec.value
    return rec[:n], gbase[:n // 16], (pout[:n] if pout is not None else None)


def encode_delta(segs, ref_codes, n_mm_bins=1, threads=1, slack_groups=1, cap_rec=None, ring_records=0, retry=True):
    lib = _lib.load()
    ref = np.ascontiguousarray(ref_codes, dtype=np.uint8)
    while True:
        cap = cap_rec if cap_rec is not None else int(lib.isx_delta_records_needed(segs.gpos.ctypes.data if segs.n_seg else None, segs.n_seg, int(threads), int(slack_groups)))
        rec = np.empty((cap, 8), dtype=np.uint32)
        gbase = np.empty(cap // 32, dtype=np.uint32)
        n_rec, need = C.c_int64(0), C.c_int64(0)
        cs = segs.c()
        rc = lib.isx_encode_delta(C.byref(cs), ref.ctypes.data, len(ref), int(n_mm_bins), int(threads), int(slack_groups), cap, int(ring_records),
                                  rec.ctypes.data, gbase.ctypes.data, None, C.byref(n_rec), C.byref(need))
        if rc == _lib.ERR_CAPACITY and retry and need.value > slack_groups and cap_rec is None:
            slack_groups = int(need.value)
            continue
        check(rc)
        n = n_rec.value
        return rec[:n], gbase[:n // 32], None, slack_groups


def encode_planes(reads, ref_planes, threads=1, slack_groups=1, cap_rec=None, ring_records=0, retry=True, n_mm_bins=1):
    lib = _lib.load()
    while True:
        cap = cap_rec if cap_rec is not None else int(lib.isx_delta_records_needed(reads.gpos.ctypes.data if reads.n_seg else None, reads.n_seg, int(threads), int(slack_groups)))
        rec = _aligned((cap, 8), np.uint32)
        gbase = np.empty(cap // 32, dtype=np.uint32)
        n_rec, need = C.c_int64(0), C.c_int64(0)
        cr, cf = reads.c(), ref_planes.c()
        rc = lib.isx_encode_planes_mm(C.byref(cr), C.byref(cf), ref_planes.n_pos, int(n_mm_bins), int(threads), int(slack_groups), cap, int(ring_records),
                                      rec.ctypes.data, gbase.ctypes.data, C.byref(n_rec), C.byref(need))
        if rc == _lib.ERR_CAPACITY and retry and need.value > slack_groups and cap_rec is None:
            slack_groups = int(need.value)
            continue
        check(rc)
        n = n_rec.value
        return rec[:n], gbase[:n // 32], None, slack_groups


def dense_cov(res, n_pos=None):
    if "cov16" in res:
        return res["cov16"]
    if "cov8" in res:
        cov = res["cov8"].astype(np.uint16)
    else:
        nib = res["cov4"]
        n_pos = 2 * len(nib) if n_pos is None else int(n_pos)
        cov = np.empty(2 * len(nib), dtype=np.uint16)
        cov[0::2] = nib & 15
        cov[1::2] = nib >> 4
        cov = cov[:n_pos]
        W = int(res["cov_window"])
        for k, w in enumerate(res["cov_row_win"].tolist()):
            lo = w * W
            hi = min(lo + W, n_pos)
            cov[lo:hi] = res["cov_rows"][k, :hi - lo]
    if "saturated" in res:
        cov[res["saturated"]["gpos"]] = np.minimum(res["saturated"]["coverage"], 65535)
    return cov


DREC_DUAL = 0x80000000
DREC_NO_EXC = 0x3FFFFFFF


def decode_delta(rec, gbase, ref_codes):
    rec = np.asarray(rec, dtype=np.uint32).reshape(-1, 8)
    ref = np.asarray(ref_codes, dtype=np.uint8)
    n = len(rec)
    dual = (rec[:, 0] >> 31) == 1
    assert ((rec[dual, 4] >> 31) == 1).all(), "a dual record's second half carries the flag too"
    zero = np.zeros(n, dtype=np.uint32)
    none = np.full(n, DREC_NO_EXC, dtype=np.uint32)
    hdr = np.stack([rec[:, 0], np.where(dual, rec[:, 4], zero)], axis=1)
    pair = np.stack([np.where(dual, rec[:, 1], rec[:, 7]), np.where(dual, rec[:, 5], zero)], axis=1)
    e0 = np.stack([np.where(dual, rec[:, 2], rec[:, 3]), np.where(dual, rec[:, 6], none)], axis=1)
    e1 = np.stack([np.where(dual, rec[:, 3], none), np.where(dual, rec[:, 7], none)], axis=1)
    skw = [np.stack([np.where(dual, zero, rec[:, k]), zero], axis=1) for k in (1, 2, 4, 5, 6)]
    gb = np.repeat(np.asarray(gbase, dtype=np.uint32), 32)[:n]
    start = (gb[:, None] + (hdr & 0xFFFF)).astype(np.int64)
    ln = ((hdr >> 16) & 0xFF).astype(np.int64)
    lvl = ((hdr >> 24) & 0x7F).astype(np.uint8)
    full = np.stack([~dual, np.zeros(n, dtype=bool)], axis=1)
    real = (ln > 0).reshape(-1)
    flat = lambda x: x.reshape(-1)[real]
    st, ln, pr, e0, e1, fl, lvl = flat(start), flat(ln), flat(pair), flat(e0), flat(e1), flat(full), flat(lvl)
    words = np.stack([flat(w) for w in skw], axis=1)
    m = len(st)
    j = np.arange(160, dtype=np.int64)[None, :]
    skip = ((words[:, :, None] >> np.arange(32, dtype=np.uint32)[None, None, :]) & 1).reshape(m, 160).astype(bool)
    assert not (skip & (j >= ln[:, None])).any(), "skip bits beyond a piece's length"
    assert skip[fl].any(axis=1).all() or True
    inside = j < ln[:, None]
    pos = np.minimum(st[:, None] + j, len(ref) - 1)
    codes = np.where(inside & ~skip, ref[pos], 4).astype(np.uint8)
    for e in (e0, e1):
        for k in range(3):
            f = (e >> (10 * k)) & 0x3FF
            has = f != 0x3FF
            off, base = (f & 0xFF).astype(np.int64), ((f >> 8) & 3).astype(np.uint8)
            rows = np.flatnonzero(has)
            assert (off[rows] < ln[rows]).all()
            mark = skip[rows, off[rows]]
            assert fl[rows[mark]].all(), "a non-ACGT marker in a dual half"
            codes[rows[mark], off[rows[mark]]] = 5
            rows = rows[~mark]
            assert (base[rows] != ref[st[rows] + off[rows]]).all(), "an exception that equals the reference"
            codes[rows, off[rows]] = base[rows]
        assert ((e >> 30) == 0).all()
    return st.astype(np.uint32), ln.astype(np.uint8), lvl, codes[:, :150], pr, fl


def decode_segs(rec, gbase):
    rec = np.asarray(rec, dtype=np.uint32).reshape(-1, 16)
    hdr = rec[:, 0]
    ln = (hdr >> 16) & 0xFF
    real = ln > 0
    start = np.repeat(np.asarray(gbase, dtype=np.uint32), 16)[:len(rec)] + (hdr & 0xFFFF)
    return start[real], ln[real].astype(np.uint8), (hdr[real] >> 24).astype(np.uint8), unpack_codes(rec[real, 1:])


def pack_reads(ref_start, clip_lo, clip_hi, cigars, seqs, quals, mm=None, pair=None, min_base_quality=30):
    lib = _lib.load()
    n = len(ref_start)
    rs = np.ascontiguousarray(ref_start, dtype=np.int64)
    lo = np.ascontiguousarray(clip_lo, dtype=np.int64)
    hi = np.ascontiguousarray(clip_hi, dtype=np.int64)
    cig_off = np.zeros(n + 1, dtype=np.int64)
    seq_off = np.zeros(n + 1, dtype=np.int64)
    if n:
        cig_off[1:] = np.cumsum([len(c) for c in cigars])
        seq_off[1:] = np.cumsum([len(q) for q in quals])
    cig = np.ascontiguousarray(np.concatenate([np.asarray(c, dtype=np.uint32) for c in cigars]) if n else np.zeros(0, np.uint32))
    seq = b"".join(s.encode() if isinstance(s, str) else bytes(s) for s in seqs)
    qual = np.ascontiguousarray(np.concatenate([np.asarray(q, dtype=np.uint8) for q in quals]) if n else np.zeros(0, np.uint8))
    assert len(seq) == len(qual)
    mmv = None if mm is None else np.ascontiguousarray(mm, dtype=np.uint8)
    pv = None if pair is None else np.ascontiguousarray(pair, dtype=np.uint32)
    ns = C.c_int64(0)
    check(lib.isx_count_read_segs(n, cig.ctypes.data, cig_off.ctypes.data, rs.ctypes.data, lo.ctypes.data, hi.ctypes.data, C.byref(ns)))
    cap = max(1, ns.value)
    g = np.empty(cap, np.uint32); ln = np.empty(cap, np.uint8); sm = np.zeros(cap, np.uint8); sp = np.zeros(cap, np.uint32)
    bs = np.empty((cap, _lib.SEG_WORDS), np.uint32)
    check(lib.isx_pack_reads(n, rs.ctypes.data, lo.ctypes.data, hi.ctypes.data, cig.ctypes.data, cig_off.ctypes.data, seq,
                             qual.ctypes.data, seq_off.ctypes.data, mmv.ctypes.data if mmv is not None else None,
                             pv.ctypes.data if pv is not None else None, int(min_base_quality), cap, g.ctypes.data, ln.ctypes.data,
                             sm.ctypes.data, sp.ctypes.data, bs.ctypes.data, C.byref(ns)))
    k = ns.value
    return SegBatch(g[:k], ln[:k], bs[:k], sm[:k] if mm is not None else None, sp[:k] if pair is not None else None)


def pack_read_planes(ref_start, clip_lo, clip_hi, cigars, seqs, quals, pair=None, min_base_quality=30):
    lib = _lib.load()
    n = len(ref_start)
    rs = np.ascontiguousarray(ref_start, dtype=np.int64)
    lo = np.ascontiguousarray(clip_lo, dtype=np.int64)
    hi = np.ascontiguousarray(clip_hi, dtype=np.int64)
    cig_off = np.zeros(n + 1, dtype=np.int64)
    seq_off = np.zeros(n + 1, dtype=np.int64)
    if n:
        cig_off[1:] = np.cumsum([len(c) for c in cigars])
        seq_off[1:] = np.cumsum([len(q) for q in quals])
    cig = np.ascontiguousarray(np.concatenate([np.asarray(c, dtype=np.uint32) for c in cigars]) if n else np.zeros(0, np.uint32))
    seq = b"".join(s.encode() if isinstance(s, str) else bytes(s) for s in seqs)
    qual = np.ascontiguousarray(np.concatenate([np.asarray(q, dtype=np.uint8) for q in quals]) if n else np.zeros(0, np.uint8))
    assert len(seq) == len(qual)
    pv = None if pair is None else np.ascontiguousarray(pair, dtype=np.uint32)
    ns = C.c_int64(0)
    check(lib.isx_count_read_segs(n, cig.ctypes.data, cig_off.ctypes.data, rs.ctypes.data, lo.ctypes.data, hi.ctypes.data, C.byref(ns)))
    cap = max(1, ns.value)
    g = np.empty(cap, np.uint32); ln = np.empty(cap, np.uint8); sp = np.zeros(cap, np.uint32)
    pl = _aligned((cap, _lib.PLANE_WORDS), np.uint64)
    check(lib.isx_pack_read_planes(n, rs.ctypes.data, lo.ctypes.data, hi.ctypes.data, cig.ctypes.data, cig_off.ctypes.data, seq,
                                   qual.ctypes.data, seq_off.ctypes.data, pv.ctypes.data if pv is not None else None, int(min_base_quality), cap,
                                   g.ctypes.data, ln.ctypes.data, sp.ctypes.data, pl.ctypes.data, C.byref(ns)))
    k = ns.value
    return PlaneBatch(g[:k], ln[:k], pl[:k], sp[:k] if pair is not None else None)


def dense_to_entries(counts, clon):
    tot = counts.sum(axis=1)
    k = np.nonzero(tot > 0)[0]
    e = np.zeros(len(k), dtype=ENTRY_DT)
    e["gpos"] = k
    e["cnt"] = counts[k]
    e["clon"] = clon[k]
    e["clon_rarefied"] = np.nan
    return e


def _name_blob(names):
    enc = [n.encode() if isinstance(n, str) else bytes(n) for n in names]
# ... 246 lines not shown
```

Before: 170.6.

## Send reference as sparse mismatch patches instead of full 2-bit plane

For shallow-coverage batches, the host encoder records each read position where the base differs from the reference, together with the reference code there, in a patch list. The device then zeroes its reference plane and rebuilds only those positions with a small atomicOr kernel, rather than receiving the whole 2-bit plane over H2D. The aim is to cut host-to-device reference bytes. In exchange it adds per-exception work in the hot encode loop, a device memset and kernel, and a fallback to the full plane when the patch region overflows. It is gated by eligibility checks on depth, N content, caching and the allele thresholds.

Result: slower. 142.1 (-16.7%).

```diff
diff --git a/include/instrain_amd.h b/include/instrain_amd.h
--- a/include/instrain_amd.h
+++ b/include/instrain_amd.h
@@ -382,6 +382,9 @@
                       int64_t cap_rec, int64_t ring_records, uint32_t *rec, uint32_t *gbase, int64_t *n_rec, int64_t *need_slack);
 int isx_encode_planes_mm(const isx_read_planes *reads, const isx_ref_planes *ref, int64_t n_pos, int32_t n_mm_bins, int32_t host_threads, int32_t slack_groups,
                          int64_t cap_rec, int64_t ring_records, uint32_t *rec, uint32_t *gbase, int64_t *n_rec, int64_t *need_slack);
+int isx_encode_planes_patches(const isx_read_planes *reads, const isx_ref_planes *ref, int64_t n_pos, int32_t host_threads, int32_t slack_groups,
+                              int64_t cap_rec, int64_t ring_records, uint32_t *rec, uint32_t *gbase, int64_t *n_rec, int64_t *need_slack,
+                              uint32_t *patches, int64_t cap_patches, int64_t *n_entries, int64_t *n_patches, int32_t *overflow);
 
 int isx_count_read_segs(int64_t n_reads, const uint32_t *cigar, const int64_t *cigar_off, const int64_t *ref_start,
                         const int64_t *clip_lo, const int64_t *clip_hi, int64_t *n_seg);
diff --git a/instrain_amd/_lib.py b/instrain_amd/_lib.py
--- a/instrain_amd/_lib.py
+++ b/instrain_amd/_lib.py
@@ -157,7 +157,7 @@
            "isx_batch_summarize", "isx_batch_summarize_genomes", "isx_compare_coverage", "isx_compare_scaffolds", "isx_compare_fetch_snps",
            "isx_genes_create", "isx_genes_destroy", "isx_genes_sites", "isx_batch_profile_genes", "isx_genes_profile_snvs",
            "isx_pipe_create", "isx_pipe_destroy", "isx_pipe_submit", "isx_pipe_submit_reads", "isx_pipe_stage_reads", "isx_pipe_submit_wire", "isx_wire_bytes", "isx_wire_free", "isx_wire_keep_reference", "isx_pipe_submit_bam", "isx_encode_segs", "isx_encode_segs_ring", "isx_seg_records_needed", "isx_encode_delta", "isx_delta_records_needed", "isx_count_read_segs", "isx_pack_reads", "isx_pipe_collect", "isx_pipe_release", "isx_pipe_fetch_entries", "isx_pipe_fetch_entries_shrunk", "isx_levels_expand", "isx_encode_obs", "isx_encode_obs_ring",
-           "isx_pack_ref_planes", "isx_planes_from_segs", "isx_pack_read_planes", "isx_pipe_submit_planes", "isx_pipe_stage_planes", "isx_encode_planes", "isx_encode_planes_mm", "isx_pipe_set_reference_budget", "isx_host_register", "isx_host_unregister",
+           "isx_pack_ref_planes", "isx_planes_from_segs", "isx_pack_read_planes", "isx_pipe_submit_planes", "isx_pipe_stage_planes", "isx_encode_planes", "isx_encode_planes_mm", "isx_encode_planes_patches", "isx_pipe_set_reference_budget", "isx_host_register", "isx_host_unregister",
            "isx_bgzf_index", "isx_bgzf_inflate_device", "isx_bgzf_inflate_host", "isx_bgzf_inflate_fast",
            "isx_bam_open", "isx_bam_close", "isx_bam_close_wait", "isx_bam_set_threads", "isx_bam_ref", "isx_bam_set_priority_reads", "isx_bam_scan", "isx_bam_scan_part",
            "isx_bam_insert_sizes", "isx_bam_set_wanted_refs", "isx_bam_pair_keys", "isx_bam_set_cross_names", "isx_bam_filter_insert_sizes", "isx_bam_filter", "isx_bam_set_r2m", "isx_bam_r2m", "isx_bam_drop_names", "isx_bam_batch_pair_names", "isx_bam_set_mm_cap", "isx_bam_mm_levels", "isx_bam_set_mm_levels", "isx_bam_ref_counts",
@@ -280,6 +280,8 @@
     lib.isx_pipe_stage_planes.argtypes = [vp, i64, C.POINTER(RefPlanes), i32, vp, C.POINTER(ReadPlanes), C.POINTER(vp)]
     lib.isx_encode_planes.argtypes = [C.POINTER(ReadPlanes), C.POINTER(RefPlanes), i64, i32, i32, i64, i64, vp, vp, C.POINTER(i64), C.POINTER(i64)]
     lib.isx_encode_planes_mm.argtypes = [C.POINTER(ReadPlanes), C.POINTER(RefPlanes), i64, i32, i32, i32, i64, i64, vp, vp, C.POINTER(i64), C.POINTER(i64)]
+    lib.isx_encode_planes_patches.argtypes = [C.POINTER(ReadPlanes), C.POINTER(RefPlanes), i64, i32, i32, i64, i64, vp, vp, C.POINTER(i64), C.POINTER(i64),
+                                              vp, i64, C.POINTER(i64), C.POINTER(i64), C.POINTER(i32)]
     lib.isx_bam_ref.argtypes = [vp, i32, C.POINTER(C.c_char_p), C.POINTER(i64), C.POINTER(i64)]
     lib.isx_bam_copy.argtypes = [vp, vp, vp, vp, vp]
     lib.isx_bam_view.argtypes = [vp, C.POINTER(vp), C.POINTER(vp)]
diff --git a/instrain_amd/csrc/isx_pipe.hip b/instrain_amd/csrc/isx_pipe.hip
--- a/instrain_amd/csrc/isx_pipe.hip
+++ b/instrain_amd/csrc/isx_pipe.hip
@@ -98,6 +98,7 @@
     int encode_passes = 0;
     int64_t h2d_bytes = 0, d2h_bytes = 0;
     uint16_t *d_gpos16 = nullptr;
+    std::unique_ptr<isxenc::PatchSink> patch;
 };
 
 static uint64_t bytes_checksum(const void *p, size_t bytes, uint64_t seed)
@@ -168,6 +169,26 @@
         h ^= h >> 29;
     }
     return h;
+}
+
+static const bool pipe_sparse_ref = [] { const char *e = getenv("ISX_PIPE_SPARSE_REF"); return !(e && atoi(e) == 0); }();
+
+constexpr int64_t SPARSE_REF_MAX_DEPTH = 8;
+
+static bool lone_allele_is_present(const std::vector<uint16_t> &thr, int32_t fallback, double min_freq, int32_t min_cov)
+{
+    if (min_cov < 1 || !(min_freq <= 1.0) || (int64_t)fallback > (int64_t)thr.size()) return false;
+    for (size_t t = (size_t)min_cov; t < thr.size(); t++) if ((size_t)thr[t] > t) return false;
+    return true;
+}
+
+__global__ void k_ref_patch(const uint32_t *__restrict__ patches, uint32_t n_entries, uint32_t *__restrict__ plane32, uint32_t n_pos)
+{
+    const uint32_t i = blockIdx.x * blockDim.x + threadIdx.x;
+    if (i >= n_entries) return;
+    const uint32_t e = patches[i], pos = e >> 2;
+    if (e == isxenc::PATCH_NONE || pos >= n_pos || (e & 3u) == 0u) return;
+    atomicOr(&plane32[pos >> 4], (e & 3u) << (2u * (pos & 15u)));
 }
 
 int cgroup_cpus()
@@ -251,6 +272,8 @@
     std::condition_variable cv_stage;
     int64_t next_promise = 0;
     bool stage_stop = false;
+    bool sparse_ref = false;
+    int64_t patch_cap = 0;
 };
 
 static int bounce_d2h(isx_pipe *p, void *hdst, const void *dsrc, size_t bytes, hipStream_t st)
@@ -846,6 +869,15 @@
         if ((i & 1) && p->s_h2d2) p->slots[(size_t)i].h2d = p->s_h2d2;
     }
     if (rc != ISX_OK) { pipe_free(p); return rc; }
+    {
+        const isx_batch *b0 = p->slots[0].b;
+        p->sparse_ref = pipe_sparse_ref && p->drec && b0->M == 1 && b0->lean && p->ring_half == 0 &&
+                        lone_allele_is_present(build_thresholds(c->h_lut, c->fallback, prm->min_freq), c->fallback, prm->min_freq, prm->min_cov);
+        p->patch_cap = (int64_t)(ref2_bytes(pp->max_pos) / sizeof(uint32_t));
+        if (const char *e = getenv("ISX_PIPE_PATCH_CAP")) p->patch_cap = std::max<int64_t>(0, std::min<int64_t>(p->patch_cap, atoll(e)));
+        if (p->sparse_ref) for (Slot &s : p->slots) s.patch.reset(new isxenc::PatchSink());
+        if (pipe_timing) fprintf(stderr, "[isx_pipe_create] reference as patches: %s\n", p->sparse_ref ? "on for eligible batches" : "off");
+    }
     if (!p->slots[0].out_pinned) {
         p->bounce_bytes = (size_t)16 << 20;
         for (int i = 0; i < 2 && rc == ISX_OK; i++) {
@@ -1102,6 +1134,7 @@
 struct RefStage {
     bool early = false;
     uint8_t *resident = nullptr;
+    bool sparse = false;
     double host_ms = 0.0;
 };
 
@@ -1131,6 +1164,19 @@
     }
 
     const bool first_trip = rp && rp->key && p->ref_cache_budget.load(std::memory_order_relaxed) > 0;
+    if (p->sparse_ref && rp && !first_trip && !ring && n_pos < ((int64_t)1 << 30) &&
+        J.n_seg * (int64_t)ISX_SEG_BASES < SPARSE_REF_MAX_DEPTH * n_pos && !(rp->nplane && plane_any(*p->pool, rp->nplane, bn))) {
+        s.ref_has_n = false;
+        J.ref2 = rp->plane2; J.refn = nullptr;
+        s.patch->region = reinterpret_cast<uint32_t *>(s.h_in + s.off_ref); s.patch->cap = p->patch_cap;
+        J.patch = s.patch.get();
+        HIP_TRY(hipEventRecord(s.ev_h2d0, st));
+        HIP_TRY(hipEventRecord(s.ev_h2da, st));
+        out->early = true; out->sparse = true;
+        out->host_ms = now_ms() - t_r;
+        return ISX_OK;
+    }
+
     if (rp && !first_trip && isx_host_is_registered(rp->plane2, b2) && (!rp->nplane || isx_host_is_registered(rp->nplane, bn))) {
         const bool any_n = rp->nplane && plane_any(*p->pool, rp->nplane, bn);
         s.ref_has_n = any_n;
@@ -1155,6 +1201,38 @@
     if (!ring) HIP_TRY(hipEventRecord(s.ev_h2da, st));
     out->early = true;
     if (rp && rp->key) ref_cache_insert(p, s, rp, n_pos);
+    return ISX_OK;
+}
+
+static int slot_send_patches(isx_pipe *p, Slot &s, int64_t n_pos, const isx_ref_planes *rp, size_t *sent, bool *patched)
+{
+    hipStream_t st = H2D(p, s);
+    const size_t b2 = ((size_t)n_pos + 3) / 4, plane_bytes = ref2_bytes(n_pos);
+    const size_t n_ent = (size_t)s.patch->entries(), bytes = n_ent * sizeof(uint32_t);
+    uint8_t *d_plane = s.d_in + s.off_ref, *d_patch = d_plane + ref2_bytes(p->pp.max_pos);
+    *patched = !s.patch->overflow.load() && bytes <= plane_bytes / 2 && bytes <= refn_bytes(p->pp.max_pos);
+    if (pipe_timing)
+        fprintf(stderr, "[isx_pipe_submit_reads] reference as patches: %zu entries (%lld real)%s -> %s\n", n_ent, (long long)s.patch->n_patches.load(),
+                s.patch->overflow.load() ? ", region overflowed" : "", *patched ? "patches" : "the plane after all");
+    if (*patched) {
+        HIP_TRY(hipMemsetAsync(d_plane, 0, plane_bytes, st));
+        if (n_ent) {
+            HIP_TRY(hipMemcpyAsync(d_patch, s.h_in + s.off_ref, bytes, hipMemcpyHostToDevice, st));
+            hipLaunchKernelGGL(k_ref_patch, dim3((unsigned)((n_ent + 255) / 256)), dim3(256), 0, st, reinterpret_cast<const uint32_t *>(d_patch), (uint32_t)n_ent,
+                               reinterpret_cast<uint32_t *>(d_plane), (uint32_t)n_pos);
+            HIP_TRY(hipGetLastError());
+        }
+        *sent = bytes;
+        return ISX_OK;
+    }
+    if (isx_host_is_registered(rp->plane2, b2)) HIP_TRY(hipMemcpyAsync(d_plane, rp->plane2, b2, hipMemcpyHostToDevice, st));
+    else {
+        isx_ref_planes only2 = *rp;
+        only2.nplane = nullptr;
+        (void)copy_ref_planes(*p->pool, &only2, n_pos, s.h_in + s.off_ref, s.h_in + s.off_ref + plane_bytes);
+        HIP_TRY(hipMemcpyAsync(d_plane, s.h_in + s.off_ref, plane_bytes, hipMemcpyHostToDevice, st));
+    }
+    *sent = plane_bytes;
     return ISX_OK;
 }
 
@@ -1321,6 +1399,9 @@
         }
         early_rec = true;
     }
+    size_t ref_sent = 0;
+    bool ref_patched = false;
+    if (rs.sparse && (rc = slot_send_patches(p, s, n_pos, rp, &ref_sent, &ref_patched)) != ISX_OK) return rc;
     if (!planes_in) s.ref_has_n = isxenc::pack_ref_planes(*p->pool, ref, n_pos, s.h_in + s.off_ref, s.h_in + s.off_ref + ref2_bytes(n_pos));
     const double t_ref = now_ms();
     memcpy(s.h_in + s.off_bounds, split_bounds, (size_t)(n_splits + 1) * sizeof(int64_t));
@@ -1351,6 +1432,7 @@
     if (ring) { if (feed.bytes != rec_bytes) { isx_set_error("internal: the staging ring did not carry the whole stream"); return ISX_ERR_STATE; } }
     else if (!early_rec) HIP_TRY(hipMemcpyAsync(s.d_in + s.off_rec, s.h_in + s.off_rec, rec_bytes, hipMemcpyHostToDevice, H2D(p, s)));
     s.h2d_bytes = (int64_t)(head + gb_bytes + rec_bytes) - (rs.resident ? (int64_t)ref_bytes : 0);
+    if (rs.sparse) s.h2d_bytes += (int64_t)ref_sent - (int64_t)ref_bytes;
     if (linkage && !p->drec) {
         HIP_TRY(hipMemcpyAsync(s.d_in + s.off_pairs, s.h_in + s.off_pairs, (size_t)b->n_rec * sizeof(uint32_t), hipMemcpyHostToDevice, H2D(p, s)));
         s.h2d_bytes += (int64_t)b->n_rec * 4;
diff --git a/instrain_amd/csrc/seg_encode.cpp b/instrain_amd/csrc/seg_encode.cpp
--- a/instrain_amd/csrc/seg_encode.cpp
+++ b/instrain_amd/csrc/seg_encode.cpp
@@ -573,6 +573,16 @@
         if ((o[0] & ISX_DREC_DUAL) && ((o[4] >> 16) & 0xFFu)) o[4] += up;
     }
     G.lo = new_lo;
+}
+
+__attribute__((noinline)) uint32_t *patch_turn_chunk(PatchSink *PS, const uint8_t *ref2, uint32_t *b, uint32_t *e, bool more)
+{
+    for (uint32_t *q = b; q < e; q++) {
+        const uint32_t pos = *q;
+        *q = (pos << 2) | (((uint32_t)ref2[pos >> 2] >> ((pos & 3u) * 2u)) & 3u);
+    }
+    if (e > b) PS->n_patches.fetch_add((int64_t)(e - b), std::memory_order_relaxed);
+    return more ? PS->take() : nullptr;
 }
 
 struct PlaneScratch {
@@ -633,6 +643,7 @@
 int encode_planes(HostPool &pool, SegJob &J)
 {
     const int64_t n = J.n_seg;
+    if (J.patch) J.patch->reset();
     const bool producer = (bool)J.produce_planes;
     const uint32_t *gpos_all = producer ? J.gpos_all : J.in2.gpos;
     const int n_tasks = (int)((n + TASK - 1) / TASK);
@@ -1054,8 +1065,32 @@
     return isx_encode_planes_mm(reads, ref, n_pos, 1, host_threads, slack_groups, cap_rec, ring_records, rec, gbase, n_rec, need_slack);
 }
 
+static int encode_planes_host(const isx_read_planes *reads, const isx_ref_planes *ref, int64_t n_pos, int32_t n_mm_bins, int32_t host_threads, int32_t slack_groups,
+                              int64_t cap_rec, int64_t ring_records, uint32_t *rec, uint32_t *gbase, int64_t *n_rec, int64_t *need_slack, isxenc::PatchSink *sink);
+
 int isx_encode_planes_mm(const isx_read_planes *reads, const isx_ref_planes *ref, int64_t n_pos, int32_t n_mm_bins, int32_t host_threads, int32_t slack_groups,
                          int64_t cap_rec, int64_t ring_records, uint32_t *rec, uint32_t *gbase, int64_t *n_rec, int64_t *need_slack)
+{
+    return encode_planes_host(reads, ref, n_pos, n_mm_bins, host_threads, slack_groups, cap_rec, ring_records, rec, gbase, n_rec, need_slack, nullptr);
+}
+
+int isx_encode_planes_patches(const isx_read_planes *reads, const isx_ref_planes *ref, int64_t n_pos, int32_t host_threads, int32_t slack_groups,
+                              int64_t cap_rec, int64_t ring_records, uint32_t *rec, uint32_t *gbase, int64_t *n_rec, int64_t *need_slack,
+                              uint32_t *patches, int64_t cap_patches, int64_t *n_entries, int64_t *n_patches, int32_t *overflow)
+{
+    if (!patches || cap_patches < 0 || !n_entries || !n_patches || !overflow || n_pos >= ((int64_t)1 << 30)) {
+        isx_set_error("isx_encode_planes_patches: bad argument (the patch array, its three results, n_pos < 2^30)");
+        return ISX_ERR_ARG;
+    }
+    isxenc::PatchSink sink;
+    sink.region = patches; sink.cap = cap_patches;
+    const int rc = encode_planes_host(reads, ref, n_pos, 1, host_threads, slack_groups, cap_rec, ring_records, rec, gbase, n_rec, need_slack, &sink);
+    *n_entries = sink.entries(); *n_patches = sink.n_patches.load(); *overflow = sink.overflow.load();
+    return rc;
+}
+
+static int encode_planes_host(const isx_read_planes *reads, const isx_ref_planes *ref, int64_t n_pos, int32_t n_mm_bins, int32_t host_threads, int32_t slack_groups,
+                              int64_t cap_rec, int64_t ring_records, uint32_t *rec, uint32_t *gbase, int64_t *n_rec, int64_t *need_slack, isxenc::PatchSink *sink)
 {
     if (n_mm_bins < 1 || n_mm_bins > 128) { isx_set_error("isx_encode_planes: n_mm_bins must be in [1, 128]"); return ISX_ERR_ARG; }
     if (!reads || !ref || !ref->plane2 || !rec || !gbase || !n_rec || reads->n_seg < 0 || cap_rec < ISX_DREC_GROUP || (cap_rec % ISX_DREC_GROUP) || n_pos <= 0 ||
@@ -1071,6 +1106,7 @@
     isxenc::SegJob J;
     J.in2 = *reads; J.n_seg = reads->n_seg; J.n_pos = n_pos; J.n_mm_bins = n_mm_bins;
     J.ref2 = ref->plane2; J.refn = ref->nplane; J.slack_groups = std::max(1, slack_groups);
+    J.patch = sink;
     J.rec = rec; J.gbase = gbase; J.pair_out = nullptr;
     J.cmin = cmin.data(); J.cmax = cmax.data(); J.cany = cany.data(); J.cap_rec = cap_rec;
     if (ring_records) {
diff --git a/instrain_amd/csrc/seg_encode.h b/instrain_amd/csrc/seg_encode.h
--- a/instrain_amd/csrc/seg_encode.h
+++ b/instrain_amd/csrc/seg_encode.h
@@ -1,6 +1,7 @@
 #pragma once
 #include <stdint.h>
 
+#include <atomic>
 #include <functional>
 #include <vector>
 
@@ -13,6 +14,24 @@
 
 namespace isxenc {
 
+constexpr int64_t PATCH_CHUNK = 512;
+constexpr uint32_t PATCH_NONE = 0xFFFFFFFFu;
+struct PatchSink {
+    uint32_t *region = nullptr;
+    int64_t cap = 0;
+    std::atomic<int64_t> taken{0};
+    std::atomic<int64_t> n_patches{0};
+    std::atomic<int> overflow{0};
+    void reset() { taken.store(0); n_patches.store(0); overflow.store(0); }
+    uint32_t *take()
+    {
+        const int64_t at = taken.fetch_add(PATCH_CHUNK, std::memory_order_relaxed);
+        if (at + PATCH_CHUNK > cap) { overflow.store(1, std::memory_order_relaxed); return nullptr; }
+        return region + at;
+    }
+    int64_t entries() const { return overflow.load() ? 0 : taken.load(); }
+};
+
 struct SegJob {
     isx_segs in{};
     std::function<void(int64_t first, int64_t count, uint32_t *gpos, uint8_t *len, uint8_t *mm, uint32_t *pair, uint32_t *bases)> produce;
@@ -20,6 +39,7 @@
     isx_read_planes in2{};
     std::function<void(int64_t first, int64_t count, uint32_t *gpos, uint8_t *len, uint8_t *mm, uint32_t *pair, uint64_t *planes)> produce_planes;
     const uint8_t *ref2 = nullptr, *refn = nullptr;
+    PatchSink *patch = nullptr;
     int64_t n_seg = 0, n_pos = 0;
     int n_mm_bins = 1;
     bool want_pairs = false;
diff --git a/instrain_amd/csrc/seg_planes.inc b/instrain_amd/csrc/seg_planes.inc
--- a/instrain_amd/csrc/seg_planes.inc
+++ b/instrain_amd/csrc/seg_planes.inc
@@ -113,6 +113,20 @@
 #endif
     const bool mm_on = J.n_mm_bins > 1;
     const int64_t pf_end = K.e - PLANES_PREFETCH;
+    PatchSink *const PS = J.patch;
+    uint32_t patch_none[1];
+    uint32_t *pb = patch_none, *pc = patch_none, *pe = nullptr;
+    bool patching = PS != nullptr;
+    auto patch_turn = [&]() __attribute__((always_inline)) {
+        uint32_t *c = patch_turn_chunk(PS, ref2, pb, pc, true);
+        patching = c != nullptr;
+        pb = pc = c ? c : patch_none; pe = c ? c + PATCH_CHUNK : nullptr;
+    };
+    auto patch_push = [&](uint32_t q) __attribute__((always_inline)) {
+        *pc++ = q;
+        if (__builtin_expect(pc == pe, 0)) patch_turn();
+    };
+    if (patching) patch_turn();
     for (int64_t s = K.a; s < K.e; s++) {
         const uint32_t L = ln[s], p = gp[s];
         const uint64_t *P = K.pl + (size_t)s * ISX_PLANE_WORDS;
@@ -202,6 +216,11 @@
             const uint32_t col = t0 + (t1 & m0) + (t2 & m01);
             const uint32_t code = (uint32_t)(P[col >> 5] >> (2 * (col & 31u))) & 3u;
             const uint32_t w0 = 0x3FFFFC00u | ((col | (code << 8) | (0u - (uint32_t)(n_exc == 0))) & 0x3FFu);
+            if (patching) {
+                *pc = p + col;
+                pc += n_exc;
+                if (__builtin_expect(pc == pe, 0)) patch_turn();
+            }
             if (__builtin_expect(plain, 0)) { add_plain(p, L, pid, w0, ISX_DREC_NO_EXC); continue; }
 #if ISX_PLANES_VARIANT == 2
             if (__builtin_expect(in_regs, 1)) {
@@ -224,6 +243,7 @@
                 const int k = ex[0] ? 0 : (ex[1] ? 1 : 2);
                 const uint32_t col = (uint32_t)(64 * k + __builtin_ctzll(ex[k]));
                 ex[k] &= ex[k] - 1;
+                if (patching) patch_push(p + col);
                 const uint64_t code = (P[col >> 5] >> (2 * (col & 31u))) & 3u;
                 fields |= ((uint64_t)col | (code << 8)) << (10 * i);
             }
@@ -243,6 +263,7 @@
                     const uint32_t col = (uint32_t)(64 * k + __builtin_ctzll(ex[k]));
                     if (nf == max_exc) { end = col; goto cut; }
                     ex[k] &= ex[k] - 1;
+                    if (patching) patch_push(p + col);
                     const uint32_t code = (uint32_t)(P[col >> 5] >> (2 * (col & 31u))) & 3u;
                     const uint32_t f = ((col - b) & 0xFFu) | (code << 8);
                     const int wi = (int)(nf / 3), shf = 10 * (int)(nf % 3);
@@ -267,6 +288,10 @@
         for (int r = 0; r < ISX_DREC_GROUP; r++) put_empty_drec(o + (size_t)r * ISX_DREC_WORDS);
         J.gbase[G.g] = 0; J.cmin[G.g] = 0xFFFFFFFFu; J.cmax[G.g] = 0; J.cany[G.g] = 0;
     }
+    if (PS && pe) {
+        (void)patch_turn_chunk(PS, ref2, pb, pc, false);
+        for (; pc < pe; pc++) *pc = PATCH_NONE;
+    }
     if (K.fast_store) _mm_sfence();
     K.used = G.used; K.np = np; K.nb = nb; K.maxp = maxp;
 }
diff --git a/instrain_amd/engine.py b/instrain_amd/engine.py
--- a/instrain_amd/engine.py
+++ b/instrain_amd/engine.py
@@ -783,6 +783,26 @@
         return rec[:n], gbase[:n // 32], None, slack_groups
 
 
+def encode_planes_patches(reads, ref_planes, cap_patches, threads=1, slack_groups=1, ring_records=0):
+    lib = _lib.load()
+    while True:
+        cap = int(lib.isx_delta_records_needed(reads.gpos.ctypes.data if reads.n_seg else None, reads.n_seg, int(threads), int(slack_groups)))
+        rec = _aligned((cap, 8), np.uint32)
+        gbase = np.empty(cap // 32, dtype=np.uint32)
+        patches = np.full(int(cap_patches) + 64, 0xA5A5A5A5, dtype=np.uint32)
+        n_rec, need, n_ent, n_pat, ovf = C.c_int64(0), C.c_int64(0), C.c_int64(0), C.c_int64(0), C.c_int32(0)
+        cr, cf = reads.c(), ref_planes.c()
+        rc = lib.isx_encode_planes_patches(C.byref(cr), C.byref(cf), ref_planes.n_pos, int(threads), int(slack_groups), cap, int(ring_records),
+                                           rec.ctypes.data, gbase.ctypes.data, C.byref(n_rec), C.byref(need),
+                                           patches.ctypes.data, int(cap_patches), C.byref(n_ent), C.byref(n_pat), C.byref(ovf))
+        if rc == _lib.ERR_CAPACITY and need.value > slack_groups:
+            slack_groups = int(need.value)
+            continue
+        check(rc)
+        n = n_rec.value
+        return rec[:n], gbase[:n // 32], patches, int(n_ent.value), int(n_pat.value), bool(ovf.value)
+
+
 def dense_cov(res, n_pos=None):
     if "cov16" in res:
         return res["cov16"]
```
